# ikergarcia1996/AI-Generated-GTAV

Hardware: AMD Instinct MI355X
Metric: generated frames/sec (32-frame clip, 100 noise steps) (higher is better)
Workload: dtype fp16 (fp32 accumulate/residual)

## Files before the change

### ai-generated-gtav_amd/csrc/api.hip

```cpp
#include "api_internal.h"

namespace gtav_shared { thread_local hipEvent_t g_launch_ev[2] = {nullptr, nullptr}; }
namespace gtav {
static thread_local char g_err[1024] = "";
void set_error(const char* fmt, ...) {
    va_list ap;
    va_start(ap, fmt);
    vsnprintf(g_err, sizeof(g_err), fmt, ap);
    va_end(ap);
}
const char* last_error() { return g_err; }
}
namespace gtav_bf16 {
void set_error(const char* fmt, ...) {
    va_list ap;
    va_start(ap, fmt);
    vsnprintf(gtav::g_err, sizeof(gtav::g_err), fmt, ap);
    va_end(ap);
}
const char* last_error() { return gtav::g_err; }
}

namespace {
const gtav_bf16::GemmParams& bfp(const GemmParams& p) { return reinterpret_cast<const gtav_bf16::GemmParams&>(p); }
const gtav_bf16::LnPending* bfl(const LnPending* p) { return reinterpret_cast<const gtav_bf16::LnPending*>(p); }
int f16_attn_spatial(const f16* Q, const f16* K, const f16* Vt, f16* O, int NB, int heads, int S, hipStream_t st, bool qp) { return launch_attn_spatial(Q, K, Vt, O, NB, heads, S, st, qp); }
int bf_gemm(const GemmParams& p, int epi, hipStream_t st) { return gtav_bf16::launch_gemm(bfp(p), epi, st); }
int bf_ln_modulate(float* x, int ldx, f16* out, int ldo, int M, int D, const float* shift, const float* scale, int mod_stride, const int* rows, int rpm,
                   const LnPending* pend, int* ef, hipStream_t st) {
    return gtav_bf16::launch_ln_modulate(x, ldx, (__bf16*)out, ldo, M, D, shift, scale, mod_stride, rows, rpm, bfl(pend), ef, st);
}
int bf_ln_affine(float* x, int ldx, f16* out, int ldo, int M, int D, const float* gamma, const float* beta, const LnPending* pend, int* ef, hipStream_t st) {
    return gtav_bf16::launch_ln_affine(x, ldx, (__bf16*)out, ldo, M, D, gamma, beta, bfl(pend), ef, st);
}
int bf_patchify(const float* img, const int* fi, int NB, int C, int H, int W, int p, f16* out, int ldo, float a, float b, int* ef, hipStream_t st) {
    return gtav_bf16::launch_patchify(img, fi, NB, C, H, W, p, (__bf16*)out, ldo, a, b, ef, st);
}
int f16_convert_pad(const float* src, int lds, int R, int C, f16* dst, int Rp, int Cp, float scale, int tiled, hipStream_t st, int* ef) {
    return launch_convert_pad_f16(src, lds, R, C, dst, Rp, Cp, scale, tiled, st, ef);
}
int bf_convert_pad(const float* src, int lds, int R, int C, f16* dst, int Rp, int Cp, float scale, int tiled, hipStream_t st, int* ef) {
    return gtav_bf16::launch_convert_pad_f16(src, lds, R, C, (__bf16*)dst, Rp, Cp, scale, tiled, st, ef);
}
int bf_unpad(const f16* src, int lds, int R, int C, float* dst, int tiled, hipStream_t st) { return gtav_bf16::launch_unpad_f16_to_f32((const __bf16*)src, lds, R, C, dst, tiled, st); }
int bf_attn_spatial(const f16* Q, const f16* K, const f16* Vt, f16* O, int NB, int heads, int S, hipStream_t st, bool qp) {
    return gtav_bf16::launch_attn_spatial((const __bf16*)Q, (const __bf16*)K, (const __bf16*)Vt, (__bf16*)O, NB, heads, S, st, qp);
}
int bf_attn_temporal(const f16* q, const f16* kv, f16* O, int B, int P, int D, int Tq, int t0, int Tmax, hipStream_t st) {
    return gtav_bf16::launch_attn_temporal((const __bf16*)q, (const __bf16*)kv, (__bf16*)O, B, P, D, Tq, t0, Tmax, st);
}
const OperandOps OPS_F16 = {launch_gemm, launch_ln_modulate, launch_ln_affine, launch_patchify, f16_convert_pad, launch_unpad_f16_to_f32, f16_attn_spatial,
                            launch_attn_temporal, false};
const OperandOps OPS_BF16 = {bf_gemm, bf_ln_modulate, bf_ln_affine, bf_patchify, bf_convert_pad, bf_unpad, bf_attn_spatial, bf_attn_temporal, true};
}
const OperandOps& gtav::operand_ops(bool bf16) { return bf16 ? OPS_BF16 : OPS_F16; }

namespace {
typedef const __bf16* cbp;
typedef __bf16* bp;
int f16_dw_grouped(const GemmDwGroup* g, int n, int K, int* ef, hipStream_t st, bool tn) { return launch_gemm_dw_grouped(g, n, K, ef, st, tn); }
int bf_gemm_tn(const GemmParams& p, hipStream_t st) { return gtav_bf16::launch_gemm_tn(bfp(p), st); }
int bf_dw_grouped(const GemmDwGroup* g, int n, int K, int* ef, hipStream_t st, bool tn) {
    return gtav_bf16::launch_gemm_dw_grouped(reinterpret_cast<const gtav_bf16::GemmDwGroup*>(g), n, K, ef, st, tn);
}
int bf_transpose(const f16* src, int R, int C, f16* dst, hipStream_t st) { return gtav_bf16::launch_transpose_tiled_f16((cbp)src, R, C, (bp)dst, st); }
int bf_convert_T(const float* src, int lds, int R, int C, f16* dst, hipStream_t st) { return gtav_bf16::launch_convert_T_f16(src, lds, R, C, (bp)dst, st); }
int bf_gelu(const f16* u, f16* h, size_t n, hipStream_t st) { return gtav_bf16::launch_gelu_tiled((cbp)u, (bp)h, n, st); }
int bf_gelu_bwd(const f16* dh, const f16* u, f16* du, size_t n, int* ef, hipStream_t st) { return gtav_bf16::launch_gelu_bwd_tiled((cbp)dh, (cbp)u, (bp)du, n, ef, st); }
int bf_gelu_bwd_colsum(const f16* dh, const f16* u, f16* du, int M, int N, float* db, float* ws, int* ef, hipStream_t st) {
    return gtav_bf16::launch_gelu_bwd_tiled_colsum((cbp)dh, (cbp)u, (bp)du, M, N, db, ws, ef, st);
}
int bf_gate_bwd(const float* dres, const float* gate, int ms, int rpm, int M, int D, f16* dy, int* ef, hipStream_t st) {
    return gtav_bf16::launch_gate_bwd(dres, gate, ms, rpm, M, D, (bp)dy, ef, st);
}
int bf_frame_reduce_gate(const float* dres, const f16* y, int frames, int P, int D, float* dgate, int ms, hipStream_t st) {
    return gtav_bf16::launch_frame_reduce_gate(dres, (cbp)y, frames, P, D, dgate, ms, st);
}
int bf_gate_bwd_fused(const float* dres, const f16* y, const float* gate, int ms, int frames, int P, int D, f16* dy, float* dgate, float* db, float* ws, int* ef,
                      hipStream_t st) {
    return gtav_bf16::launch_gate_bwd_fused(dres, (cbp)y, gate, ms, frames, P, D, (bp)dy, dgate, db, ws, ef, st);
}
int bf_colsum(const f16* dy, int M, int N, float* db, float* ws, hipStream_t st) { return gtav_bf16::launch_colsum_tiled_f16((cbp)dy, M, N, db, ws, st); }
int bf_to_tiled(const float* a, int M, int D, f16* out, int* ef, hipStream_t st) { return gtav_bf16::launch_to_tiled_f16(a, M, D, (bp)out, ef, st); }
int bf_mse_bwd(const float* vp, const float* vt, int B, int T, int C, int H, int W, int p, float scale, f16* dfo, int ldf, int* ef, hipStream_t st) {
    return gtav_bf16::launch_mse_bwd_patch(vp, vt, B, T, C, H, W, p, scale, (bp)dfo, ldf, ef, st);
}
int bf_attn_spatial_bwd(const f16* Q, const f16* K, const f16* Vt, const f16* dO, int NB, int heads, int S, int D, const float* cs, f16* dqkv, int* ef,
                        hipStream_t st) {
    return gtav_bf16::launch_attn_spatial_bwd((cbp)Q, (cbp)K, (cbp)Vt, (cbp)dO, NB, heads, S, D, cs, (bp)dqkv, ef, st);
}
int bf_attn_temporal_bwd(const f16* q, const f16* kv, const f16* dO, int B, int P, int D, int T, int Tmax, const float* cs, f16* dqkv, int* ef, hipStream_t st) {
    return gtav_bf16::launch_attn_temporal_bwd((cbp)q, (cbp)kv, (cbp)dO, B, P, D, T, Tmax, cs, (bp)dqkv, ef, st);
}
int bf_adamw_multi(const AdamParam* params, const AdamItem* items, int n, const float* ctl, float lr, float b1, float b2, float eps, float wd, hipStream_t st) {
    return gtav_bf16::launch_adamw_multi(reinterpret_cast<const gtav_bf16::AdamParam*>(params), reinterpret_cast<const gtav_bf16::AdamItem*>(items), n, ctl, lr,
                                         b1, b2, eps, wd, st);
}
const TrainOps TRAIN_F16 = {launch_gemm_tn, f16_dw_grouped, launch_transpose_tiled_f16, launch_convert_T_f16, launch_gelu_tiled, launch_gelu_bwd_tiled,
                            launch_gelu_bwd_tiled_colsum, launch_gate_bwd, launch_frame_reduce_gate, launch_gate_bwd_fused, launch_colsum_tiled_f16,
                            launch_to_tiled_f16, launch_mse_bwd_patch, launch_attn_spatial_bwd, launch_attn_temporal_bwd, launch_adamw_multi, false};
const TrainOps TRAIN_BF16 = {bf_gemm_tn, bf_dw_grouped, bf_transpose, bf_convert_T, bf_gelu, bf_gelu_bwd, bf_gelu_bwd_colsum, bf_gate_bwd, bf_frame_reduce_gate,
                             bf_gate_bwd_fused, bf_colsum, bf_to_tiled, bf_mse_bwd, bf_attn_spatial_bwd, bf_attn_temporal_bwd, bf_adamw_multi, true};
// ... 79 lines not shown
    g.gate = gate; g.gate_stride = gate_stride; g.rows_per_gate = rows_per_gate;
    return launch_gemm(g, epilogue, (hipStream_t)stream);
}
int gtav_op_gemm_qkv(const void* x, int32_t ldx, const void* w, const float* bias, int32_t M, int32_t D, int32_t mode, void* q,
                     void* k, void* v, int32_t S, int32_t Tq, int32_t t0, int32_t Tmax, const float* rope_cs, void* stream) {
    GemmParams g;
    memset(&g, 0, sizeof(g));
    g.X = (const f16*)x; g.ldx = ldx; g.W = (const f16*)w; g.M = M; g.N = 3 * D; g.K = D; g.bias = bias; g.D = D; g.S = S;
    g.qkv_mode = mode; g.q = (f16*)q; g.k = (f16*)k; g.v = (f16*)v; g.Tq = Tq; g.t0 = t0; g.Tmax = Tmax;
    g.rope_cs = rope_cs;
    return launch_gemm(g, EPI_QKV, (hipStream_t)stream);
}
#ifdef GTAV_EXPERIMENTS
int gtav_op_gemm_fold_producer(const void* x, const void* w, const float* bias, float* resid, int32_t M, int32_t N, int32_t K, const float* gate,
                               const float* next_scale, int32_t mod_stride, int32_t tokens_per_frame, void* a_out, float* stats_out, void* stream) {
    GemmParams g;
    memset(&g, 0, sizeof(g));
    g.X = (const f16*)x; g.ldx = K; g.W = (const f16*)w; g.M = M; g.N = N; g.K = K; g.bias = bias; g.out = resid; g.ldo = N;
    g.gate = gate; g.gate_stride = mod_stride; g.rows_per_gate = tokens_per_frame;
    g.f_P = tokens_per_frame; g.f_scale = next_scale; g.f_stats_out = stats_out; g.f_a = (f16*)a_out;
    return launch_gemm(g, EPI_RESID_FOLD, (hipStream_t)stream);
}
int gtav_op_gemm_fold_consumer(const void* a, const void* w, int32_t M, int32_t N, int32_t K, int32_t epi, const float* stats, const float* c1, const float* c2,
                               int32_t ldc, int32_t tokens_per_frame, void* out, int32_t ldo, void* stream) {
    GTAV_REQUIRE(epi == EPI_F32 || epi == EPI_GELU_TANH, "gemm_fold_consumer: epilogue %d (0 = f32 row-major, 2 = GELU-tanh fp16 tile-major)", epi);
    GemmParams g;
    memset(&g, 0, sizeof(g));
    g.X = (const f16*)a; g.ldx = K; g.W = (const f16*)w; g.M = M; g.N = N; g.K = K; g.out = out; g.ldo = ldo;
    g.f_P = tokens_per_frame; g.f_stats = stats; g.f_nslot = K / 64; g.f_c1 = c1; g.f_c2 = c2; g.f_ldc = ldc;
    return launch_gemm(g, epi == EPI_F32 ? EPI_F32_FOLD : EPI_GELU_TANH_FOLD, (hipStream_t)stream);
}
#endif
int gtav_op_skinny_f32(const float* x, int32_t ldx, const float* w, const float* bias, float* y, int32_t ldy, int32_t M,
                       int32_t N, int32_t K, int32_t act_silu, void* stream) {
    RET_IF(skinny_init());
    return launch_skinny_f32(x, ldx, w, bias, y, ldy, M, N, K, act_silu, (hipStream_t)stream);
}
int gtav_op_ln_modulate(const float* x, void* out, int32_t M, int32_t D, const float* shift, const float* scale,
                        int32_t mod_stride, int32_t rows_per_mod, void* stream) {
    return launch_ln_modulate((float*)x, D, (f16*)out, D, M, D, shift, scale, mod_stride, nullptr, rows_per_mod, nullptr, nullptr, (hipStream_t)stream);
}
int gtav_op_ln_affine(const float* x, void* out, int32_t M, int32_t D, const float* gamma, const float* beta, void* stream) {
    return launch_ln_affine((float*)x, D, (f16*)out, D, M, D, gamma, beta, nullptr, nullptr, (hipStream_t)stream);
}
int gtav_op_attn_spatial(const void* q, const void* k, const void* vt, void* o, int32_t NB, int32_t heads, int32_t S, void* stream) {
    return launch_attn_spatial((const f16*)q, (const f16*)k, (const f16*)vt, (f16*)o, NB, heads, S, (hipStream_t)stream);
}
int gtav_op_attn_temporal(const void* q, const void* kv, void* o, int32_t B, int32_t P, int32_t D, int32_t Tq, int32_t t0,
                          int32_t Tmax, void* stream) {
    return launch_attn_temporal((const f16*)q, (const f16*)kv, (f16*)o, B, P, D, Tq, t0, Tmax, (hipStream_t)stream);
}
int gtav_op_attn_temporal_bf16(const void* q, const void* kv, void* o, int32_t B, int32_t P, int32_t D, int32_t Tq, int32_t t0,
                               int32_t Tmax, void* stream) {
    return gtav_bf16::launch_attn_temporal((const __bf16*)q, (const __bf16*)kv, (__bf16*)o, B, P, D, Tq, t0, Tmax, (hipStream_t)stream);
}
int gtav_op_qkv_head_major(const void* w, void* w_hm, int32_t D, void* stream) {
    return launch_qkv_head_major((const f16*)w, (f16*)w_hm, D, (hipStream_t)stream);
}
int gtav_op_gemm_qkvt_attn(const void* x_tperm, const void* w_hm, int32_t M, int32_t D, int32_t P, int32_t Tq, int32_t t0,
                           int32_t Tmax, const float* rope_cs, void* kv, void* o, void* stream) {
    GemmParams g;
    memset(&g, 0, sizeof(g));
    g.X = (const f16*)x_tperm; g.ldx = D; g.W = (const f16*)w_hm; g.M = M; g.N = 3 * D; g.K = D; g.D = D; g.S = P;
    g.qkv_mode = QKV_TEMPORAL; g.k = (f16*)kv; g.v = (f16*)kv; g.out = o; g.ldo = D; g.Tq = Tq; g.t0 = t0; g.Tmax = Tmax;
    g.rope_cs = rope_cs;
    return launch_gemm_qkvt_attn(g, (hipStream_t)stream);
}
int gtav_op_qkv_head_major_spatial(const void* w, void* w_hm, int32_t D, void* stream) {
    return launch_qkv_head_major((const f16*)w, (f16*)w_hm, D, (hipStream_t)stream, 1);
}
int gtav_op_gemm_qkvs_attn(const void* x, const void* w_hm, int32_t M, int32_t D, int32_t P, const float* rope_cs, void* o, void* stream) {
    GemmParams g;
    memset(&g, 0, sizeof(g));
    g.X = (const f16*)x; g.ldx = D; g.W = (const f16*)w_hm; g.M = M; g.N = 3 * D; g.K = D; g.D = D; g.S = P;
    g.qkv_mode = QKV_SPATIAL; g.out = o; g.ldo = D; g.rope_cs = rope_cs;
    return launch_gemm_qkvs_attn(g, (hipStream_t)stream);
}
int gtav_op_attn_spatial_bwd(const void* q, const void* k, const void* vt, const void* d_o, int32_t NB, int32_t heads, int32_t S,
                             const float* rope_cs, void* dqkv, void* stream) {
    return launch_attn_spatial_bwd((const f16*)q, (const f16*)k, (const f16*)vt, (const f16*)d_o, NB, heads, S, heads * 64, rope_cs, (f16*)dqkv, nullptr,
                                   (hipStream_t)stream);
}
int gtav_op_attn_spatial_bwd_bf16(const void* q, const void* k, const void* vt, const void* d_o, int32_t NB, int32_t heads, int32_t S,
                                  const float* rope_cs, void* dqkv, void* stream) {
    return gtav_bf16::launch_attn_spatial_bwd((const __bf16*)q, (const __bf16*)k, (const __bf16*)vt, (const __bf16*)d_o, NB, heads, S, heads * 64, rope_cs,
                                              (__bf16*)dqkv, nullptr, (hipStream_t)stream);
}
int gtav_op_gemm_tn(const void* x, const void* w, int32_t M, int32_t N, int32_t K, float* out, int32_t ldo, void* stream) {
    GemmParams q;
    memset(&q, 0, sizeof(q));
    q.X = (const f16*)x; q.ldx = M; q.W = (const f16*)w; q.M = M; q.N = N; q.K = K; q.out = out; q.ldo = ldo;
    return launch_gemm_tn(q, (hipStream_t)stream);
}
int gtav_op_gemm_dw_grouped(int32_t n, const void* const* x, const void* const* w, float* const* out, const int32_t* M, const int32_t* N, const int32_t* ldo,
                            int32_t K, void* stream) {
    GTAV_REQUIRE(n >= 1 && n <= GEMM_DW_MAX_GROUPS && x && w && out && M && N && ldo, "op_gemm_dw_grouped: 1 .. %d groups", GEMM_DW_MAX_GROUPS);
    GemmDwGroup g[GEMM_DW_MAX_GROUPS];
    for (int i = 0; i < n; ++i) g[i] = GemmDwGroup{(const f16*)x[i], (const f16*)w[i], out[i], M[i], N[i], ldo[i]};
    return launch_gemm_dw_grouped(g, n, K, nullptr, (hipStream_t)stream);
}
int gtav_op_gemm_splitk_ln(const void* x, int32_t ldx, const void* w, const float* bias, int32_t M, int32_t N, int32_t K,
                           int32_t splitk, float* parts, float* resid, const float* gate, int32_t gate_stride,
                           int32_t rows_per_gate, void* out_f16, const float* shift, const float* scale, int32_t mod_stride,
                           void* stream) {
    GemmParams g;
    memset(&g, 0, sizeof(g));
    g.X = (const f16*)x; g.ldx = ldx; g.W = (const f16*)w; g.M = M; g.N = N; g.K = K; g.out = parts; g.ldo = N;
// ... 62 lines not shown
```

### ai-generated-gtav_amd/csrc/api_dit.hip

```cpp
#include "api_internal.h"

#ifdef GTAV_EXPERIMENTS
static int fold_alloc(gtav_dit* h) {
    gtav_dit::Fold& f = h->fold;
    if (f.ok) return 0;
    GTAV_REQUIRE(f.geom_ok, "dit_set_fold: this geometry has no LayerNorm fold (tokens per frame %d must be a multiple of 16 and >= 64, hidden %% 256 == 0)", h->P);
    Arena& a = h->arena;
    const int D = h->D;
    const size_t Mx = round_up(h->Mmax, 128);
    int rc = 0;
#define A_(expr) do { if (!rc) rc = (expr); } while (0)
    {
        const int nhb = h->L * 2, nseam = 2 * nhb + 1;
        f.col_c.assign(nseam, 0);
        int col = 0;
        for (int hb = 0; hb < nhb; ++hb) { f.col_c[2 * hb + 1] = col; col += 2 * h->Hm; }
        for (int hb = 0; hb < nhb; ++hb) { f.col_c[2 * hb] = col; col += 2 * 3 * D; }
        f.col_c[2 * nhb] = col; col += 2 * h->Nfin;
        f.CTW = col;
        f.n_groups = 2 * nseam; f.n_groups_a = 2 * nhb;
        f.Rp = round_up(h->max_rows, 128);
        A_(a.alloc_t(&f.ctab, (size_t)h->max_rows * f.CTW));
        A_(a.alloc_t(&f.ctab_cur, (size_t)h->maxB * h->maxT * f.CTW));
        A_(a.alloc_t(&f.stats, Mx * (size_t)(D / 64) * 2));
// ... 15 lines not shown
                add(nhb + hb, 2 * hb, h->halves[hb].w_qkv, 3 * D, nullptr, (hb * 6 + 0) * D, (hb * 6 + 1) * D);
            }
            add(2 * nhb, 2 * nhb, h->w_final, h->Nfin, h->b_final, h->L * 12 * D, h->L * 12 * D + D);
            if (hipMemcpy(f.groups_dev, groups.data(), groups.size() * sizeof(GemmGroup), hipMemcpyHostToDevice) != hipSuccess ||
                hipMemcpy(f.gcol_dev, gcol.data(), gcol.size() * sizeof(int), hipMemcpyHostToDevice) != hipSuccess ||
                hipMemcpy(f.gscale_dev, gsc.data(), gsc.size() * sizeof(int), hipMemcpyHostToDevice) != hipSuccess) {
                set_error("dit_create: upload of the LayerNorm-fold group tables failed");
                rc = 1;
            }
            f.ok = !rc;
        }
    }
#undef A_
    return rc;
}
#endif

static bool fused_spatial_ok(int M, int D, int P) { return gemm_qkvs_attn_ok(M, D, P) && M / P >= 5 && (M / P) * (D / 64) >= 80; }

static void fold_policy(const gtav_dit* h, int M, bool& fa, bool& fb) {
    const gtav_dit::Fold& f = h->fold;
    fa = fb = false;
    if (!f.ok || f.mode == 0 || h->tr.on || h->fuse_tattn || h->any_bf16) return;
    fa = f.mode == 2 || M >= f.min_m_a;
    fb = f.mode == 2 || M >= f.min_m_b;
}
static int dit_fold_tables(gtav_dit* h, int rows, bool fa, bool fb, hipStream_t s) {
    if (!fa && !fb) return 0;
#ifndef GTAV_EXPERIMENTS
    (void)h; (void)rows; (void)s;
    GTAV_REQUIRE(false, "the LayerNorm fold exists only in the experiments build");
#else
    gtav_dit::Fold& f = h->fold;
    const int ng = fb ? f.n_groups : f.n_groups_a;
    RET_IF(launch_ctab_inputs(h->mod, h->MODW, rows, round_up(rows, 128), h->D, f.gcol_dev, f.gscale_dev, ng, f.sx, (size_t)f.Rp * h->D, s));
    return launch_gemm_grouped(f.groups_dev, ng, h->Hm > 3 * h->D ? h->Hm : 3 * h->D, rows, h->D, s);
#endif
}

static int dit_cond(gtav_dit* h, const int64_t* t64, int rows, int Tq, const StepParams* sp, int use_cur, const float* actions,
                    int64_t act_outer, int64_t act_inner, hipStream_t s) {
    GTAV_REQUIRE(rows <= h->max_rows, "conditioning rows %d exceed max_cond_rows %d", rows, h->max_rows);
    const int ldhc = h->D + h->Apad;
    RET_IF(launch_cond_inputs(t64, rows, Tq, sp, use_cur, h->sincos, h->E, actions, act_outer, act_inner, h->A, h->HC, ldhc,
                              h->D, h->Apad, h->err_flag, s));
    RET_IF(launch_skinny_f32(h->E, 256, h->w_t0, h->b_t0, h->HC, ldhc, rows, h->D, 256, 1, s));
    RET_IF(launch_skinny_f32(h->HC, ldhc, h->w_t2cat, actions ? h->b_t2a : h->b_t2, h->Sc, h->D, rows, h->D, ldhc, 1, s));
    RET_IF(launch_skinny_f32(h->Sc, h->D, h->w_ada, h->b_ada, h->mod, h->MODW, rows, h->MODW, h->D, 0, s));
    bool fa, fb;
    fold_policy(h, rows * h->P, fa, fb);
    return dit_fold_tables(h, rows, fa, fb, s);
}

static int dit_forward_core(gtav_dit* h, const float* x_src, const int* frame_index, int B, int Tq, int t0,
                            const float* mod, const int* mod_rows, const float* ctab, float* v_out, hipStream_t s) {
    const int D = h->D, P = h->P, NB = B * Tq, M = NB * P;
    GTAV_REQUIRE(M <= h->Mmax, "forward: %d tokens exceed workspace (%d)", M, h->Mmax);
    bool fold_a, fold_b;
    fold_policy(h, M, fold_a, fold_b);
    const gtav_dit::Fold& fo = h->fold;
    auto fold_consumer = [&](GemmParams& q, int seam, int N) {
        q.bias = nullptr;
        q.f_P = P; q.f_rows = mod_rows; q.f_stats = fo.stats; q.f_nslot = D / 64;
        q.f_c1 = ctab + fo.col_c[seam]; q.f_c2 = q.f_c1 + N; q.f_ldc = fo.CTW;
    };
    auto fold_producer = [&](int cls, const f16* X, const f16* Wt, int K, const float* bias, const float* gate, const float* next_scale) -> int {
        GemmParams q;
        memset(&q, 0, sizeof(q));
        q.X = X; q.ldx = K; q.W = Wt; q.M = M; q.N = D; q.K = K; q.out = h->resid; q.ldo = D; q.bias = bias; q.err_flag = h->err_flag;
        q.gate = gate; q.gate_stride = h->MODW; q.gate_rows = mod_rows; q.rows_per_gate = P;
        q.f_P = P; q.f_rows = mod_rows; q.f_scale = next_scale; q.f_stats_out = fo.stats; q.f_a = h->xn;
        PROF(h, cls, s, launch_gemm(q, EPI_RESID_FOLD, s));
        return 0;
    };
    const int g_embed = 2 * h->L, g_final = 2 * h->L + 1;
    PROF(h, PC_OTHER, s, h->ops(g_embed).patchify(x_src, frame_index, NB, h->C, h->H, h->W, h->p, h->xp, h->Kpe, 1.f, 0.f, h->err_of(g_embed), s));
    GemmParams g;
    memset(&g, 0, sizeof(g));
    g.X = h->xp; g.ldx = h->Kpe; g.W = h->w_pe; g.M = M; g.N = D; g.K = h->Kpe; g.bias = h->b_pe; g.out = h->resid; g.ldo = D;
    PROF(h, PC_OTHER, s, h->ops(g_embed).gemm(g, EPI_F32, s));
    LnPending pend;
    bool have_pend = false;
    const int pf_max_m = 1536;
    static const int pf_min_m = GTAV_ENV_INT("GTAV_PF_MIN_M", 256);
    const bool pf_on = h->w_prefetch && M >= pf_min_m && M <= pf_max_m;
    struct PfNext { const f16* W; int N, K, sk, consumer; };
    auto pf_target = [&](int hb, int pos) -> PfNext {
        const int q = pos + 1, hb2 = hb + q / 4, p2 = q % 4;
        if (!pf_on || hb2 >= 2 * h->L) return PfNext{nullptr, 0, 0, 1, 0};
        const gtav_dit::Half& w2 = h->halves[hb2];
        if (p2 == 0) {
            const bool fused2 = !h->tr.on && w2.w_qkv_hm && !h->ops(hb2).bf16 &&
                                ((hb2 & 1) ? h->fuse_tattn && gemm_qkvt_attn_ok(M, D, P, Tq, t0) : h->fuse_sattn && fused_spatial_ok(M, D, P));
            return PfNext{fused2 ? w2.w_qkv_hm : w2.w_qkv, 3 * D, D, 1, 3};
        }
        if (p2 == 1) return PfNext{w2.w_out, D, D, gemm_choose_splitk(M, D, D), 0};
        if (p2 == 2) return PfNext{w2.w_fc1, h->Hm, D, 1, 1};
        return PfNext{w2.w_fc2, D, h->Hm_pad, gemm_choose_splitk(M, D, h->Hm_pad), 2};
    };
    auto set_pf = [&](GemmParams& q, const PfNext& t) {
        const int v = h->w_prefetch_cls[t.consumer];
        if (!pf_on || !t.W || !v) return;
        const int nkt = t.K / 64;
        int skn = t.sk;
        if (skn < 1 || nkt % skn || (skn >= 8 ? skn % 8 : 8 % skn)) skn = 1;
        q.pf = PrefetchDesc{t.W, cdiv(t.N, 128), nkt, skn, v >= 2 ? v : 0};
    };
    auto resid_gemm = [&](const OperandOps& ops, int cls, const f16* X, int ldx, const f16* Wt, int K, const float* bias, const float* gate, const PfNext& pfn) -> int {
        GemmParams q;
        memset(&q, 0, sizeof(q));
        q.X = X; q.ldx = ldx; q.W = Wt; q.M = M; q.N = D; q.K = K; q.out = h->parts; q.ldo = D;
        set_pf(q, pfn);
        q.splitk = gemm_choose_splitk(M, D, K);
        if (gemm_pp_ok(M, D, K, EPI_RESID) || (q.splitk == 1 && M >= h->resid_inplace_min_m) || gemm_resid_inplace_ok(M, D, K, P)) {
            q.splitk = 0; q.out = h->resid; q.bias = bias; q.gate = gate; q.gate_stride = h->MODW; q.gate_rows = mod_rows;
            q.rows_per_gate = P;
            PROF(h, cls, s, ops.gemm(q, EPI_RESID, s));
            have_pend = false;
            return 0;
        }
        GTAV_REQUIRE((size_t)q.splitk * M <= h->parts_rows, "split-K slabs exceed workspace");
        PROF(h, cls, s, ops.gemm(q, EPI_PARTIAL, s));
        memset(&pend, 0, sizeof(pend));
        pend.parts = h->parts; pend.nsplit = q.splitk; pend.slab_stride = (size_t)M * D; pend.ld = D; pend.bias = bias;
        pend.gate = gate; pend.gate_stride = h->MODW; pend.gate_rows = mod_rows; pend.rows_per_gate = P;
        have_pend = true;
        return 0;
    };
    bool folded_in = false;
    for (int l = 0; l < h->L; ++l) {
        for (int hf = 0; hf < 2; ++hf) {
            const int hb = l * 2 + hf;
            const gtav_dit::Half& w = h->halves[hb];
            const OperandOps& ops = h->ops(hb);
            int* const ef = h->err_of(hb);
            const float* mb = mod + (size_t)hb * 6 * D;
            const bool fused_t = hf == 1 && h->fuse_tattn && !h->tr.on && !ops.bf16 && w.w_qkv_hm && gemm_qkvt_attn_ok(M, D, P, Tq, t0);
            if (fused_t) {
                if (!have_pend) memset(&pend, 0, sizeof(pend));
                pend.tperm_T = Tq; pend.tperm_P = P;
            }
            if (!folded_in)
                PROF(h, PC_LN, s, ops.ln_modulate(h->resid, D, h->xn, D, M, D, mb, mb + D, h->MODW, mod_rows, P, (have_pend || fused_t) ? &pend : nullptr, ef, s));
            have_pend = false;
            memset(&g, 0, sizeof(g));
            g.X = h->xn; g.ldx = D; g.W = w.w_qkv; g.M = M; g.N = 3 * D; g.K = D; g.D = D; g.S = P; g.err_flag = ef;
            if (folded_in) fold_consumer(g, 2 * hb, 3 * D);
            set_pf(g, pf_target(hb, 0));
            const bool fused_s = hf == 0 && h->fuse_sattn && !h->tr.on && !ops.bf16 && !folded_in && w.w_qkv_hm && fused_spatial_ok(M, D, P);
            if (fused_t) {
                g.W = w.w_qkv_hm; g.qkv_mode = QKV_TEMPORAL; g.k = h->kvcache[l]; g.v = h->kvcache[l]; g.out = h->ao; g.ldo = D;
                g.Tq = Tq; g.t0 = t0; g.Tmax = h->maxT; g.rope_cs = h->rope_t.cs_dev;
                PROF(h, PC_ATTN_T, s, launch_gemm_qkvt_attn(g, s));
            } else if (fused_s) {
                g.W = w.w_qkv_hm; g.qkv_mode = QKV_SPATIAL; g.out = h->ao; g.ldo = D; g.rope_cs = h->rope_s.cs_dev;
                PROF(h, PC_ATTN_S, s, launch_gemm_qkvs_attn(g, s));
            } else {
                if (hf == 0) {
                    g.qkv_mode = QKV_SPATIAL; g.q = h->qs; g.k = h->ks; g.v = h->vts;
                    g.rope_cs = h->rope_s.cs_dev;
                } else {
                    g.qkv_mode = QKV_TEMPORAL; g.q = h->qt; g.k = h->kvcache[l]; g.v = h->kvcache[l];
                    g.Tq = Tq; g.t0 = t0; g.Tmax = h->maxT;
                    g.rope_cs = h->rope_t.cs_dev;
                }
                PROF(h, PC_QKV, s, ops.gemm(g, folded_in ? EPI_QKV_FOLD : EPI_QKV, s));
                if (hf == 0) PROF(h, PC_ATTN_S, s, ops.attn_spatial(h->qs, h->ks, h->vts, h->ao, NB, h->heads, P, s, false));
                else PROF(h, PC_ATTN_T, s, ops.attn_temporal(h->qt, h->kvcache[l], h->ao, B, P, D, Tq, t0, h->maxT, s));
            }
            folded_in = false;
            memset(&g, 0, sizeof(g));
            g.X = h->xn; g.ldx = D; g.W = w.w_fc1; g.M = M; g.N = h->Hm; g.K = D; g.bias = w.b_fc1; g.out = h->hbuf; g.ldo = h->Hm_pad; g.err_flag = ef;
            set_pf(g, pf_target(hb, 2));
            if (fold_a) {
                RET_IF(fold_producer(PC_OUT, h->ao, w.w_out, D, w.b_out, mb + 2 * D, mb + 4 * D));
                fold_consumer(g, 2 * hb + 1, h->Hm);
                PROF(h, PC_FC1, s, launch_gemm(g, EPI_GELU_TANH_FOLD, s));
            } else {
                RET_IF(resid_gemm(ops, PC_OUT, h->ao, D, w.w_out, D, w.b_out, mb + 2 * D, pf_target(hb, 1)));
                PROF(h, PC_LN, s, ops.ln_modulate(h->resid, D, h->xn, D, M, D, mb + 3 * D, mb + 4 * D, h->MODW, mod_rows, P, have_pend ? &pend : nullptr, ef, s));
                have_pend = false;
                PROF(h, PC_FC1, s, ops.gemm(g, EPI_GELU_TANH, s));
            }
            if (fold_b) {
                const float* next_scale = hb + 1 < 2 * h->L ? mod + (size_t)(hb + 1) * 6 * D + D : mod + (size_t)h->L * 12 * D + D;
                RET_IF(fold_producer(PC_FC2, h->hbuf, w.w_fc2, h->Hm_pad, w.b_fc2, mb + 5 * D, next_scale));
                folded_in = true;
            } else {
                RET_IF(resid_gemm(ops, PC_FC2, h->hbuf, h->Hm_pad, w.w_fc2, h->Hm_pad, w.b_fc2, mb + 5 * D, pf_target(hb, 3)));
            }
        }
    }
    const float* mf = mod + (size_t)h->L * 12 * D;
    if (!folded_in)
        PROF(h, PC_LN, s, h->ops(g_final).ln_modulate(h->resid, D, h->xn, D, M, D, mf, mf + D, h->MODW, mod_rows, P, have_pend ? &pend : nullptr, h->err_of(g_final), s));
    memset(&g, 0, sizeof(g));
    g.X = h->xn; g.ldx = D; g.W = h->w_final; g.M = M; g.N = h->Nfin; g.K = D; g.bias = h->b_final; g.out = h->fo; g.ldo = h->Nfin;
    if (folded_in) fold_consumer(g, 4 * h->L, h->Nfin);
    PROF(h, PC_OTHER, s, h->ops(g_final).gemm(g, folded_in ? EPI_F32_FOLD : EPI_F32, s));
    PROF(h, PC_OTHER, s, launch_unpatchify(h->fo, h->Nfin, v_out, NB, h->C, h->H, h->W, h->p, 0, 1.f, 0.f, s));
    PROF(h, PC_EMPTY, s, 0);
    return h->prof.collect(s);
}

extern "C" {



int gtav_dit_create(const gtav_dit_config* c, gtav_dit** out) {
    GTAV_REQUIRE(c && out, "dit_create: null argument");
    GTAV_REQUIRE(c->hidden_size % 256 == 0 && c->hidden_size <= 2048, "hidden_size=%d must be a multiple of 256, <= 2048", c->hidden_size);
    GTAV_REQUIRE(c->num_heads > 0 && c->hidden_size / c->num_heads == 64 && c->hidden_size % c->num_heads == 0,
                 "only head_dim 64 is implemented (hidden %d, heads %d)", c->hidden_size, c->num_heads);
    GTAV_REQUIRE(c->input_h % c->patch_size == 0 && c->input_w % c->patch_size == 0, "input %dx%d not divisible by patch %d",
                 c->input_h, c->input_w, c->patch_size);
    GTAV_REQUIRE(c->max_frames >= 1 && c->max_frames <= 32, "max_frames=%d must be in [1, 32]", c->max_frames);
    GTAV_REQUIRE(c->max_batch >= 1 && c->depth >= 1, "bad max_batch/depth");
    RET_IF(skinny_init());
    gtav_dit* h = new gtav_dit();
    h->cfg = *c;
    h->D = c->hidden_size; h->L = c->depth; h->heads = c->num_heads; h->C = c->in_channels; h->p = c->patch_size;
    h->H = c->input_h; h->W = c->input_w; h->gh = h->H / h->p; h->gw = h->W / h->p; h->P = h->gh * h->gw;
    const int D = h->D;
    if ((h->P % 8) != 0) {
        set_error("tokens per frame P=%d must be a multiple of 8", h->P);
        delete h;
        return 2;
    }
    h->Hm = (int)(D * c->mlp_ratio); h->Hm_pad = round_up(h->Hm, 128);
    h->A = c->external_cond_dim > 0 ? c->external_cond_dim : 0; h->Apad = round_up(h->A > 0 ? h->A : 1, 32);
    h->MODW = h->L * 12 * D + 2 * D;
    h->Kpe = round_up(h->C * h->p * h->p, 64);
    h->Nfin = h->p * h->p * h->C;
    h->maxB = c->max_batch; h->maxT = c->max_frames; h->Mmax = h->maxB * h->maxT * h->P;
    h->max_rows = c->max_cond_rows > h->maxB * h->maxT ? c->max_cond_rows : h->maxB * h->maxT;
    Arena& a = h->arena;
    WeightTable& wt = h->wt;
    int rc = 0;
#define A_(expr) do { if (!rc) rc = (expr); } while (0)
    A_(a.alloc_t(&h->w_pe, (size_t)round_up(D, 128) * h->Kpe));
    h->n_groups = 2 * h->L + 2;
    h->grp_bf16.assign(h->n_groups, 0);
    wt.add_f16("x_embedder.proj.weight", D, h->C * h->p * h->p, h->w_pe, round_up(D, 128), h->Kpe, 2 * h->L);
    A_(a.alloc_t(&h->b_pe, D)); wt.add_f32("x_embedder.proj.bias", 1, D, h->b_pe, D);
    A_(a.alloc_t(&h->w_t0, (size_t)D * 256)); wt.add_f32("t_embedder.mlp.0.weight", D, 256, h->w_t0, 256);
    A_(a.alloc_t(&h->b_t0, D)); wt.add_f32("t_embedder.mlp.0.bias", 1, D, h->b_t0, D);
    const int ldhc = D + h->Apad;
    A_(a.alloc_t(&h->w_t2cat, (size_t)D * ldhc)); wt.add_f32("t_embedder.mlp.2.weight", D, D, h->w_t2cat, ldhc, 0);
    A_(a.alloc_t(&h->b_t2, D)); wt.add_f32("t_embedder.mlp.2.bias", 1, D, h->b_t2, D);
    A_(a.alloc_t(&h->b_ext, D)); A_(a.alloc_t(&h->b_t2a, D));
    if (h->A > 0) {
        wt.add_f32("external_cond.weight", D, h->A, h->w_t2cat, ldhc, D);
        wt.add_f32("external_cond.bias", 1, D, h->b_ext, D);
// ... 106 lines not shown
                const float ang = (float)t * ft[d / 2];
                c[t * 64 + d] = cosf(ang); sn[t * 64 + d] = sinf(ang);
            }
        RET_IF(upload(h->rope_t.cos_dev, c)); RET_IF(upload(h->rope_t.sin_dev, sn));
    }
    if (!h->wt.slots["tables.timestep_sincos"].set) {
        std::vector<float> tab((size_t)1000 * 256);
        for (int k = 0; k < 128; ++k) {
            const float f = expf(-logf(10000.0f) * (float)k / 128.0f);
            for (int t = 0; t < 1000; ++t) {
                const float arg = (float)t * f;
                tab[(size_t)t * 256 + k] = cosf(arg);
                tab[(size_t)t * 256 + 128 + k] = sinf(arg);
            }
        }
        RET_IF(upload(h->sincos, tab));
    }
    for (size_t hb = 0; hb < h->halves.size(); ++hb) {
        gtav_dit::Half& w = h->halves[hb];
        if (w.w_qkv_hm) RET_IF(launch_qkv_head_major(w.w_qkv, w.w_qkv_hm, D, s, (hb & 1) ? 0 : 1));
    }
    RET_IF(launch_rope_interleave(h->rope_s.cos_dev, h->rope_s.sin_dev, h->rope_s.cs_dev, h->P, s));
    RET_IF(launch_rope_interleave(h->rope_t.cos_dev, h->rope_t.sin_dev, h->rope_t.cs_dev, h->maxT, s));
    GTAV_CHECK_HIP(hipStreamSynchronize(s));
    h->finalized = true;
    return 0;
}

int gtav_dit_forward(gtav_dit* h, const float* x, const int64_t* t, const float* actions, float* out, int32_t B, int32_t T,
                     void* stream) {
    GTAV_REQUIRE(h && x && t && out, "dit_forward: null argument");
    GTAV_REQUIRE(h->finalized, "dit_forward: call gtav_dit_finalize first");
    GTAV_REQUIRE(B >= 1 && B <= h->maxB && T >= 1 && T <= h->maxT, "dit_forward: B=%d T=%d outside capacity (%d, %d)", B, T, h->maxB, h->maxT);
    GTAV_REQUIRE(!actions || h->A > 0, "dit_forward: model has no external_cond");
    hipStream_t s = (hipStream_t)stream;
    h->prepared.valid = false;
    h->kvrec.valid = false;
    RET_IF(dit_cond(h, t, B * T, 1, nullptr, 0, actions, h->A, 0, s));
    return dit_forward_core(h, x, nullptr, B, T, 0, h->mod, nullptr, h->fold.ctab, out, s);
}

int gtav_dit_set_schedule(gtav_dit* h, const float* ac, int32_t n) {
    GTAV_REQUIRE(h && ac && n == 1000, "dit_set_schedule: expected 1000 alphas_cumprod values");
    h->ac_host.assign(ac, ac + n);
    GTAV_CHECK_HIP(hipMemcpy(h->ac_table, ac, n * sizeof(float), hipMemcpyHostToDevice));
    return 0;
}

static int denoise_step_body(gtav_dit* h, float* x, int B, int F, int T, const float* actions, int mode, float* v_out,
                             bool prepared, hipStream_t s) {
    const size_t fsz = (size_t)h->C * h->H * h->W;
    const int Tq = mode == 1 ? 1 : T, t0 = mode == 1 ? T - 1 : 0;
    if (!prepared) RET_IF(dit_cond(h, nullptr, B * Tq, Tq, h->step_dev, mode == 1, actions, (int64_t)F * h->A, h->A, s));
    RET_IF(dit_forward_core(h, x, h->frame_idx, B, Tq, t0, prepared ? h->mod_cur : h->mod, nullptr, prepared ? h->fold.ctab_cur : h->fold.ctab, h->vout, s));
    const float* vlast = h->vout + (size_t)(Tq - 1) * fsz;
    RET_IF(launch_ddim_update_step(x, F, vlast, (size_t)Tq * fsz, B, (int)fsz, h->step_dev, s));
    if (v_out) RET_IF(launch_copy_rows_f32(vlast, (size_t)Tq * fsz, v_out, fsz, B, fsz, s));
    return 0;
}

int gtav_dit_prepare_frame(gtav_dit* h, int32_t B, int32_t F, int32_t start, int32_t cur, int32_t t_ctx,
                           const int32_t* t_steps_host, int32_t n_steps, const float* actions, void* stream) {
    GTAV_REQUIRE(h && t_steps_host, "prepare_frame: null argument");
    GTAV_REQUIRE(h->finalized, "prepare_frame: finalize the model first");
    const int T = cur - start + 1;
    GTAV_REQUIRE(start >= 0 && cur < F && T >= 1 && T <= h->maxT && B >= 1 && B <= h->maxB && n_steps >= 1 && n_steps <= 1024,
                 "prepare_frame: bad window [%d, %d] / steps %d", start, cur, n_steps);
    GTAV_REQUIRE(!actions || h->A > 0, "prepare_frame: model has no external_cond");
    const int rows = B * (T - 1) + n_steps * B;
    GTAV_REQUIRE(rows <= h->max_rows, "prepare_frame: %d conditioning rows exceed max_cond_rows %d", rows, h->max_rows);
    hipStream_t s = (hipStream_t)stream;
    GTAV_CHECK_HIP(hipStreamSynchronize(s));
    GTAV_CHECK_HIP(hipMemcpy(h->t_steps_dev, t_steps_host, n_steps * sizeof(int), hipMemcpyHostToDevice));
    const int ldhc = h->D + h->Apad;
    RET_IF(launch_cond_inputs_frame(rows, B, T, F, start, cur, t_ctx, h->t_steps_dev, h->sincos, h->E, actions, h->A, h->HC, ldhc,
                                    h->D, h->Apad, h->err_flag, s));
    RET_IF(launch_skinny_f32(h->E, 256, h->w_t0, h->b_t0, h->HC, ldhc, rows, h->D, 256, 1, s));
    RET_IF(launch_skinny_f32(h->HC, ldhc, h->w_t2cat, actions ? h->b_t2a : h->b_t2, h->Sc, h->D, rows, h->D, ldhc, 1, s));
    RET_IF(launch_skinny_f32(h->Sc, h->D, h->w_ada, h->b_ada, h->mod, h->MODW, rows, h->MODW, h->D, 0, s));
    {
        bool fa, fb, fa1, fb1;
        fold_policy(h, B * T * h->P, fa, fb);
        fold_policy(h, B * h->P, fa1, fb1);
        RET_IF(dit_fold_tables(h, rows, fa || fa1, fb || fb1, s));
        h->prepared.fold_tables = fa || fa1 || fb || fb1;
    }
    GTAV_CHECK_HIP(hipMemsetAsync(h->mod_last, 0xFF, (size_t)h->maxB * h->maxT * sizeof(int), s));
    h->prepared.valid = true; h->prepared.B = B; h->prepared.F = F; h->prepared.start = start; h->prepared.cur = cur;
    h->prepared.n_steps = n_steps; h->prepared.actions = actions;
    return 0;
}

int gtav_dit_denoise_step(gtav_dit* h, float* x, int32_t B, int32_t F, int32_t start, int32_t cur, int32_t t_ctx,
                          int32_t t_cur, int32_t t_next, int32_t is_final, const float* actions, int32_t mode,
                          int32_t cond_step, float* v_out, void* stream) {
    GTAV_REQUIRE(h && x, "denoise_step: null argument");
    GTAV_REQUIRE(h->finalized && !h->ac_host.empty(), "denoise_step: finalize the model and set the schedule first");
    const int T = cur - start + 1;
    GTAV_REQUIRE(start >= 0 && cur < F && T >= 1 && T <= h->maxT && B >= 1 && B <= h->maxB, "denoise_step: bad window [%d, %d] of %d frames", start, cur, F);
    GTAV_REQUIRE(t_cur >= 0 && t_cur < 1000 && t_next >= 0 && t_next < 1000 && t_ctx >= 0 && t_ctx < 1000, "denoise_step: timestep out of range");
    GTAV_REQUIRE(!actions || h->A > 0, "denoise_step: model has no external_cond");
    GTAV_REQUIRE(mode == 0 || mode == 1, "denoise_step: mode %d", mode);
    const bool prepared = cond_step >= 0;
    if (prepared)
        GTAV_REQUIRE(h->prepared.valid && h->prepared.B == B && h->prepared.F == F && h->prepared.start == start &&
                         h->prepared.cur == cur && cond_step < h->prepared.n_steps && h->prepared.actions == actions,
                     "denoise_step: cond_step=%d but gtav_dit_prepare_frame was not called for this window", cond_step);
// ... 247 lines not shown
```

### ai-generated-gtav_amd/csrc/api_train.hip

```cpp
#include "api_internal.h"

static int g_dw_grouped = GTAV_ENV_INT("GTAV_DW_GROUPED", 1);
static int g_fuse_gelu_fwd = GTAV_ENV_INT("GTAV_FUSE_GELU_FWD", 1);
static int g_fuse_gelu = GTAV_ENV_INT("GTAV_FUSE_GELU_BWD", 1);
static int g_fuse_ln = GTAV_ENV_INT("GTAV_FUSE_LN_BWD", 1);
static int g_fuse_gate = GTAV_ENV_INT("GTAV_FUSE_GATE", 1);
static int g_dw_tn = GTAV_ENV_INT("GTAV_DW_TN", 1);

static int train_enable_body(gtav_dit* h, float* grad_arena_dev, int64_t grad_arena_numel);

static int train_window_ok(const gtav_dit* h) {
    GTAV_REQUIRE(h->maxT <= 8, "train_enable: training is implemented for windows of at most 8 frames (the backward temporal attention and the adaLN-gradient "
                 "reduction are sized for it); this handle was created with max_frames=%d", h->maxT);
    return 0;
}

extern "C" {

int gtav_dit_train_enable(gtav_dit* h, float* grad_arena_dev, int64_t grad_arena_numel) {
    GTAV_REQUIRE(h, "train_enable: null handle");
    RET_IF(train_window_ok(h));
    GTAV_REQUIRE(!h->tr.on, "train_enable: already enabled");
    GTAV_REQUIRE(!h->any_bf16, "train_enable: the training step runs on fp16 operands (gtav_dit_set_operand_dtype(h, -1, GTAV_OPERAND_F16) first)");
    return train_enable_body(h, grad_arena_dev, grad_arena_numel);
// ... 161 lines not shown
    GTAV_REQUIRE(h && x && t64 && out, "train_forward: null argument");
    GTAV_REQUIRE(h->tr.on && h->finalized, "train_forward: call gtav_dit_train_enable, load the weights and finalize first");
    GTAV_REQUIRE(B >= 1 && B <= h->maxB && T >= 1 && T <= h->maxT, "train_forward: B=%d T=%d outside capacity (%d, %d)", B, T, h->maxB, h->maxT);
    GTAV_REQUIRE(!actions || h->A > 0, "train_forward: model has no external_cond");
    hipStream_t s = (hipStream_t)stream;
    gtav_dit::Train& tr = h->tr;
    const int D = h->D, P = h->P, NB = B * T, M = NB * P, L = h->L, rows = NB, ldhc = D + h->Apad;
    h->prepared.valid = false;
    h->kvrec.valid = false;
    RET_IF(launch_cond_inputs(t64, rows, 1, nullptr, 0, h->sincos, h->E, actions, h->A, 0, h->A, h->HC, ldhc, D, h->Apad, h->err_flag, s));
    RET_IF(launch_skinny_f32(h->E, 256, h->w_t0, h->b_t0, tr.z0, D, rows, D, 256, 0, s));
    RET_IF(launch_silu(tr.z0, D, h->HC, ldhc, rows, D, s));
    RET_IF(launch_skinny_f32(h->HC, ldhc, h->w_t2cat, actions ? h->b_t2a : h->b_t2, tr.cpre, D, rows, D, ldhc, 0, s));
    RET_IF(launch_silu(tr.cpre, D, h->Sc, D, rows, D, s));
    RET_IF(launch_skinny_f32(h->Sc, D, h->w_ada, h->b_ada, h->mod, h->MODW, rows, h->MODW, D, 0, s));
    const float* mod = h->mod;
    const OperandOps& oe = h->ops(2 * L), &ofin = h->ops(2 * L + 1);
    RET_IF(oe.patchify(x, nullptr, NB, h->C, h->H, h->W, h->p, tr.xp, h->Kpe, 1.f, 0.f, h->err_flag, s));
    GemmParams g;
    memset(&g, 0, sizeof(g));
    g.X = tr.xp; g.ldx = h->Kpe; g.W = h->w_pe; g.M = M; g.N = D; g.K = h->Kpe; g.bias = h->b_pe; g.out = tr.res[0]; g.ldo = D;
    RET_IF(oe.gemm(g, EPI_F32, s));
    LnPending pend;
    bool have_pend = false;
    auto resid_gemm = [&](const OperandOps& o, const f16* X, const f16* Wt, int K, const float* bias, const float* gate, float* x_out, f16* y_save) -> int {
        GemmParams q;
        memset(&q, 0, sizeof(q));
        q.X = X; q.ldx = K; q.W = Wt; q.M = M; q.N = D; q.K = K; q.out = h->parts; q.ldo = D;
        q.splitk = gemm_choose_splitk(M, D, K);
        GTAV_REQUIRE((size_t)q.splitk * M <= h->parts_rows, "split-K slabs exceed workspace");
        RET_IF(o.gemm(q, EPI_PARTIAL, s));
        memset(&pend, 0, sizeof(pend));
        pend.parts = h->parts; pend.nsplit = q.splitk; pend.slab_stride = (size_t)M * D; pend.ld = D; pend.bias = bias;
        pend.gate = gate; pend.gate_stride = h->MODW; pend.gate_rows = nullptr; pend.rows_per_gate = P;
        pend.x_out = x_out; pend.y_save = y_save;
        have_pend = true;
        return 0;
    };
    for (int l = 0; l < L; ++l)
        for (int hf = 0; hf < 2; ++hf) {
            const int i = l * 2 + hf;
            const gtav_dit::Half& w = h->halves[i];
            gtav_dit::Train::HB& b = tr.hb[i];
            const float* mb = mod + (size_t)i * 6 * D;
            const OperandOps& o = h->ops(i);
            RET_IF(o.ln_modulate(i == 0 ? tr.res[0] : tr.res[2 * i - 1], D, b.xnA, D, M, D, mb, mb + D, h->MODW, nullptr, P, have_pend ? &pend : nullptr, h->err_flag, s));
            have_pend = false;
            memset(&g, 0, sizeof(g));
            g.X = b.xnA; g.ldx = D; g.W = w.w_qkv; g.M = M; g.N = 3 * D; g.K = D; g.D = D; g.S = P; g.err_flag = h->err_flag;
            if (hf == 0) { g.qkv_mode = QKV_SPATIAL; g.q = b.q; g.k = b.k; g.v = b.v; g.rope_cs = h->rope_s.cs_dev; }
            else { g.qkv_mode = QKV_TEMPORAL; g.q = b.q; g.k = b.k; g.v = b.k; g.Tq = T; g.t0 = 0; g.Tmax = h->maxT; g.rope_cs = h->rope_t.cs_dev; }
            RET_IF(o.gemm(g, EPI_QKV, s));
            if (hf == 0) RET_IF(o.attn_spatial(b.q, b.k, b.v, b.ao, NB, h->heads, P, s, false));
            else RET_IF(o.attn_temporal(b.q, b.k, b.ao, B, P, D, T, 0, h->maxT, s));
            RET_IF(resid_gemm(o, b.ao, w.w_out, D, w.b_out, mb + 2 * D, tr.res[2 * i + 1], b.y1));
            RET_IF(o.ln_modulate(tr.res[2 * i], D, b.xnB, D, M, D, mb + 3 * D, mb + 4 * D, h->MODW, nullptr, P, &pend, h->err_flag, s));
            have_pend = false;
            memset(&g, 0, sizeof(g));
            g.X = b.xnB; g.ldx = D; g.W = w.w_fc1; g.M = M; g.N = h->Hm; g.K = D; g.bias = w.b_fc1; g.out = b.u; g.ldo = h->Hm_pad; g.err_flag = h->err_flag;
            if (g_fuse_gelu_fwd) g.out2 = b.hh;
            RET_IF(o.gemm(g, EPI_F16_TILED, s));
            if (!g_fuse_gelu_fwd) RET_IF(h->tops(i).gelu_tiled(b.u, b.hh, (size_t)round_up(M, 128) * h->Hm_pad, s));
            RET_IF(resid_gemm(o, b.hh, w.w_fc2, h->Hm_pad, w.b_fc2, mb + 5 * D, tr.res[2 * i + 2], b.y2));
        }
    const float* mf = mod + (size_t)L * 12 * D;
    RET_IF(ofin.ln_modulate(tr.res[4 * L - 1], D, tr.xnF, D, M, D, mf, mf + D, h->MODW, nullptr, P, &pend, h->err_flag, s));
    memset(&g, 0, sizeof(g));
    g.X = tr.xnF; g.ldx = D; g.W = h->w_final; g.M = M; g.N = h->Nfin; g.K = D; g.bias = h->b_final; g.out = h->fo; g.ldo = h->Nfin;
    RET_IF(ofin.gemm(g, EPI_F32, s));
    RET_IF(launch_unpatchify(h->fo, h->Nfin, out, NB, h->C, h->H, h->W, h->p, 0, 1.f, 0.f, s));
    tr.B = B; tr.T = T; tr.M = M; tr.Mp = round_up(M, 64); tr.rows = rows; tr.have_actions = actions != nullptr; tr.have_fwd = true;
    return 0;
}

int gtav_dit_train_get_residual(gtav_dit* h, int32_t k, float* dst, int64_t numel, void* stream) {
    GTAV_REQUIRE(h && dst && h->tr.on && h->tr.have_fwd, "train_get_residual: no saved forward");
    GTAV_REQUIRE(k >= 0 && k <= 4 * h->L, "train_get_residual: k=%d must be in [0, %d]", k, 4 * h->L);
    GTAV_REQUIRE(numel == (int64_t)h->tr.M * h->D, "train_get_residual: expected %lld elements", (long long)h->tr.M * h->D);
    GTAV_CHECK_HIP(hipMemcpyAsync(dst, h->tr.res[k], numel * sizeof(float), hipMemcpyDeviceToDevice, (hipStream_t)stream));
    return 0;
}

int gtav_dit_train_backward_phases(gtav_dit* h, const float* v_pred, const float* v_target, int32_t phase_begin, int32_t phase_end, void* stream) {
    GTAV_REQUIRE(h && v_pred && v_target, "train_backward: null argument");
    GTAV_REQUIRE(h->tr.on && h->tr.have_fwd, "train_backward: no saved forward (gtav_dit_train_forward)");
    GTAV_REQUIRE(phase_begin >= 0 && phase_begin <= phase_end && phase_end <= h->L + 2, "train_backward: phases [%d, %d) outside [0, %d]", phase_begin, phase_end,
                 h->L + 2);
    hipStream_t s = (hipStream_t)stream;
    gtav_dit::Train& tr = h->tr;
    const int D = h->D, P = h->P, L = h->L, B = tr.B, T = tr.T, M = tr.M, Mp = tr.Mp, NB = B * T, rows = tr.rows, Hp = h->Hm_pad, MODW = h->MODW;
    const int ldhc = D + h->Apad;
    auto slot = [&](const std::string& n) -> Slot& { return h->wt.slots[n]; };
    const OperandOps* op = &h->ops(2 * L + 1);
    const TrainOps* to = &h->tops(2 * L + 1);
    auto gemm_dx = [&](const f16* A, const f16* WT, int N, int Kc, int epi, void* out, int ldo) -> int {
        GemmParams q;
        memset(&q, 0, sizeof(q));
        q.X = A; q.ldx = Kc; q.W = WT; q.M = M; q.N = N; q.K = Kc; q.out = out; q.ldo = ldo; q.err_flag = h->err_flag;
        return op->gemm(q, epi, s);
    };
    GemmDwGroup dwg[GEMM_DW_MAX_GROUPS];
    int ndw = 0;
    bool defer_dw = false;
    if (tr.tAg[0] && g_dw_grouped) {
        const GemmDwGroup probe[4] = {{tr.tAg[0], tr.tBg[0], tr.dres, D, Hp, Hp}, {tr.tAg[1], tr.tBg[1], tr.dres, Hp, D, D}, {tr.tAg[2], tr.tBg[2], tr.dres, D, D, D},
                                      {tr.tAg[3], tr.tBg[3], tr.dres, 3 * D, D, D}};
        defer_dw = gemm_dw_grouped_ok(probe, 4, Mp);
// ... 240 lines not shown
```

### ai-generated-gtav_amd/csrc/attention.hip

```cpp
#include "ops.h"
#include "attn_tile.h"

#include <cstdlib>

namespace gtav {

namespace {

constexpr float kScaleLog2e = kAttnQScale;

template <int NW, int NK>
__global__ __launch_bounds__(64 * NW) void attn_spatial_1p_kernel(const f16* __restrict__ Q, const f16* __restrict__ K,
                                                              const f16* __restrict__ Vt, f16* __restrict__ O, int heads, int S,
                                                              int qsplit, int sc1) {
    constexpr int S_pad = 16 * NK;
    static_assert(NK % 2 == 0 && NK <= 10, "an even number of 16-key tiles, at most 160 keys");
    extern __shared__ __attribute__((aligned(16))) char smem[];
    char* Ks = smem;
    constexpr int vstride = (S_pad + 8) * 2;
    char* Vs = smem + (size_t)S_pad * 128;
    const int tid = threadIdx.x, lane = tid & 63, w = tid >> 6;
    const int li = lane & 15, g = lane >> 4;
    const int bh = blockIdx.x;
    const int nb = bh / heads, head = bh - nb * heads;
// ... 249 lines not shown
                    const float alpha = __builtin_amdgcn_exp2f(-delta);
#pragma unroll
                    for (int dt = 0; dt < 5; ++dt) o[qt][dt] = o[qt][dt] * alpha;
                }
                nmref[qt] -= delta;
#pragma unroll
                for (int kt = 0; kt < 4; ++kt)
#pragma unroll
                    for (int r = 0; r < 4; ++r) sc[qt][kt][r] -= delta;
            }
        }
#pragma unroll
        for (int s2 = 0; s2 < 2; ++s2) {
            f16x8 pf[NQT];
#pragma unroll
            for (int qt = 0; qt < NQT; ++qt)
#pragma unroll
                for (int r = 0; r < 4; ++r) {
                    pf[qt][r] = (f16)__builtin_amdgcn_exp2f(sc[qt][2 * s2][r]);
                    pf[qt][4 + r] = (f16)__builtin_amdgcn_exp2f(sc[qt][2 * s2 + 1][r]);
                }
#pragma unroll
            for (int dt = 0; dt < 4; ++dt) {
                const f16x8 vf = *(const f16x8*)(sb + dt * 2048 + voff[s2]);
#pragma unroll
                for (int qt = 0; qt < NQT; ++qt) o[qt][dt] = mfma16(vf, pf[qt], o[qt][dt], 0, 0, 0);
            }
#pragma unroll
            for (int qt = 0; qt < NQT; ++qt) o[qt][4] = mfma16(ones, pf[qt], o[qt][4], 0, 0, 0);
        }
    }

    const int Dm = heads * 64;
#pragma unroll
    for (int qt = 0; qt < NQT; ++qt) {
        const float inv = 1.0f / o[qt][4][0];
        const int qrow = (qt0 + qt) * 16 + li;
        if (qrow < S) {
            const int mrow = nb * S + qrow;
#pragma unroll
            for (int dt = 0; dt < 4; ++dt) {
                f16x4 h;
#pragma unroll
                for (int r = 0; r < 4; ++r) h[r] = (f16)(o[qt][dt][r] * inv);
                store_f16x4_paired<16>(O + tiled_off(mrow, head * 64 + dt * 16 + 4 * g, Dm), h, lane, sc1 & 1);
            }
        }
    }
}

template <int TM>
__global__ __launch_bounds__(256) void attn_temporal_kernel(const f16* __restrict__ q, const f16* __restrict__ kv,
                                                            f16* __restrict__ O, int ncol, int P, int D, int Tq, int t0, int Tmax,
                                                            int split) {
    const int tpc = D >> 3;
    const int ci = threadIdx.x / tpc, lc = threadIdx.x - ci * tpc;
    const int bp = blockIdx.x * ((int)blockDim.x / tpc) + ci;
    if (bp >= ncol) return;
    const int b = bp / P, p = bp - b * P;
    const int c = lc * 8;
    const int tl_lo = split ? blockIdx.y : 0, tl_hi = split ? blockIdx.y + 1 : Tq;
    const int Tk = t0 + tl_hi;
    union H8 { f16x8 v; f16x2 h[4]; };
    H8 k8[TM], v8[TM];
#pragma unroll
    for (int t = 0; t < TM; ++t) {
        if (t < Tk) {
            const f16* base = kv + (((size_t)b * Tmax + t) * P + p) * 2 * D;
            k8[t].v = *(const f16x8*)(base + c);
            v8[t].v = *(const f16x8*)(base + D + c);
        }
    }
    H8 qall[TM];
#pragma unroll
    for (int tl = 0; tl < TM; ++tl)
        if (tl >= tl_lo && tl < tl_hi) qall[tl].v = *(const f16x8*)(q + (((size_t)b * Tq + tl) * P + p) * D + c);
#pragma unroll
    for (int tl = 0; tl < TM; ++tl) {
        if (tl >= tl_hi) break;
        if (tl < tl_lo) continue;
        const int tq = t0 + tl;
        const size_t row = ((size_t)b * Tq + tl) * P + p;
        float s[TM];
        float mx = -INFINITY;
#pragma unroll
        for (int t = 0; t < TM; ++t) {
            s[t] = -INFINITY;
            if (t <= tq) {
                float d = 0.f;
#pragma unroll
                for (int e = 0; e < 4; ++e) d = dot2acc(qall[tl].h[e], k8[t].h[e], d, false);
                s[t] = group8_sum(d) * 0.125f;
                mx = fmaxf(mx, s[t]);
            }
        }
        float den = 0.f, acc[8] = {0.f, 0.f, 0.f, 0.f, 0.f, 0.f, 0.f, 0.f};
#pragma unroll
        for (int t = 0; t < TM; ++t) {
            if (t <= tq) {
                const float pr = __builtin_amdgcn_exp2f((s[t] - mx) * 1.4426950408889634f);
                den += pr;
#pragma unroll
                for (int e = 0; e < 8; ++e) acc[e] = __builtin_fmaf(pr, (float)v8[t].v[e], acc[e]);
            }
        }
        const float inv = 1.0f / den;
        f16x8 o8;
#pragma unroll
        for (int e = 0; e < 8; ++e) o8[e] = (f16)(acc[e] * inv);
        *(f16x8*)(O + tiled_off((int)row, c, D)) = o8;
    }
}

template <int QG, int FB>
__global__ __launch_bounds__(256) void attn_temporal_stream_kernel(const f16* __restrict__ q, const f16* __restrict__ kv,
                                                                   f16* __restrict__ O, int ncol, int P, int D, int Tq, int t0, int Tmax) {
#pragma clang fp contract(off)
    const int tpc = D >> 3;
    const int ci = threadIdx.x / tpc, lc = threadIdx.x - ci * tpc;
    const int bp = blockIdx.x * ((int)blockDim.x / tpc) + ci;
    if (bp >= ncol) return;
    const int b = bp / P, p = bp - b * P;
    const int c = lc * 8;
    const int tl0 = blockIdx.y * QG;
    const int nq = Tq - tl0 < QG ? Tq - tl0 : QG;
    const int Tk = t0 + tl0 + nq;
    union H8 { f16x8 v; f16x2 h[4]; };
    H8 qv[QG];
    float m[QG], den[QG], acc[QG][8];
#pragma unroll
    for (int j = 0; j < QG; ++j) {
        qv[j].v = f16x8{};
        if (j < nq) qv[j].v = *(const f16x8*)(q + (((size_t)b * Tq + tl0 + j) * P + p) * D + c);
        m[j] = -INFINITY; den[j] = 0.f;
#pragma unroll
        for (int e = 0; e < 8; ++e) acc[j][e] = 0.f;
    }
    const size_t fstride = (size_t)P * 2 * D;
    const f16* const base = kv + ((size_t)b * Tmax * P + p) * 2 * D + c;
    H8 kc[FB], vc[FB];
#pragma unroll
    for (int i = 0; i < FB; ++i) {
        kc[i].v = f16x8{}; vc[i].v = f16x8{};
        if (i < Tk) {
            kc[i].v = *(const f16x8*)(base + i * fstride);
            vc[i].v = *(const f16x8*)(base + i * fstride + D);
        }
    }
    for (int tb = 0; tb < Tk; tb += FB) {
        H8 kn[FB], vn[FB];
#pragma unroll
        for (int i = 0; i < FB; ++i) {
            kn[i].v = f16x8{}; vn[i].v = f16x8{};
            if (tb + FB + i < Tk) {
                kn[i].v = *(const f16x8*)(base + (size_t)(tb + FB + i) * fstride);
                vn[i].v = *(const f16x8*)(base + (size_t)(tb + FB + i) * fstride + D);
            }
        }
#pragma unroll
        for (int i = 0; i < FB; ++i) {
            const int t = tb + i;
            if (t < Tk) {
                float vf[8];
#pragma unroll
                for (int e = 0; e < 8; ++e) vf[e] = (float)vc[i].v[e];
#pragma unroll
                for (int j = 0; j < QG; ++j) {
                    if (j < nq && t <= t0 + tl0 + j) {
                        float d = 0.f;
#pragma unroll
                        for (int e = 0; e < 4; ++e) d = dot2acc(qv[j].h[e], kc[i].h[e], d, false);
                        const float s = group8_sum(d) * 0.125f;
                        if (s > m[j]) {
                            const float r = __builtin_amdgcn_exp2f((m[j] - s) * 1.4426950408889634f);
                            den[j] *= r;
#pragma unroll
                            for (int e = 0; e < 8; ++e) acc[j][e] *= r;
                            m[j] = s;
                        }
                        const float pr = __builtin_amdgcn_exp2f((s - m[j]) * 1.4426950408889634f);
                        den[j] += pr;
#pragma unroll
                        for (int e = 0; e < 8; ++e) acc[j][e] = __builtin_fmaf(pr, vf[e], acc[j][e]);
                    }
                }
            }
// ... 49 lines not shown
            }                                                                                                                         \
            GTAV_LAUNCH((attn_spatial_1p_kernel<4, NK_>), grid, dim3(256), lds, stream, Q, K, Vt, O, heads, S, qsplit, g_attn_sc1 & 1);   \
        } while (0)
#ifdef GTAV_EXPERIMENTS
        static const int nw_exp = GTAV_ENV_INT("GTAV_ATTN_1P_NW", 4);
#define GTAV_ATTN_1P_NW(NW_)                                                                                                            \
        do {                                                                                                                          \
            GTAV_CHECK_HIP(hipFuncSetAttribute((const void*)attn_spatial_1p_kernel<NW_, 10>, hipFuncAttributeMaxDynamicSharedMemorySize, 160 * 1024)); \
            int qs_ = 1;                                                                                                              \
            GTAV_LAUNCH((attn_spatial_1p_kernel<NW_, 10>), dim3(NB * heads, qs_), dim3(64 * NW_), lds, stream, Q, K, Vt, O, heads, S, qs_, g_attn_sc1 & 1); \
        } while (0)
        if (nk == 10 && nw_exp == 3) { GTAV_ATTN_1P_NW(3); GTAV_CHECK_HIP(hipGetLastError()); return 0; }
        if (nk == 10 && nw_exp == 5) { GTAV_ATTN_1P_NW(5); GTAV_CHECK_HIP(hipGetLastError()); return 0; }
        if (nk == 10 && nw_exp == 9) { GTAV_ATTN_1P_NW(9); GTAV_CHECK_HIP(hipGetLastError()); return 0; }
#undef GTAV_ATTN_1P_NW
#endif
        if (nk == 2) GTAV_ATTN_1P(2);
        else if (nk == 4) GTAV_ATTN_1P(4);
        else if (nk == 6) GTAV_ATTN_1P(6);
        else if (nk == 8) GTAV_ATTN_1P(8);
        else GTAV_ATTN_1P(10);
#undef GTAV_ATTN_1P
        GTAV_CHECK_HIP(hipGetLastError());
        return 0;
    }
    int best = 0, best_pad = 1 << 30, best_nqb = 0;
    for (int c = 2; c <= 4; ++c) {
        const int nqb_c = cdiv(nqt, 4 * c), pad = nqb_c * c;
        const bool better = pad < best_pad || (pad == best_pad && NB * heads * best_nqb >= 512);
        if (better) best = c, best_pad = pad, best_nqb = nqb_c;
    }
    static const int force_nqt = GTAV_ENV_INT("GTAV_ATTN_FLASH_NQT", 0), occ3 = GTAV_ENV_INT("GTAV_ATTN_FLASH_OCC3", 1);
    if (force_nqt >= 2 && force_nqt <= 4) best = force_nqt, best_nqb = cdiv(nqt, 4 * force_nqt);
    const int nfh = NB * heads;
    GTAV_REQUIRE((long long)nfh * best_nqb < (1ll << 31) && (long long)S * 64 * 2 < (1ll << 31), "attn_spatial: grid / sequence too large");
    const dim3 fgrid(nfh * best_nqb);
#define GTAV_ATTN_FLASH_(NQT_, OCC_, RG_, PS_) GTAV_LAUNCH((attn_flash_kernel<NQT_, OCC_, RG_, PS_>), fgrid, dim3(256), 0, stream, Q, K, Vt, O, heads, S, nfh, best_nqb, g_attn_sc1)
#define GTAV_ATTN_FLASH(NQT_, OCC_)                                                                    \
    do {                                                                                               \
        if (S % 64 != 0) { if (q_prescaled) GTAV_ATTN_FLASH_(NQT_, OCC_, true, true); else GTAV_ATTN_FLASH_(NQT_, OCC_, true, false); }   \
        else { if (q_prescaled) GTAV_ATTN_FLASH_(NQT_, OCC_, false, true); else GTAV_ATTN_FLASH_(NQT_, OCC_, false, false); }             \
    } while (0)
    if (best == 2) GTAV_ATTN_FLASH(2, 3);
    else if (best == 3 && occ3) GTAV_ATTN_FLASH(3, 3);
    else if (best == 3) GTAV_ATTN_FLASH(3, 2);
    else GTAV_ATTN_FLASH(4, 2);
#undef GTAV_ATTN_FLASH
#undef GTAV_ATTN_FLASH_
    GTAV_CHECK_HIP(hipGetLastError());
    return 0;
}

int launch_attn_temporal(const f16* q, const f16* kv, f16* O, int B, int P, int D, int Tq, int t0, int Tmax,
                         hipStream_t stream) {
    GTAV_REQUIRE(D % 256 == 0 && D <= 2048, "attn_temporal: D=%d must be a multiple of 256 and <= 2048", D);
    GTAV_REQUIRE(Tq > 0 && t0 >= 0 && t0 + Tq <= Tmax && Tmax <= 32, "attn_temporal: window t0=%d Tq=%d Tmax=%d (max 32)", t0, Tq, Tmax);
    GTAV_REQUIRE(P > 0 && B > 0 && (long long)B * Tq * P < (1ll << 31), "attn_temporal: B=%d P=%d Tq=%d", B, P, Tq);
    const int tpc = D / 8, cpb = tpc >= 256 ? 1 : 256 / tpc;
    const int Tvis = t0 + Tq;
    if (Tvis > 8) {
        if (Tq == 1) {
            GTAV_LAUNCH((attn_temporal_stream_kernel<1, 8>), dim3(cdiv(B * P, cpb), 1), dim3(tpc * cpb), 0, stream, q, kv, O, B * P, P, D, Tq, t0, Tmax);
        } else {
            GTAV_LAUNCH((attn_temporal_stream_kernel<8, 4>), dim3(cdiv(B * P, cpb), cdiv(Tq, 8)), dim3(tpc * cpb), 0, stream, q, kv, O, B * P, P, D, Tq, t0, Tmax);
        }
        GTAV_CHECK_HIP(hipGetLastError());
        return 0;
    }
    static const int split_max = GTAV_ENV_INT("GTAV_ATTN_T_SPLIT_MAX", 1024);
    const int split = (Tq > 1 && B * P < split_max) ? 1 : 0;
    const dim3 grid(cdiv(B * P, cpb), split ? Tq : 1), block(tpc * cpb);
    if (Tvis <= 5) GTAV_LAUNCH(attn_temporal_kernel<5>, grid, block, 0, stream, q, kv, O, B * P, P, D, Tq, t0, Tmax, split);
    else GTAV_LAUNCH(attn_temporal_kernel<8>, grid, block, 0, stream, q, kv, O, B * P, P, D, Tq, t0, Tmax, split);
    GTAV_CHECK_HIP(hipGetLastError());
    return 0;
}

}
```

### ai-generated-gtav_amd/csrc/common.h

```cpp
#pragma once
#include <hip/hip_runtime.h>
#include <hip/hip_fp16.h>
#include <hip/hip_ext.h>
#include <stdint.h>

#ifdef GTAV_BF16_OPERANDS
#define GTAV_F16_T __bf16
#else
#define GTAV_F16_T _Float16
#endif

namespace gtav {

typedef GTAV_F16_T f16;
typedef GTAV_F16_T f16x4 __attribute__((ext_vector_type(4)));
typedef GTAV_F16_T f16x8 __attribute__((ext_vector_type(8)));
typedef GTAV_F16_T f16x2 __attribute__((ext_vector_type(2)));
typedef float f32x4 __attribute__((ext_vector_type(4)));
typedef float f32x16 __attribute__((ext_vector_type(16)));

__device__ __forceinline__ f32x4 mfma16(f16x8 a, f16x8 b, f32x4 c, int, int, int) {
#ifdef GTAV_BF16_OPERANDS
    return __builtin_amdgcn_mfma_f32_16x16x32_bf16(a, b, c, 0, 0, 0);
#else
// ... 107 lines not shown
__device__ __forceinline__ f16x4 sat4(float a, float b, float c, float d, float& amax) {
    amax = __builtin_fmaxf(__builtin_fmaxf(__builtin_fabsf(a), __builtin_fabsf(b)), amax);
    amax = __builtin_fmaxf(__builtin_fmaxf(__builtin_fabsf(c), __builtin_fabsf(d)), amax);
    return f16x4{(f16)__builtin_amdgcn_fmed3f(a, -F16_MAX, F16_MAX), (f16)__builtin_amdgcn_fmed3f(b, -F16_MAX, F16_MAX),
                 (f16)__builtin_amdgcn_fmed3f(c, -F16_MAX, F16_MAX), (f16)__builtin_amdgcn_fmed3f(d, -F16_MAX, F16_MAX)};
}
__device__ __forceinline__ void sat_report(float amax, int* err_flag) {
    if (err_flag && amax > F16_MAX) atomicOr(err_flag, ERR_F16_SAT);
}

__device__ __forceinline__ float group8_sum(float v) {
    v += __builtin_bit_cast(float, __builtin_amdgcn_update_dpp(0, __builtin_bit_cast(int, v), 0xB1, 0xF, 0xF, true));
    v += __builtin_bit_cast(float, __builtin_amdgcn_update_dpp(0, __builtin_bit_cast(int, v), 0x4E, 0xF, 0xF, true));
    v += __builtin_bit_cast(float, __builtin_amdgcn_update_dpp(0, __builtin_bit_cast(int, v), 0x141, 0xF, 0xF, true));
    return v;
}

__device__ __forceinline__ float silu_f(float x) { return x / (1.0f + __expf(-x)); }

__device__ __forceinline__ float gelu_tanh_f(float x) {
    const float a = -2.0f * 1.4426950408889634f * 0.7978845608028654f, b = a * 0.044715f;
    const float e = __builtin_amdgcn_exp2f(x * __builtin_fmaf(x * x, b, a));
    return x * __builtin_amdgcn_rcpf(1.0f + e);
}

typedef float f32x2_ __attribute__((ext_vector_type(2)));
__device__ __forceinline__ void gelu_tanh_f4(const float (&x)[4], float (&y)[4]) {
    const float a = -2.0f * 1.4426950408889634f * 0.7978845608028654f, b = a * 0.044715f;
#pragma unroll
    for (int h = 0; h < 2; ++h) {
        const f32x2_ v = f32x2_{x[2 * h], x[2 * h + 1]};
        const f32x2_ t = __builtin_elementwise_fma(v * v, f32x2_{b, b}, f32x2_{a, a});
        const f32x2_ arg = v * t;
        const f32x2_ e = f32x2_{__builtin_amdgcn_exp2f(arg[0]), __builtin_amdgcn_exp2f(arg[1])};
        const f32x2_ d = e + f32x2_{1.0f, 1.0f};
        const f32x2_ r = f32x2_{__builtin_amdgcn_rcpf(d[0]), __builtin_amdgcn_rcpf(d[1])};
        const f32x2_ o = v * r;
        y[2 * h] = o[0];
        y[2 * h + 1] = o[1];
    }
}

__device__ __forceinline__ f32x2_ gelu_tanh_grad_f2(f32x2_ v) {
    const float k = 0.7978845608028654f, c = 0.044715f;
    const float a = -2.0f * 1.4426950408889634f * k, b = a * c, k2 = 2.0f * k, k6 = 6.0f * k * c;
    const f32x2_ z = v * v;
    const f32x2_ arg = v * __builtin_elementwise_fma(z, f32x2_{b, b}, f32x2_{a, a});
    const f32x2_ d = f32x2_{__builtin_amdgcn_exp2f(arg[0]), __builtin_amdgcn_exp2f(arg[1])} + f32x2_{1.0f, 1.0f};
    const f32x2_ s = f32x2_{__builtin_amdgcn_rcpf(d[0]), __builtin_amdgcn_rcpf(d[1])};
    const f32x2_ t = (v * s) * __builtin_elementwise_fma(z, f32x2_{k6, k6}, f32x2_{k2, k2});
    return __builtin_elementwise_fma(t, f32x2_{1.0f, 1.0f} - s, s);
}

__device__ __forceinline__ float gelu_erf_f(float x) { return 0.5f * x * (1.0f + erff(x * 0.7071067811865476f)); }

constexpr float kGeluErfL = 4.5f;
constexpr float kGeluErfC[10] = {9.985491633e-01f, -4.911968410e-01f, 3.479329944e-01f, -2.564433515e-01f, 1.821636558e-01f,
                                 -1.155658439e-01f, 6.453407556e-02f, -4.252957553e-02f, 2.962661162e-02f, -9.964072146e-03f};
__device__ __forceinline__ void gelu_erf_f4(const float (&x)[4], float (&y)[4]) {
    constexpr float r2 = 1.4142135623730951f, zs = r2 / kGeluErfL;
#pragma unroll
    for (int h = 0; h < 2; ++h) {
        const f32x2_ v = f32x2_{x[2 * h], x[2 * h + 1]};
        const f32x2_ z = v * f32x2_{zs, zs};
        const f32x2_ zc = f32x2_{__builtin_amdgcn_fmed3f(z[0], -r2, r2), __builtin_amdgcn_fmed3f(z[1], -r2, r2)};
        const f32x2_ sm = __builtin_elementwise_fma(zc, zc, f32x2_{-1.0f, -1.0f});
        f32x2_ q = f32x2_{kGeluErfC[9], kGeluErfC[9]};
#pragma unroll
        for (int k = 8; k >= 0; --k) q = __builtin_elementwise_fma(q, sm, f32x2_{kGeluErfC[k], kGeluErfC[k]});
        const f32x2_ f = zc * q;
        const f32x2_ hx = v * f32x2_{0.5f, 0.5f};
        const f32x2_ o = __builtin_elementwise_fma(hx, f, hx);
        y[2 * h] = o[0];
        y[2 * h + 1] = o[1];
    }
}

__device__ __forceinline__ float wave_sum_dpp(float v) {
#define GTAV_DPP_ADD(ctrl, rmask) \
    v += __builtin_bit_cast(float, __builtin_amdgcn_update_dpp(0, __builtin_bit_cast(int, v), ctrl, rmask, 0xF, true))
    GTAV_DPP_ADD(0xB1, 0xF);
    GTAV_DPP_ADD(0x4E, 0xF);
    GTAV_DPP_ADD(0x141, 0xF);
    GTAV_DPP_ADD(0x140, 0xF);
    GTAV_DPP_ADD(0x142, 0xA);
    GTAV_DPP_ADD(0x143, 0xC);
#undef GTAV_DPP_ADD
    return __builtin_bit_cast(float, __builtin_amdgcn_readlane(__builtin_bit_cast(int, v), 63));
}

__device__ __forceinline__ float wave_sum(float v) {
#pragma unroll
    for (int o = 32; o > 0; o >>= 1) v += __shfl_xor(v, o, 64);
    return v;
}
__device__ __forceinline__ float wave_max(float v) {
#pragma unroll
    for (int o = 32; o > 0; o >>= 1) v = fmaxf(v, __shfl_xor(v, o, 64));
    return v;
}

typedef unsigned u32x4 __attribute__((ext_vector_type(4)));
__device__ __forceinline__ void store16_sc1(void* dst, u32x4 v) {
    asm volatile("global_store_dwordx4 %0, %1, off sc1\n\ts_nop 1" ::"v"(dst), "v"(v) : "memory");
}
__device__ __forceinline__ void store16_sc1(void* dst, f32x4 v) {
// ... 25 lines not shown
```

### ai-generated-gtav_amd/csrc/elementwise.hip

```cpp
#include "ops.h"

#include <cstdlib>
#include <type_traits>

#include <cstring>

namespace gtav {

namespace {

template <int MODE, int NV>
__global__ __launch_bounds__(256) void ln_wave_row_kernel(const float* __restrict__ x, int ldx, f16* __restrict__ out, int M, int D,
                                                          const float* __restrict__ p0, const float* __restrict__ p1, int mod_stride,
                                                          const int* __restrict__ rows, int rows_per_mod, int flags, int* err_flag) {
    const int lane = threadIdx.x & 63;
    const int m = blockIdx.x * 4 + (threadIdx.x >> 6);
    if (m >= M) return;
    const float* xr = x + (size_t)m * ldx;
    f32x4 v[NV], av[NV], bv[NV];
#pragma unroll
    for (int i = 0; i < NV; ++i) v[i] = *(const f32x4*)(xr + i * 256 + lane * 4);
    const float *a, *b;
    if (MODE == 0) {
        int row = m / rows_per_mod;
        if (rows) row = rows[row];
        a = p1 + (size_t)row * mod_stride;
        b = p0 + (size_t)row * mod_stride;
    } else {
        a = p0;
        b = p1;
    }
#pragma unroll
    for (int i = 0; i < NV; ++i) {
        av[i] = *(const f32x4*)(a + i * 256 + lane * 4);
        bv[i] = *(const f32x4*)(b + i * 256 + lane * 4);
    }
    const float kshift = __builtin_bit_cast(float, __builtin_amdgcn_readfirstlane(__builtin_bit_cast(int, v[0][0])));
    float s1 = 0.f, s2 = 0.f;
#pragma unroll
    for (int i = 0; i < NV; ++i) {
        const float a0 = v[i][0] - kshift, a1 = v[i][1] - kshift, a2 = v[i][2] - kshift, a3 = v[i][3] - kshift;
        s1 += (a0 + a1) + (a2 + a3);
        s2 += (a0 * a0 + a1 * a1) + (a2 * a2 + a3 * a3);
    }
    const float t1 = wave_sum_dpp(s1), t2 = wave_sum_dpp(s2);
    const float m1 = t1 / (float)D, mean = kshift + m1;
    const float var = fmaxf(t2 / (float)D - m1 * m1, 0.f);
    const float rstd = 1.0f / sqrtf(var + 1e-6f);
    float amax = 0.f;
#pragma unroll
    for (int i = 0; i < NV; ++i) {
        float yv[4];
#pragma unroll
        for (int e = 0; e < 4; ++e) {
            const float xh = (v[i][e] - mean) * rstd;
            if (MODE == 0) {
                const float sc = av[i][e] + 1e-6f;
                yv[e] = xh * (1.0f + sc) + bv[i][e];
            } else {
                yv[e] = xh * av[i][e] + bv[i][e];
            }
        }
        store_f16x4_paired<1>(out + tiled_off(m, i * 256 + lane * 4, D), sat4(yv[0], yv[1], yv[2], yv[3], amax), lane, flags & 2);
    }
    sat_report(amax, err_flag);
}

#ifdef GTAV_EXPERIMENTS
#define LN_DBG(pd, b) ((pd).flags & (b))
#else
#define LN_DBG(pd, b) false
#endif
template <int MODE, bool PEND>
__global__ __launch_bounds__(512) void ln_row_block_kernel(float* __restrict__ x, int ldx, f16* __restrict__ out, int M, int D,
                                                           const float* __restrict__ p0, const float* __restrict__ p1,
                                                           int mod_stride, const int* __restrict__ rows, int rows_per_mod,
                                                           LnPending pd) {
    __shared__ float red[16];
    const int m = blockIdx.x;
    const int c = threadIdx.x * 4;
    const int nw = (blockDim.x + 63) >> 6, wid = threadIdx.x >> 6, lane = threadIdx.x & 63;
    float* xr = x + (size_t)m * ldx;
    const bool act = c < D;
    const bool nt = PEND && (pd.flags & 4);
    f32x4 v = f32x4{0.f, 0.f, 0.f, 0.f}, av = v, bv = v;
    if (act) v = nt ? __builtin_nontemporal_load((const f32x4*)(xr + c)) : *(const f32x4*)(xr + c);
    f32x4 sl[8];
    int nchunk = 0;
    if (PEND && act) {
        const float* pp = pd.parts + (size_t)m * pd.ld + c;
        auto slab = [&](int sp) -> f32x4 {
            const f32x4* q = (const f32x4*)(pp + (size_t)sp * pd.slab_stride);
            return nt ? __builtin_nontemporal_load(q) : *q;
        };
        nchunk = pd.nsplit <= 1 ? 1 : pd.nsplit <= 2 ? 2 : pd.nsplit <= 4 ? 4 : 8;
        if (nchunk == 1) {
            sl[0] = slab(0);
        } else if (nchunk == 2) {
#pragma unroll
            for (int sp = 0; sp < 2; ++sp) sl[sp] = slab(sp < pd.nsplit ? sp : 0);
        } else if (nchunk == 4) {
#pragma unroll
            for (int sp = 0; sp < 4; ++sp) sl[sp] = slab(sp < pd.nsplit ? sp : 0);
        } else {
#pragma unroll
            for (int sp = 0; sp < 8; ++sp) sl[sp] = slab(sp < pd.nsplit ? sp : 0);
        }
    }
    int row = 0, gr = 0;
    if (MODE == 0) {
        row = m / rows_per_mod;
        if (rows && !LN_DBG(pd, 0x2000)) row = rows[row];
    }
    if (PEND && pd.gate) {
        gr = m / pd.rows_per_gate;
        if (pd.gate_rows && !LN_DBG(pd, 0x2000)) gr = pd.gate_rows[gr];
    }
    const float kshift = LN_DBG(pd, 0x200) ? 0.f : xr[0];
    if (act && !LN_DBG(pd, 0x100)) {
        av = *(const f32x4*)((MODE == 0 ? p1 + (size_t)row * mod_stride : p0) + c);
        bv = *(const f32x4*)((MODE == 0 ? p0 + (size_t)row * mod_stride : p1) + c);
    }
    if (PEND && act) {
        f32x4 y = pd.bias && !LN_DBG(pd, 0x100) ? *(const f32x4*)(pd.bias + c) : f32x4{0.f, 0.f, 0.f, 0.f};
        f32x4 g4 = f32x4{1.f, 1.f, 1.f, 1.f};
        if (pd.gate && !LN_DBG(pd, 0x100)) g4 = *(const f32x4*)(pd.gate + (size_t)gr * pd.gate_stride + c);
#pragma unroll
        for (int sp = 0; sp < 8; ++sp)
            if (sp < nchunk && sp < pd.nsplit) y = y + sl[sp];
        if (pd.y_save) {
            float am = 0.f;
            *(f16x4*)(pd.y_save + (size_t)m * pd.ld + c) = sat4(y[0], y[1], y[2], y[3], am);
        }
        if (pd.gate) y = y * g4;
        v = v + y;
    }
    const float a0 = act ? v[0] - kshift : 0.f, a1 = act ? v[1] - kshift : 0.f, a2 = act ? v[2] - kshift : 0.f, a3 = act ? v[3] - kshift : 0.f;
    const float s1 = wave_sum_dpp((a0 + a1) + (a2 + a3));
    const float s2 = wave_sum_dpp((a0 * a0 + a1 * a1) + (a2 * a2 + a3 * a3));
    if (lane == 0) { red[wid] = s1; red[8 + wid] = s2; }
    if (!LN_DBG(pd, 0x400)) __syncthreads();
    if (PEND && act) {
        float* xw = pd.x_out ? pd.x_out + (size_t)m * ldx + c : xr + c;
        if (LN_DBG(pd, 0x800)) {}
        else if (pd.flags & 1) store16_sc1(xw, v);
        else *(f32x4*)xw = v;
    }
    float t1 = 0.f, t2 = 0.f;
#pragma unroll
    for (int i = 0; i < 8; ++i) { t1 += i < nw ? red[i] : 0.f; t2 += i < nw ? red[8 + i] : 0.f; }
    const float m1 = t1 / (float)D, mean = kshift + m1;
    const float var = fmaxf(t2 / (float)D - m1 * m1, 0.f);
    const float rstd = 1.0f / sqrtf(var + 1e-6f);
    if (!act) return;
    const float dd[4] = {v[0] - mean, v[1] - mean, v[2] - mean, v[3] - mean};
    float yv[4], amax = 0.f;
#pragma unroll
    for (int e = 0; e < 4; ++e) {
        const float xh = dd[e] * rstd;
        if (MODE == 0) {
            const float sc = av[e] + 1e-6f;
            yv[e] = xh * (1.0f + sc) + bv[e];
        } else {
            yv[e] = xh * av[e] + bv[e];
        }
    }
    int mo = m;
    if (pd.tperm_T > 0) {
        const int fr = m / pd.tperm_P, pp = m - fr * pd.tperm_P, bb = fr / pd.tperm_T, tt = fr - bb * pd.tperm_T;
        mo = ((bb * (pd.tperm_P >> 4) + (pp >> 4)) * pd.tperm_T + tt) * 16 + (pp & 15);
    }
    if (!LN_DBG(pd, 0x1000)) store_f16x4_paired<1>(out + tiled_off(mo, c, D), sat4(yv[0], yv[1], yv[2], yv[3], amax), lane, pd.flags & 2);
    else if (yv[0] == 1.2345f) out[0] = (f16)yv[1];
    sat_report(amax, pd.err_flag);
}

__global__ void patchify_kernel(const float* __restrict__ img, const int* __restrict__ frame_index, int NB, int C, int H,
                                int W, int p, f16* __restrict__ out, int ldo, float a, float b, int* err_flag) {
    const int gh = H / p, gw = W / p, Kp = C * p * p;
    const size_t total = (size_t)NB * gh * gw * ldo;
    for (size_t idx = (size_t)blockIdx.x * blockDim.x + threadIdx.x; idx < total; idx += (size_t)gridDim.x * blockDim.x) {
        const int k = (int)(idx % ldo);
        const size_t m = idx / ldo;
        float val = 0.f;
        if (k < Kp) {
            const int pw = k % p, ph = (k / p) % p, c = k / (p * p);
            const int x = (int)(m % gw), y = (int)((m / gw) % gh), nb = (int)(m / ((size_t)gw * gh));
            const int f = frame_index ? frame_index[nb] : nb;
            val = a * img[(((size_t)f * C + c) * H + (y * p + ph)) * W + (x * p + pw)] + b;
            if (!(__builtin_fabsf(val) <= F16_MAX)) {
                if (err_flag) atomicOr(err_flag, val != val || __builtin_isinf(val) ? ERR_NONFINITE : ERR_F16_SAT);
                if (val == val) val = __builtin_amdgcn_fmed3f(val, -F16_MAX, F16_MAX);
            }
        }
        out[tiled_off((int)m, k, ldo)] = (f16)val;
    }
// ... 149 lines not shown
    *(u32x4*)(sx + (size_t)g * group_stride + tiled_off(r, k, D)) = o.u;
}

__global__ void cond_inputs_frame_kernel(int rows, int B, int T, int F, int start, int cur, int t_ctx, const int* __restrict__ t_steps,
                                         const float* __restrict__ sincos, float* __restrict__ E,
                                         const float* __restrict__ actions, int A, float* __restrict__ HC, int ldhc, int D,
                                         int Apad, int* err_flag) {
    const int r = blockIdx.x;
    if (r >= rows) return;
    const int nctx = B * (T - 1);
    int t, b, frame;
    if (r < nctx) {
        b = r / (T - 1);
        frame = start + (r - b * (T - 1));
        t = t_ctx;
    } else {
        const int q = r - nctx;
        const int sidx = q / B;
        b = q - sidx * B;
        frame = cur;
        t = t_steps[sidx];
    }
    if (t < 0 || t > 999) {
        if (threadIdx.x == 0 && err_flag) atomicOr(err_flag, 1);
        t = t < 0 ? 0 : 999;
    }
    for (int j = threadIdx.x; j < 256; j += blockDim.x) E[(size_t)r * 256 + j] = sincos[(size_t)t * 256 + j];
    const float* arow = actions ? actions + ((size_t)b * F + frame) * A : nullptr;
    for (int j = threadIdx.x; j < Apad; j += blockDim.x) HC[(size_t)r * ldhc + D + j] = (arow && j < A) ? arow[j] : 0.f;
}

__global__ void cond_inputs_kernel(const int64_t* __restrict__ t64, int rows, int Tq, const StepParams* __restrict__ sp, int use_cur,
                                   const float* __restrict__ sincos, float* __restrict__ E, const float* __restrict__ actions,
                                   long long act_outer, long long act_inner, int A, float* __restrict__ HC, int ldhc, int D,
                                   int Apad, int* err_flag) {
    const int r = blockIdx.x;
    if (r >= rows) return;
    const int ro = r / Tq, ri = r - ro * Tq;
    long long t;
    int frame0 = 0;
    if (t64) {
        t = (long long)t64[r];
    } else {
        t = ri == Tq - 1 ? sp->t_cur : sp->t_ctx;
        frame0 = use_cur ? sp->cur : sp->first;
    }
    if (t < 0 || t > 999) {
        if (threadIdx.x == 0 && err_flag) atomicOr(err_flag, 1);
        t = t < 0 ? 0 : 999;
    }
    for (int j = threadIdx.x; j < 256; j += blockDim.x) E[(size_t)r * 256 + j] = sincos[(size_t)t * 256 + j];
    const float* arow = actions ? actions + ro * act_outer + (frame0 + ri) * act_inner : nullptr;
    for (int j = threadIdx.x; j < Apad; j += blockDim.x) HC[(size_t)r * ldhc + D + j] = (arow && j < A) ? arow[j] : 0.f;
}

__device__ __forceinline__ float ddim_one(float xc, float vp, float at, float an, int is_final) {
    const float x0 = sqrtf(at) * xc - sqrtf(1.0f - at) * vp;
    if (is_final) return x0;
    const float eps = (sqrtf(1.0f / at) * xc - x0) / sqrtf(1.0f / at - 1.0f);
    return sqrtf(an) * x0 + sqrtf(1.0f - an) * eps;
}

__global__ void ddim_update_kernel(const float* __restrict__ x, size_t x_stride, const float* __restrict__ v, size_t v_stride,
                                   float* __restrict__ out, size_t out_stride, int n, const float* __restrict__ alpha_t,
                                   const float* __restrict__ alpha_next, int is_final) {
    const int b = blockIdx.y;
    const float at = alpha_t[b];
    const float an = alpha_next ? alpha_next[b] : 1.f;
    for (int i = blockIdx.x * blockDim.x + threadIdx.x; i < n; i += gridDim.x * blockDim.x)
        out[b * out_stride + i] = ddim_one(x[b * x_stride + i], v[b * v_stride + i], at, an, is_final);
}

__global__ void ddim_update_step_kernel(float* __restrict__ x, size_t frames_per_sample, const float* __restrict__ v,
                                        size_t v_stride, int n, const StepParams* __restrict__ sp) {
    const int b = blockIdx.y;
    const float at = sp->alpha_t, an = sp->alpha_next;
    const int fin = sp->is_final;
    float* xf = x + ((size_t)b * frames_per_sample + sp->cur) * n;
    for (int i = blockIdx.x * blockDim.x + threadIdx.x; i < n; i += gridDim.x * blockDim.x)
        xf[i] = ddim_one(xf[i], v[b * v_stride + i], at, an, fin);
}

__global__ void add_noise_kernel(const float* __restrict__ x, const float* __restrict__ noise, const float* __restrict__ alpha,
                                 float* __restrict__ out, int n, float clamp_abs) {
    const int r = blockIdx.y;
    const float a = alpha[r];
    const float sa = sqrtf(a), s1 = sqrtf(1.0f - a);
    for (int i = blockIdx.x * blockDim.x + threadIdx.x; i < n; i += gridDim.x * blockDim.x) {
        const size_t o = (size_t)r * n + i;
        const float z = fminf(fmaxf(noise[o], -clamp_abs), clamp_abs);
        out[o] = x[o] * sa + s1 * z;
    }
}

__global__ void vtarget_kernel(const float* __restrict__ x, const float* __restrict__ noise, const float* __restrict__ alpha,
                               float* __restrict__ vt, int n, float clamp_abs) {
    const int r = blockIdx.y;
    const float a = alpha[r];
    const float sa = sqrtf(a), s1 = sqrtf(1.0f - a);
    for (int i = blockIdx.x * blockDim.x + threadIdx.x; i < n; i += gridDim.x * blockDim.x) {
        const size_t o = (size_t)r * n + i;
        const float z = fminf(fmaxf(noise[o], -clamp_abs), clamp_abs);
        vt[o] = sa * z - s1 * x[o];
    }
}

__global__ __launch_bounds__(256) void mse_partial_kernel(const float* __restrict__ a, size_t a_stride, const float* __restrict__ b,
                                                          size_t b_stride, int n, float* __restrict__ partial) {
    __shared__ float red[4];
    const int r = blockIdx.x;
    float s = 0.f;
    for (int i = threadIdx.x; i < n; i += 256) {
        const float d = a[r * a_stride + i] - b[r * b_stride + i];
// ... 113 lines not shown
inline int grid_for(size_t total, int block = 256) {
    size_t g = (total + block - 1) / block;
    if (g > 256 * 16) g = 256 * 16;
    if (g < 1) g = 1;
    return (int)g;
}

__global__ void qkv_head_major_kernel(const f16* __restrict__ src, f16* __restrict__ dst, int D, int mode) {
    const size_t i = (size_t)blockIdx.x * blockDim.x + threadIdx.x;
    const int cpr = D >> 3;
    if (i >= (size_t)3 * D * cpr) return;
    const int nd = (int)(i / cpr), kc = (int)(i - (size_t)nd * cpr);
    const int hd = nd / 192, rem = nd - hd * 192;
    int which, d;
    if (mode == 0) {
        which = rem >> 6;
        d = rem & 63;
    } else {
        const int w = rem / 48, r48 = rem - w * 48;
        which = r48 >> 4;
        d = 16 * w + (r48 & 15);
    }
    const int ns = which * D + hd * 64 + d;
    *(uint4*)(dst + tiled_off(nd, kc * 8, D)) = *(const uint4*)(src + tiled_off(ns, kc * 8, D));
}

__global__ void calib_spin_kernel(unsigned long long ticks, unsigned long long* __restrict__ dev_ticks) {
    const unsigned long long t0 = __builtin_amdgcn_s_memrealtime();
    unsigned long long t1 = t0;
    while (t1 - t0 < ticks) {
        __builtin_amdgcn_s_sleep(2);
        t1 = __builtin_amdgcn_s_memrealtime();
    }
    if (threadIdx.x == 0) dev_ticks[0] = t1 - t0;
}

}

static int g_ln_flags = GTAV_ENV_INT("GTAV_LN_FLAGS", 7);

static int g_ln_wave_row_min = GTAV_ENV_INT("GTAV_LN_WAVE_ROW_MIN", 0);

#define LN_WAVE_ROW_(MODE, NV, P0, P1, STRIDE, ROWS, RPM) \
    GTAV_LAUNCH((ln_wave_row_kernel<MODE, NV>), dim3(cdiv(M, 4)), dim3(256), 0, stream, x, ldx, out, M, D, P0, P1, STRIDE, ROWS, RPM, pd_.flags, err_flag)
#define LN_DISPATCH(MODE, P0, P1, STRIDE, ROWS, RPM)                                                     \
    do {                                                                                                  \
        LnPending pd_;                                                                                    \
        memset(&pd_, 0, sizeof(pd_));                                                                     \
        if (pend) pd_ = *pend;                                                                            \
        pd_.flags = g_ln_flags;                                                                           \
        pd_.err_flag = err_flag;                                                                          \
        GTAV_REQUIRE(pd_.tperm_T == 0 || (pd_.tperm_P % 16 == 0 && M % (pd_.tperm_T * pd_.tperm_P) == 0), "ln: bad output row permutation"); \
        const bool upd_ = pend && pend->parts;    \
        if (!upd_ && pd_.tperm_T == 0 && M >= g_ln_wave_row_min && (D == 256 || D == 512 || D == 1024 || D == 2048)) { \
            if (D == 256) LN_WAVE_ROW_(MODE, 1, P0, P1, STRIDE, ROWS, RPM);                               \
            else if (D == 512) LN_WAVE_ROW_(MODE, 2, P0, P1, STRIDE, ROWS, RPM);                          \
            else if (D == 1024) LN_WAVE_ROW_(MODE, 4, P0, P1, STRIDE, ROWS, RPM);                         \
            else LN_WAVE_ROW_(MODE, 8, P0, P1, STRIDE, ROWS, RPM);                                        \
        } else {                                                                   \
            const dim3 g_(M), b_(round_up(D / 4, 64));                                                    \
            if (upd_) GTAV_LAUNCH((ln_row_block_kernel<MODE, true>), g_, b_, 0, stream, x, ldx, out, M, D, P0, P1, STRIDE, ROWS, RPM, pd_); \
            else GTAV_LAUNCH((ln_row_block_kernel<MODE, false>), g_, b_, 0, stream, x, ldx, out, M, D, P0, P1, STRIDE, ROWS, RPM, pd_);     \
        }                                                                                                 \
    } while (0)

int launch_ln_modulate(float* x, int ldx, f16* out, int ldo, int M, int D, const float* shift, const float* scale,
                       int mod_stride, const int* rows, int rows_per_mod, const LnPending* pend, int* err_flag, hipStream_t stream) {
    GTAV_REQUIRE(D % 64 == 0 && D <= 2048 && rows_per_mod > 0 && ldo == D, "ln_modulate: D=%d must be %%64, <= 2048, ldo == D", D);
    GTAV_REQUIRE(!pend || !pend->parts || (pend->nsplit >= 1 && pend->nsplit <= 8 && pend->ld % 4 == 0 && (!pend->gate || pend->rows_per_gate > 0)),
                 "ln_modulate: bad pending update");
    LN_DISPATCH(0, shift, scale, mod_stride, rows, rows_per_mod);
    GTAV_CHECK_HIP(hipGetLastError());
    return 0;
}

int launch_ln_affine(float* x, int ldx, f16* out, int ldo, int M, int D, const float* gamma, const float* beta,
                     const LnPending* pend, int* err_flag, hipStream_t stream) {
    GTAV_REQUIRE(D % 64 == 0 && D <= 2048 && ldo == D, "ln_affine: D=%d must be %%64, <= 2048, ldo == D", D);
    GTAV_REQUIRE(!pend || !pend->parts || (pend->nsplit >= 1 && pend->nsplit <= 8 && pend->ld % 4 == 0 && (!pend->gate || pend->rows_per_gate > 0)),
                 "ln_affine: bad pending update");
    LN_DISPATCH(1, gamma, beta, 0, (const int*)nullptr, 1);
    GTAV_CHECK_HIP(hipGetLastError());
    return 0;
}
#undef LN_DISPATCH
#undef LN_WAVE_ROW_

int launch_patchify(const float* img, const int* frame_index, int NB, int C, int H, int W, int p, f16* out, int ldo,
                    float a, float b, int* err_flag, hipStream_t stream) {
    GTAV_REQUIRE(H % p == 0 && W % p == 0 && ldo >= C * p * p, "patchify: bad geometry");
    const size_t total = (size_t)NB * (H / p) * (W / p) * ldo;
    if (p % 4 == 0 && W % 4 == 0 && ldo % 4 == 0 && ((uintptr_t)img & 15) == 0 && (size_t)NB * (H / p) * (W / p) < (1u << 31)) {
        hipLaunchKernelGGL(patchify4_kernel, dim3(NB * (H / p) * (W / p)), dim3(256), 0, stream, img, frame_index, C, H, W, p, out, ldo, a, b, err_flag);
        GTAV_CHECK_HIP(hipGetLastError());
        return 0;
    }
    hipLaunchKernelGGL(patchify_kernel, dim3(grid_for(total)), dim3(256), 0, stream, img, frame_index, NB, C, H, W, p, out,
                       ldo, a, b, err_flag);
    GTAV_CHECK_HIP(hipGetLastError());
    return 0;
}

int launch_unpatchify(const float* y, int ldy, float* img, int NB, int C, int H, int W, int p, int order, float a,
                      float b, hipStream_t stream) {
    GTAV_REQUIRE(H % p == 0 && W % p == 0 && ldy >= C * p * p, "unpatchify: bad geometry");
    const size_t total = (size_t)NB * C * H * W;
    hipLaunchKernelGGL(unpatchify_kernel, dim3(grid_for(total)), dim3(256), 0, stream, y, ldy, img, NB, C, H, W, p, order,
                       a, b);
    GTAV_CHECK_HIP(hipGetLastError());
    return 0;
}

int launch_convert_pad_f16(const float* src, int lds, int R, int C, f16* dst, int Rp, int Cp, float scale, int tiled,
                           hipStream_t stream, int* err_flag) {
// ... 180 lines not shown
```

### ai-generated-gtav_amd/csrc/gemm.h

```cpp
#pragma once
#include "common.h"

namespace gtav {

enum GemmEpi : int {
    EPI_F32 = 0,
    EPI_F16 = 1,
    EPI_GELU_TANH = 2,
    EPI_GELU_ERF = 3,
    EPI_RESID = 4,
    EPI_QKV = 5,
    EPI_PARTIAL = 6,
    EPI_F16_TILED = 7,
    EPI_RESID_FOLD = 8,
    EPI_QKV_FOLD = 9,
    EPI_GELU_TANH_FOLD = 10,
    EPI_F32_FOLD = 11,
};
constexpr bool epi_is_fold_consumer(int e) { return e == EPI_QKV_FOLD || e == EPI_GELU_TANH_FOLD || e == EPI_F32_FOLD; }
constexpr int epi_base(int e) { return e == EPI_QKV_FOLD ? EPI_QKV : e == EPI_GELU_TANH_FOLD ? EPI_GELU_TANH : e == EPI_F32_FOLD ? EPI_F32 : e; }

enum QkvMode : int {
    QKV_SPATIAL = 0,
    QKV_TEMPORAL = 1,
};

struct GemmParams {
    const f16* X;
    int ldx;
    const f16* W;
    int M, N, K;
    int debug;
    unsigned long long* stamps;
    int* err_flag;
    int out_sc1;
    int splitk;
    const float* bias;
    void* out2;
    void* out;
    int ldo;
    const float* gate;
    int gate_stride;
    const int* gate_rows;
    int rows_per_gate;
    int qkv_mode;
    f16* q;
    f16* k;
    f16* v;
    int D;
    int S;
    int Tq;
    int t0;
    int Tmax;
    const float* rope_cs;
    const float* rope_cs_q;
    struct TileMap { int tiles_m, tiles_n, gn, group, tiles; unsigned rcp_tiles, rcp_group, rcp_gn, rcp_gnlast; } tm;
    int f_P;
    const int* f_rows;
    const float* f_stats;
    int f_nslot;
    const float* f_c1;
    const float* f_c2;
    int f_ldc;
    float* f_stats_out;
    const float* f_scale;
    f16* f_a;
    PrefetchDesc pf;
    float* sk_ws;
    int* sk_flags;
    int sk_dp, sk_r;
};
constexpr int GEMM_SK_MAX_SPLIT = 128;
constexpr size_t gemm_sk_ws_bytes() { return (size_t)GEMM_SK_MAX_SPLIT * 256 * 256 * 4; }
constexpr size_t gemm_sk_flag_bytes() { return (size_t)GEMM_SK_MAX_SPLIT * 4; }

struct GemmGroup { const f16* X; const f16* W; float* out; const float* bias; int N; int ldo; };
int launch_gemm_grouped(const GemmGroup* groups_dev, int n_groups, int max_N, int M, int K, hipStream_t stream);

constexpr int GEMM_DW_MAX_GROUPS = 4;
struct GemmDwGroup { const f16* X; const f16* W; float* out; int M; int N; int ldo; };
bool gemm_dw_grouped_ok(const GemmDwGroup* g, int n, int K);
int launch_gemm_dw_grouped(const GemmDwGroup* g, int n, int K, int* err_flag, hipStream_t stream, bool tn = false);
// ... 21 lines not shown
```

### ai-generated-gtav_amd/csrc/gemm.hip

```cpp
#include "gemm.h"
#include "attn_tile.h"

#include <cstdlib>
#include <cstring>
#include <type_traits>
#include <hip/hip_ext.h>

namespace gtav {

namespace {

constexpr int TN = 128, TK = 64;
constexpr int TILE_BYTES = 128 * TK * 2;

typedef const __attribute__((address_space(1))) void* gptr_t;
typedef __attribute__((address_space(3))) void* lptr_t;

__device__ __forceinline__ void glds16(const char* src, char* lds_wave_base) {
    __builtin_amdgcn_global_load_lds((gptr_t)src, (lptr_t)lds_wave_base, 16, 0, 0);
}

__device__ __forceinline__ void glds16_s(const void* sbase, unsigned voff, unsigned lds_addr) {
    unsigned keep;
    asm volatile("s_mov_b32 %0, m0\n\ts_mov_b32 m0, %3\n\ts_nop 0\n\tglobal_load_lds_dwordx4 %1, %2\n\ts_mov_b32 m0, %0"
// ... 2132 lines not shown
    mainloop_l<false, NS, FI, FJ, WN, WM, NL>(p, smem, n0, m0, kt0, nkt, acc, bs, []() {});
    GTAV_STAMP(bs.t[2]);
    const int tid = threadIdx.x, lane = tid & 63, w = (tid >> 6) - NL, li = lane & 15, g = lane >> 4;
    const int head = n0 / TNB;
    const int pgs = p.S >> 4, tile_m = m0 / TM, b = tile_m / pgs, pg = tile_m - b * pgs;
    float amax = 0.f;
    __syncthreads();
    if (w >= 0) {
#pragma unroll
        for (int i = 0; i < FI; ++i) {
            const int nl = 16 * FI * w + 16 * i + 4 * g;
            const bool rope = nl < 128;
            const int d = nl & 63;
#pragma unroll
            for (int j = 0; j < FJ; ++j) {
                const int ml = 16 * j + li;
                f32x4 v = acc[i][j];
                if (rope) {
                    const f32x4 cs = *(const f32x4*)(p.rope_cs + (p.t0 + j) * 64 + d);
                    v = rope4(v, cs);
                }
                char* dst = smem + ml * PN + (((nl >> 3) ^ (ml & 7)) << 4) + ((nl >> 2) & 1) * 8;
                *(uint2*)dst = pack4(amax, v[0], v[1], v[2], v[3]);
            }
        }
    }
    sat_report(amax, p.err_flag);
    __syncthreads();
    for (int q = tid; q < TM * 16 && !GTAV_DBG(p, 512); q += 512) {
        const int r = q >> 4, cc = q & 15, t = r >> 4, pl = r & 15;
        const uint4 val = *(const uint4*)(smem + r * PN + (((8 + cc) ^ (r & 7)) << 4));
        const size_t slot = ((size_t)b * p.Tmax + p.t0 + t) * p.S + 16 * pg + pl;
        f16* dst = p.k + slot * 2 * p.D + (cc >= 8 ? p.D : 0) + head * 64 + (cc & 7) * 8;
        if (p.out_sc1) store16q_sc1(dst, val);
        else *(uint4*)dst = val;
    }
    union H8 { f16x8 v; f16x2 h[4]; };
    if (tid < 3 * 128) {
        const int c = tid & 7, pl = (tid >> 3) & 15, grp = tid >> 7;
        H8 k8[TMAX], v8[TMAX];
        const int thi = TMAX - 1 - grp;
#pragma unroll
        for (int t = 0; t < TMAX; ++t) {
            if (t <= thi) {
                const int r = 16 * t + pl;
                k8[t].v = *(const f16x8*)(smem + r * PN + (((8 + c) ^ (r & 7)) << 4));
                v8[t].v = *(const f16x8*)(smem + r * PN + (((16 + c) ^ (r & 7)) << 4));
            }
        }
#pragma unroll
        for (int half = 0; half < 2; ++half) {
            const int tl = half == 0 ? thi : grp;
            if (half == 1 && grp == thi) break;
            H8 q8;
            {
                const int r = 16 * tl + pl;
                q8.v = *(const f16x8*)(smem + r * PN + ((c ^ (r & 7)) << 4));
            }
            float sc[TMAX];
            float mx = -INFINITY;
#pragma unroll
            for (int t = 0; t < TMAX; ++t) {
                sc[t] = -INFINITY;
                if (t <= tl) {
                    float dsum = 0.f;
#pragma unroll
                    for (int e = 0; e < 4; ++e) dsum = dot2acc(q8.h[e], k8[t].h[e], dsum, false);
                    sc[t] = group8_sum(dsum) * 0.125f;
                    mx = fmaxf(mx, sc[t]);
                }
            }
            float den = 0.f, o[8] = {0.f, 0.f, 0.f, 0.f, 0.f, 0.f, 0.f, 0.f};
#pragma unroll
            for (int t = 0; t < TMAX; ++t) {
                if (t <= tl) {
                    const float pr = __builtin_amdgcn_exp2f((sc[t] - mx) * 1.4426950408889634f);
                    den += pr;
#pragma unroll
                    for (int e = 0; e < 8; ++e) o[e] = __builtin_fmaf(pr, (float)v8[t].v[e], o[e]);
                }
            }
            const float inv = 1.0f / den;
            union { f16x8 h; u32x4 u; } o8;
#pragma unroll
            for (int e = 0; e < 8; ++e) o8.h[e] = (f16)(o[e] * inv);
            const int row = (b * p.Tq + tl) * p.S + 16 * pg + pl;
            store16_sc1((f16*)p.out + tiled_off(row, head * 64 + c * 8, p.D), o8.u);
        }
    }
    bs.template end<true>(p);
}


template <int NS>
__global__ __launch_bounds__(768, 1) void gemm_qkvs_attn_kernel(GemmParams p) {
    constexpr int FI = 3, FJ = 5, WN = 4, WM = 2, NL = 4, TNB = 192, TM = 144, NQT = TM / 16, NK = 10;
    constexpr int S_pad = 16 * NK, vstride = (S_pad + 8) * 2;
    constexpr int QS = 0, KS = TM * 128, VS = KS + S_pad * 128, IMG = VS + 64 * vstride;
    extern __shared__ __attribute__((aligned(16))) char smem_l[];
    static_assert(NS * (2 * FI * WN + 2 * FJ * WM) * 1024 >= IMG, "the ring must cover the epilogue's LDS image");
    static_assert(16 * FJ * WM >= TM && 16 * FJ * WM == S_pad, "two token halves cover the frame");
    char* smem = smem_l;
#define GTAV_PIN_S(x) asm volatile("" ::"s"(x))
    GTAV_PIN_S(p.X); GTAV_PIN_S(p.W); GTAV_PIN_S(p.M); GTAV_PIN_S(p.N); GTAV_PIN_S(p.K);
    GTAV_PIN_S(p.tm.tiles_m); GTAV_PIN_S(p.tm.tiles_n); GTAV_PIN_S(p.tm.gn); GTAV_PIN_S(p.tm.group); GTAV_PIN_S(p.tm.tiles);
    GTAV_PIN_S(p.tm.rcp_group); GTAV_PIN_S(p.tm.rcp_gn); GTAV_PIN_S(p.tm.rcp_gnlast);
#undef GTAV_PIN_S
    BlockStamps bs;
    bs.begin(p);
    int n0, m0, ks, kt0, nkt;
    tile_map_fast<false, TNB, TM>(p, n0, m0, ks, kt0, nkt);
    const int tid = threadIdx.x, lane = tid & 63, wraw = tid >> 6, w = wraw - NL, li = lane & 15, g = lane >> 4;
    const int wn = w & (WN - 1), wm = w >> 2;
    f32x4 acc[FI][FJ];
#pragma unroll
    for (int i = 0; i < FI; ++i)
#pragma unroll
        for (int j = 0; j < FJ; ++j) acc[i][j] = f32x4{0.f, 0.f, 0.f, 0.f};
    f32x4 cs[FJ];
    auto pf = [&]() {
#pragma unroll
        for (int j = 0; j < FJ; ++j) {
            const int pos = 16 * (FJ * wm + j) + li;
            cs[j] = *(const f32x4*)(p.rope_cs + (pos < TM ? pos : TM - 1) * 64 + 16 * wn + 4 * g);
        }
    };
    mainloop_l<false, NS, FI, FJ, WN, WM, NL, 2, true>(p, smem, n0, m0, kt0, nkt, acc, bs, pf);
    GTAV_STAMP(bs.t[2]);
    const int head = n0 / TNB, frame = m0 / TM;
    float amax = 0.f;
    __syncthreads();
    if (w >= 0) {
        const int d = 16 * wn + 4 * g;
#pragma unroll
        for (int j = 0; j < FJ; ++j) {
            const int jj = FJ * wm + j;
            if (jj < NQT) {
                const int ml = 16 * jj + li;
                const int off = ml * 128 + (((d >> 3) ^ (ml & 7)) << 4) + ((d >> 2) & 1) * 8;
// ... 768 lines not shown
```

### ai-generated-gtav_amd/csrc/ops.h

```cpp
#pragma once
#include "common.h"
#include "gemm.h"
#include "struct_layout.h"

namespace gtav {

int launch_skinny_f32(const float* X, int ldx, const float* W, const float* bias, float* Y, int ldy, int M, int N,
                      int K, int act_silu, hipStream_t stream);
int skinny_init();

struct StepParams {
    int first;
    int cur;
    int t_ctx;
    int t_cur;
    int is_final;
    float alpha_t, alpha_next;
    int cond_step;
};
int launch_step_setup(StepParams* dst, const StepParams& v, int* frame_idx, int* mod_rows, int* last_rows, int* changed, int B, int Tq, int T, int F,
                      int use_cur, hipStream_t stream);
int launch_gather_rows(const float* table, const int* rows, const int* changed, float* cur, int slots, int W, const float* table2, float* cur2, int W2,
                       hipStream_t stream);
int launch_ctab_inputs(const float* mod, int MODW, int R, int Rp, int D, const int* col, const int* is_scale, int n_groups, f16* sx, size_t group_stride,
                       hipStream_t stream);
int launch_cond_inputs_frame(int rows, int B, int T, int F, int start, int cur, int t_ctx, const int* t_steps, const float* sincos,
                             float* E, const float* actions, int A, float* HC, int ldhc, int D, int Apad, int* err_flag,
                             hipStream_t stream);

struct LnPending {
    const float* parts;
    int nsplit;
    size_t slab_stride;
    int ld;
    const float* bias;
    const float* gate;
    int gate_stride;
    const int* gate_rows;
    int rows_per_gate;
    int flags;
    int* err_flag;
    float* x_out;
    f16* y_save;
    int tperm_T, tperm_P;
};

int launch_ln_modulate(float* x, int ldx, f16* out, int ldo, int M, int D, const float* shift, const float* scale,
                       int mod_stride, const int* rows, int rows_per_mod, const LnPending* pend, int* err_flag, hipStream_t stream);
int launch_ln_affine(float* x, int ldx, f16* out, int ldo, int M, int D, const float* gamma, const float* beta,
                     const LnPending* pend, int* err_flag, hipStream_t stream);

int launch_patchify(const float* img, const int* frame_index, int NB, int C, int H, int W, int p, f16* out, int ldo,
                    float a, float b, int* err_flag, hipStream_t stream);
int launch_unpatchify(const float* y, int ldy, float* img, int NB, int C, int H, int W, int p, int order, float a,
                      float b, hipStream_t stream);

int launch_convert_pad_f16(const float* src, int lds, int R, int C, f16* dst, int Rp, int Cp, float scale, int tiled,
                           hipStream_t stream, int* err_flag = nullptr);
int launch_unpad_f16_to_f32(const f16* src, int lds, int R, int C, float* dst, int tiled, hipStream_t stream);
int launch_copy_f32_strided(const float* src, int lds, int R, int C, float* dst, int ldd, hipStream_t stream);
int launch_copy_rows_f32(const float* src, size_t src_stride, float* dst, size_t dst_stride, int rows, size_t n, hipStream_t stream);
int launch_clamp_cols(float* buf, int M, int ld, int c0, int c1, float lo, float hi, hipStream_t stream);
int launch_frames_to_u8(const float* img, uint8_t* out, int N, int H, int W, hipStream_t stream);
int launch_moments_to_latents(const float* mom, float* lat, int N, int hw, int latent, int mom_ch, float scale, hipStream_t stream);
int launch_latents_to_tokens(const float* lat, float* z, int N, int hw, int latent, hipStream_t stream);
int launch_resize_aa(const void* src, int src_is_u8_strip, float* dst, int n, int H, int W, int OH, int OW, hipStream_t stream);
int launch_copy_f32(const float* src, int lds, int R, int C, float* dst, int ldd, int c0, hipStream_t stream);
int launch_qkv_head_major(const f16* src, f16* dst, int D, hipStream_t stream, int mode = 0);
int launch_fill_f32(float* dst, size_t n, float v, hipStream_t stream);
int launch_rope_interleave(const float* cos_t, const float* sin_t, float* cs, int npos, hipStream_t stream);
int launch_add_f32(const float* a, const float* b, float* out, size_t n, hipStream_t stream);
int launch_calib_spin(unsigned long long ticks, unsigned long long* dev_ticks, hipStream_t stream);
int launch_axpy_f32(float* y, const float* x, float alpha, size_t n, hipStream_t stream);

int launch_cond_inputs(const int64_t* t64, int rows, int Tq, const StepParams* sp, int use_cur, const float* sincos ,
                       float* E, const float* actions, int64_t act_outer, int64_t act_inner, int A, float* HC, int ldhc,
                       int D, int Apad, int* err_flag, hipStream_t stream);

int launch_ddim_update(const float* x, size_t x_stride, const float* v, size_t v_stride, float* out, size_t out_stride,
                       int B, int n, const float* alpha_t, const float* alpha_next, int is_final, hipStream_t stream);
int launch_ddim_update_step(float* x, size_t frames_per_sample, const float* v, size_t v_stride, int B, int n,
                            const StepParams* sp, hipStream_t stream);

int launch_add_noise(const float* x, const float* noise, const float* alpha , float* out, int rows, int n,
                     float clamp_abs, hipStream_t stream);
int launch_vtarget(const float* x, const float* noise, const float* alpha , float* vt, int rows, int n,
                   float clamp_abs, hipStream_t stream);
int launch_mse(const float* a, size_t a_stride, const float* b, size_t b_stride, int rows, int n, float* out_scalar,
               hipStream_t stream);

int launch_transpose_tiled_f16(const f16* src, int R, int C, f16* dst, hipStream_t stream);
int launch_convert_T_f16(const float* src, int lds, int R, int C, f16* dst, hipStream_t stream);
int launch_gelu_tiled(const f16* u, f16* h, size_t n, hipStream_t stream);
int launch_gelu_bwd_tiled(const f16* dh, const f16* u, f16* du, size_t n, int* err_flag, hipStream_t stream);
int launch_ln_mod_bwd(const float* dxn, const float* x, const float* scale, int mod_stride, int rows_per_mod, int M, int D, float* dres, int accumulate,
                      float* stats, hipStream_t stream);
int launch_frame_reduce_ln(const float* dxn, const float* x, const float* stats, int frames, int P, int D, float* dshift, float* dscale, int mod_stride,
                           hipStream_t stream);
int launch_gelu_bwd_tiled_colsum(const f16* dh, const f16* u, f16* du, int M, int N, float* db, float* ws, int* err_flag, hipStream_t stream);
int gelu_bwd_colsum_splits(int M);
int launch_colsum_reduce_multi(const float* const* ws, float* const* db, const int* splits, const int* N, int njobs, hipStream_t stream);
bool ln_bwd_fused_ok(int D);
size_t ln_bwd_fused_workspace(int frames, int P, int D);
int launch_ln_mod_bwd_fused(const float* dxn, const float* x, const float* scale, int mod_stride, int frames, int P, int D, float* dres, int accumulate,
                            float* dshift, float* dscale, float* part, hipStream_t stream);
int launch_gate_bwd(const float* dres, const float* gate, int mod_stride, int rows_per_mod, int M, int D, f16* dy_tiled, int* err_flag, hipStream_t stream);
int launch_frame_reduce_gate(const float* dres, const f16* y, int frames, int P, int D, float* dgate, int mod_stride, hipStream_t stream);
int launch_gate_bwd_fused(const float* dres, const f16* y, const float* gate, int mod_stride, int frames, int P, int D, f16* dy_tiled, float* dgate, float* db,
                          float* ws, int* err_flag, hipStream_t stream);
size_t colsum_workspace(int M, int N);
int launch_colsum_tiled_f16(const f16* dy, int M, int N, float* db, float* ws, hipStream_t stream);
int launch_colsum_f32(const float* a, int lda, int M, int N, float* db, float* ws, hipStream_t stream);
int launch_to_tiled_f16(const float* a, int M, int D, f16* out, int* err_flag, hipStream_t stream);
int launch_mse_bwd_patch(const float* vpred, const float* vtarget, int B, int T, int C, int H, int W, int p, float scale, f16* dfo, int ldf, int* err_flag,
                         hipStream_t stream);
int launch_attn_spatial_bwd(const f16* Q, const f16* K, const f16* Vt, const f16* dO, int NB, int heads, int S, int D, const float* rope_cs, f16* dqkv,
                            int* err_flag, hipStream_t stream);
int launch_attn_temporal_bwd(const f16* q, const f16* kv, const f16* dO, int B, int P, int D, int T, int Tmax, const float* rope_cs, f16* dqkv, int* err_flag,
                             hipStream_t stream);
int launch_silu(const float* x, int ldx, float* y, int ldy, int R, int C, hipStream_t stream);
int launch_silu_bwd(const float* dy, int lddy, const float* x, int ldx, float* dx, int lddx, int R, int C, hipStream_t stream);
int launch_gemm_tn_f32(const float* dY, int lddy, const float* X, int ldx, int R, int N, int K, float* dW, int lddw, hipStream_t stream);
int launch_gemm_nn_f32(const float* dY, int lddy, const float* W, int ldw, int R, int N, int K, float* dX, int lddx, hipStream_t stream);
size_t ada_bwd_dx_workspace(int MODW, int D, int R);
int launch_ada_bwd_dx(const float* dmod, int MODW, const float* W, int D, int R, float* dSc, float* part, hipStream_t stream);
struct AdamParam {
    float* p; int ldp, R, C;
    const float* g; float *m, *v;
    f16* w16; int Cp16;
    f16* wT; int RpT;
};
struct AdamItem { int param; unsigned start; };
int launch_adamw_multi(const AdamParam* params, const AdamItem* items, int n_items, const float* ctl, float lr, float beta1, float beta2, float eps, float wd,
                       hipStream_t stream);
int sumsq_parts(size_t n);
int launch_sumsq(const float* g, size_t n, float* part, hipStream_t stream);
int launch_overflow_publish(const int* err_flag, float* g, hipStream_t stream);
int launch_err_clear(int* err_flag, int bits, hipStream_t stream);
int launch_clip_coef(float* ctl, const float* part, int nparts, float inv_scale, float max_norm, float beta1, float beta2, int* err_flag, hipStream_t stream);
int launch_adamw(float* p, int ldp, int R, int C, const float* g, float* m, float* v, const float* ctl, float lr, float beta1, float beta2, float eps,
                 float wd, hipStream_t stream);

int launch_attn_spatial(const f16* Q, const f16* K, const f16* Vt, f16* O, int NB, int heads, int S, hipStream_t stream, bool q_prescaled = false);
bool attn_spatial_wants_prescaled_q(int S);
constexpr float kAttnQScale = 0.125f * 1.4426950408889634f;
int launch_attn_temporal(const f16* q, const f16* kv, f16* O, int B, int P, int D, int Tq, int t0, int Tmax,
                         hipStream_t stream);

GTAV_LAYOUT_ASSERT(GemmParams)
GTAV_LAYOUT_ASSERT(LnPending)
GTAV_LAYOUT_ASSERT(GemmDwGroup)
GTAV_LAYOUT_ASSERT(AdamParam)
GTAV_LAYOUT_ASSERT(AdamItem)

}
```

### ai-generated-gtav_amd/csrc/ops_bf16.h

```cpp
#pragma once
#include "ops.h"

namespace gtav_bf16 {
struct GemmParams;
struct LnPending;
int launch_gemm(const GemmParams& p, int epi, hipStream_t stream);
int launch_ln_modulate(float* x, int ldx, __bf16* out, int ldo, int M, int D, const float* shift, const float* scale, int mod_stride, const int* rows,
                       int rows_per_mod, const LnPending* pend, int* err_flag, hipStream_t stream);
int launch_ln_affine(float* x, int ldx, __bf16* out, int ldo, int M, int D, const float* gamma, const float* beta, const LnPending* pend, int* err_flag,
                     hipStream_t stream);
int launch_patchify(const float* img, const int* frame_index, int NB, int C, int H, int W, int p, __bf16* out, int ldo, float a, float b, int* err_flag,
                    hipStream_t stream);
int launch_convert_pad_f16(const float* src, int lds, int R, int C, __bf16* dst, int Rp, int Cp, float scale, int tiled, hipStream_t stream, int* err_flag);
int launch_unpad_f16_to_f32(const __bf16* src, int lds, int R, int C, float* dst, int tiled, hipStream_t stream);
int launch_attn_spatial(const __bf16* Q, const __bf16* K, const __bf16* Vt, __bf16* O, int NB, int heads, int S, hipStream_t stream, bool q_prescaled);
int launch_attn_temporal(const __bf16* q, const __bf16* kv, __bf16* O, int B, int P, int D, int Tq, int t0, int Tmax, hipStream_t stream);
struct GemmDwGroup;
struct AdamParam;
struct AdamItem;
int launch_gemm_tn(const GemmParams& p, hipStream_t stream);
int launch_gemm_dw_grouped(const GemmDwGroup* g, int n, int K, int* err_flag, hipStream_t stream, bool tn);
int launch_transpose_tiled_f16(const __bf16* src, int R, int C, __bf16* dst, hipStream_t stream);
int launch_convert_T_f16(const float* src, int lds, int R, int C, __bf16* dst, hipStream_t stream);
int launch_gelu_tiled(const __bf16* u, __bf16* h, size_t n, hipStream_t stream);
int launch_gelu_bwd_tiled(const __bf16* dh, const __bf16* u, __bf16* du, size_t n, int* err_flag, hipStream_t stream);
int launch_gelu_bwd_tiled_colsum(const __bf16* dh, const __bf16* u, __bf16* du, int M, int N, float* db, float* ws, int* err_flag, hipStream_t stream);
int launch_gate_bwd(const float* dres, const float* gate, int mod_stride, int rows_per_mod, int M, int D, __bf16* dy_tiled, int* err_flag, hipStream_t stream);
int launch_frame_reduce_gate(const float* dres, const __bf16* y, int frames, int P, int D, float* dgate, int mod_stride, hipStream_t stream);
int launch_gate_bwd_fused(const float* dres, const __bf16* y, const float* gate, int mod_stride, int frames, int P, int D, __bf16* dy_tiled, float* dgate,
                          float* db, float* ws, int* err_flag, hipStream_t stream);
int launch_colsum_tiled_f16(const __bf16* dy, int M, int N, float* db, float* ws, hipStream_t stream);
int launch_to_tiled_f16(const float* a, int M, int D, __bf16* out, int* err_flag, hipStream_t stream);
int launch_mse_bwd_patch(const float* vpred, const float* vtarget, int B, int T, int C, int H, int W, int p, float scale, __bf16* dfo, int ldf, int* err_flag,
                         hipStream_t stream);
int launch_attn_spatial_bwd(const __bf16* Q, const __bf16* K, const __bf16* Vt, const __bf16* dO, int NB, int heads, int S, int D, const float* rope_cs,
                            __bf16* dqkv, int* err_flag, hipStream_t stream);
int launch_attn_temporal_bwd(const __bf16* q, const __bf16* kv, const __bf16* dO, int B, int P, int D, int T, int Tmax, const float* rope_cs, __bf16* dqkv,
                             int* err_flag, hipStream_t stream);
int launch_adamw_multi(const AdamParam* params, const AdamItem* items, int n_items, const float* ctl, float lr, float beta1, float beta2, float eps, float wd,
                       hipStream_t stream);
void set_error(const char* fmt, ...);
const char* last_error();
}

namespace gtav {

struct OperandOps {
    int (*gemm)(const GemmParams& p, int epi, hipStream_t stream);
    int (*ln_modulate)(float* x, int ldx, f16* out, int ldo, int M, int D, const float* shift, const float* scale, int mod_stride, const int* rows, int rows_per_mod,
                       const LnPending* pend, int* err_flag, hipStream_t stream);
    int (*ln_affine)(float* x, int ldx, f16* out, int ldo, int M, int D, const float* gamma, const float* beta, const LnPending* pend, int* err_flag, hipStream_t stream);
    int (*patchify)(const float* img, const int* frame_index, int NB, int C, int H, int W, int p, f16* out, int ldo, float a, float b, int* err_flag, hipStream_t stream);
    int (*convert_pad)(const float* src, int lds, int R, int C, f16* dst, int Rp, int Cp, float scale, int tiled, hipStream_t stream, int* err_flag);
    int (*unpad)(const f16* src, int lds, int R, int C, float* dst, int tiled, hipStream_t stream);
    int (*attn_spatial)(const f16* Q, const f16* K, const f16* Vt, f16* O, int NB, int heads, int S, hipStream_t stream, bool q_prescaled);
    int (*attn_temporal)(const f16* q, const f16* kv, f16* O, int B, int P, int D, int Tq, int t0, int Tmax, hipStream_t stream);
    bool bf16;
};
const OperandOps& operand_ops(bool bf16);

struct TrainOps {
    int (*gemm_tn)(const GemmParams& p, hipStream_t stream);
    int (*gemm_dw_grouped)(const GemmDwGroup* g, int n, int K, int* err_flag, hipStream_t stream, bool tn);
    int (*transpose_tiled)(const f16* src, int R, int C, f16* dst, hipStream_t stream);
    int (*convert_T)(const float* src, int lds, int R, int C, f16* dst, hipStream_t stream);
    int (*gelu_tiled)(const f16* u, f16* h, size_t n, hipStream_t stream);
    int (*gelu_bwd_tiled)(const f16* dh, const f16* u, f16* du, size_t n, int* err_flag, hipStream_t stream);
    int (*gelu_bwd_tiled_colsum)(const f16* dh, const f16* u, f16* du, int M, int N, float* db, float* ws, int* err_flag, hipStream_t stream);
    int (*gate_bwd)(const float* dres, const float* gate, int mod_stride, int rows_per_mod, int M, int D, f16* dy_tiled, int* err_flag, hipStream_t stream);
    int (*frame_reduce_gate)(const float* dres, const f16* y, int frames, int P, int D, float* dgate, int mod_stride, hipStream_t stream);
    int (*gate_bwd_fused)(const float* dres, const f16* y, const float* gate, int mod_stride, int frames, int P, int D, f16* dy_tiled, float* dgate, float* db,
                          float* ws, int* err_flag, hipStream_t stream);
    int (*colsum_tiled)(const f16* dy, int M, int N, float* db, float* ws, hipStream_t stream);
    int (*to_tiled)(const float* a, int M, int D, f16* out, int* err_flag, hipStream_t stream);
    int (*mse_bwd_patch)(const float* vpred, const float* vtarget, int B, int T, int C, int H, int W, int p, float scale, f16* dfo, int ldf, int* err_flag,
                         hipStream_t stream);
    int (*attn_spatial_bwd)(const f16* Q, const f16* K, const f16* Vt, const f16* dO, int NB, int heads, int S, int D, const float* rope_cs, f16* dqkv,
                            int* err_flag, hipStream_t stream);
    int (*attn_temporal_bwd)(const f16* q, const f16* kv, const f16* dO, int B, int P, int D, int T, int Tmax, const float* rope_cs, f16* dqkv, int* err_flag,
                             hipStream_t stream);
    int (*adamw_multi)(const AdamParam* params, const AdamItem* items, int n_items, const float* ctl, float lr, float beta1, float beta2, float eps, float wd,
                       hipStream_t stream);
    bool bf16;
};
const TrainOps& train_ops(bool bf16);

}
```

### ai-generated-gtav_amd/csrc/struct_layout.h

```cpp
#pragma once
#include <cstddef>

#define GTAV_LAYOUT_GemmParams_SIZE 352
#define GTAV_LAYOUT_GemmParams(F) \
    F(X, 0) F(ldx, 8) F(W, 16) F(M, 24) F(N, 28) F(K, 32) F(debug, 36) F(stamps, 40) F(err_flag, 48) F(out_sc1, 56) F(splitk, 60) F(bias, 64) \
    F(out2, 72) F(out, 80) F(ldo, 88) F(gate, 96) F(gate_stride, 104) F(gate_rows, 112) F(rows_per_gate, 120) F(qkv_mode, 124) F(q, 128) F(k, 136) \
    F(v, 144) F(D, 152) F(S, 156) F(Tq, 160) F(t0, 164) F(Tmax, 168) F(rope_cs, 176) F(rope_cs_q, 184) F(tm, 192) F(f_P, 228) F(f_rows, 232) \
    F(f_stats, 240) F(f_nslot, 248) F(f_c1, 256) F(f_c2, 264) F(f_ldc, 272) F(f_stats_out, 280) F(f_scale, 288) F(f_a, 296) F(pf, 304) F(sk_ws, 328) \
    F(sk_flags, 336) F(sk_dp, 344) F(sk_r, 348)
#define GTAV_LAYOUT_LnPending_SIZE 104
#define GTAV_LAYOUT_LnPending(F) \
    F(parts, 0) F(nsplit, 8) F(slab_stride, 16) F(ld, 24) F(bias, 32) F(gate, 40) F(gate_stride, 48) F(gate_rows, 56) F(rows_per_gate, 64) \
    F(flags, 68) F(err_flag, 72) F(x_out, 80) F(y_save, 88) F(tperm_T, 96) F(tperm_P, 100)
#define GTAV_LAYOUT_GemmDwGroup_SIZE 40
#define GTAV_LAYOUT_GemmDwGroup(F) \
    F(X, 0) F(W, 8) F(out, 16) F(M, 24) F(N, 28) F(ldo, 32)
#define GTAV_LAYOUT_AdamParam_SIZE 80
#define GTAV_LAYOUT_AdamParam(F) \
    F(p, 0) F(ldp, 8) F(R, 12) F(C, 16) F(g, 24) F(m, 32) F(v, 40) F(w16, 48) F(Cp16, 56) F(wT, 64) F(RpT, 72)
#define GTAV_LAYOUT_AdamItem_SIZE 8
#define GTAV_LAYOUT_AdamItem(F) \
    F(param, 0) F(start, 4)

#define GTAV_LAYOUT_ASSERT_FIELD_(S, f, off) static_assert(offsetof(S, f) == (off), #S "::" #f " is not at the offset its twin expects (struct_layout.h)");
#define GTAV_LAYOUT_FIELD_GemmParams(f, off) GTAV_LAYOUT_ASSERT_FIELD_(GemmParams, f, off)
#define GTAV_LAYOUT_FIELD_LnPending(f, off) GTAV_LAYOUT_ASSERT_FIELD_(LnPending, f, off)
#define GTAV_LAYOUT_FIELD_GemmDwGroup(f, off) GTAV_LAYOUT_ASSERT_FIELD_(GemmDwGroup, f, off)
#define GTAV_LAYOUT_FIELD_AdamParam(f, off) GTAV_LAYOUT_ASSERT_FIELD_(AdamParam, f, off)
#define GTAV_LAYOUT_FIELD_AdamItem(f, off) GTAV_LAYOUT_ASSERT_FIELD_(AdamItem, f, off)
#define GTAV_LAYOUT_ASSERT(S)                                                                                                      \
    static_assert(sizeof(S) == GTAV_LAYOUT_##S##_SIZE, "sizeof(" #S ") differs from the size its twin expects (struct_layout.h)"); \
    GTAV_LAYOUT_##S(GTAV_LAYOUT_FIELD_##S)
```

Measured before the change: 5.039.

## Fuse step head/tail kernels and compute only last-frame rows in final block

Adds a fused head kernel that does patchify, patch-embed GEMM and the first LayerNorm-modulate in one launch. It also adds a fused tail kernel that does the final LN, the final projection, unpatchify and the DDIM update in one launch. In addition, when several frames are processed, the last transformer block's attention output, out-projection, MLP and final head are restricted to the last frame's rows, since only the last frame's velocity is consumed. This removes several launches and intermediate buffers, and skips work on rows whose outputs are discarded. The cost is new custom kernels and extra geometry and route conditions, with a risk to correctness on edge paths.

```diff
diff --git a/ai-generated-gtav_amd/csrc/api.hip b/ai-generated-gtav_amd/csrc/api.hip
--- a/ai-generated-gtav_amd/csrc/api.hip
+++ b/ai-generated-gtav_amd/csrc/api.hip
@@ -46,8 +46,8 @@
 int bf_attn_spatial(const f16* Q, const f16* K, const f16* Vt, f16* O, int NB, int heads, int S, hipStream_t st, bool qp) {
     return gtav_bf16::launch_attn_spatial((const __bf16*)Q, (const __bf16*)K, (const __bf16*)Vt, (__bf16*)O, NB, heads, S, st, qp);
 }
-int bf_attn_temporal(const f16* q, const f16* kv, f16* O, int B, int P, int D, int Tq, int t0, int Tmax, hipStream_t st) {
-    return gtav_bf16::launch_attn_temporal((const __bf16*)q, (const __bf16*)kv, (__bf16*)O, B, P, D, Tq, t0, Tmax, st);
+int bf_attn_temporal(const f16* q, const f16* kv, f16* O, int B, int P, int D, int Tq, int t0, int Tmax, hipStream_t st, int live_last) {
+    return gtav_bf16::launch_attn_temporal((const __bf16*)q, (const __bf16*)kv, (__bf16*)O, B, P, D, Tq, t0, Tmax, st, live_last);
 }
 const OperandOps OPS_F16 = {launch_gemm, launch_ln_modulate, launch_ln_affine, launch_patchify, f16_convert_pad, launch_unpad_f16_to_f32, f16_attn_spatial,
                             launch_attn_temporal, false};
@@ -233,7 +233,7 @@
 }
 int gtav_op_attn_temporal_bf16(const void* q, const void* kv, void* o, int32_t B, int32_t P, int32_t D, int32_t Tq, int32_t t0,
                                int32_t Tmax, void* stream) {
-    return gtav_bf16::launch_attn_temporal((const __bf16*)q, (const __bf16*)kv, (__bf16*)o, B, P, D, Tq, t0, Tmax, (hipStream_t)stream);
+    return gtav_bf16::launch_attn_temporal((const __bf16*)q, (const __bf16*)kv, (__bf16*)o, B, P, D, Tq, t0, Tmax, (hipStream_t)stream, 0);
 }
 int gtav_op_qkv_head_major(const void* w, void* w_hm, int32_t D, void* stream) {
     return launch_qkv_head_major((const f16*)w, (f16*)w_hm, D, (hipStream_t)stream);
diff --git a/ai-generated-gtav_amd/csrc/api_dit.hip b/ai-generated-gtav_amd/csrc/api_dit.hip
--- a/ai-generated-gtav_amd/csrc/api_dit.hip
+++ b/ai-generated-gtav_amd/csrc/api_dit.hip
@@ -91,12 +91,22 @@
     return dit_fold_tables(h, rows, fa, fb, s);
 }
 
+struct StepTail { float* x; int F; float* v_last; bool fused; };
+
 static int dit_forward_core(gtav_dit* h, const float* x_src, const int* frame_index, int B, int Tq, int t0,
-                            const float* mod, const int* mod_rows, const float* ctab, float* v_out, hipStream_t s) {
+                            const float* mod, const int* mod_rows, const float* ctab, float* v_out, hipStream_t s, StepTail* st = nullptr) {
     const int D = h->D, P = h->P, NB = B * Tq, M = NB * P;
     GTAV_REQUIRE(M <= h->Mmax, "forward: %d tokens exceed workspace (%d)", M, h->Mmax);
     bool fold_a, fold_b;
     fold_policy(h, M, fold_a, fold_b);
+    const int g_embed = 2 * h->L, g_final = 2 * h->L + 1;
+    const bool head_fused = !h->tr.on && !h->ops(g_embed).bf16 && !h->ops(0).bf16 && step_head_ok(D, h->Kpe);
+    const bool tail_fused = !h->tr.on && !fold_b && !h->ops(g_final).bf16 && step_tail_ok(D, h->Nfin, nullptr);
+    const int hb_last = 2 * h->L - 1, Ml = B * P;
+    auto slab_route = [&](int Mx, int K) {
+        return !(gemm_pp_ok(Mx, D, K, EPI_RESID) || (gemm_choose_splitk(Mx, D, K) == 1 && Mx >= h->resid_inplace_min_m) || gemm_resid_inplace_ok(Mx, D, K, P));
+    };
+    const bool live = st && Tq > 1 && tail_fused && !fold_a && !h->ops(hb_last).bf16 && slab_route(Ml, D) && slab_route(Ml, h->Hm_pad);
     const gtav_dit::Fold& fo = h->fold;
     auto fold_consumer = [&](GemmParams& q, int seam, int N) {
         q.bias = nullptr;
@@ -112,12 +122,16 @@
         PROF(h, cls, s, launch_gemm(q, EPI_RESID_FOLD, s));
         return 0;
     };
-    const int g_embed = 2 * h->L, g_final = 2 * h->L + 1;
-    PROF(h, PC_OTHER, s, h->ops(g_embed).patchify(x_src, frame_index, NB, h->C, h->H, h->W, h->p, h->xp, h->Kpe, 1.f, 0.f, h->err_of(g_embed), s));
     GemmParams g;
-    memset(&g, 0, sizeof(g));
-    g.X = h->xp; g.ldx = h->Kpe; g.W = h->w_pe; g.M = M; g.N = D; g.K = h->Kpe; g.bias = h->b_pe; g.out = h->resid; g.ldo = D;
-    PROF(h, PC_OTHER, s, h->ops(g_embed).gemm(g, EPI_F32, s));
+    if (head_fused) {
+        PROF(h, PC_OTHER, s, launch_step_head(x_src, frame_index, NB, h->C, h->H, h->W, h->p, h->w_pe, h->b_pe, h->Kpe, h->resid, h->xn, D, mod, mod + D, h->MODW,
+                                              mod_rows, h->err_of(g_embed), h->err_of(0), s));
+    } else {
+        PROF(h, PC_OTHER, s, h->ops(g_embed).patchify(x_src, frame_index, NB, h->C, h->H, h->W, h->p, h->xp, h->Kpe, 1.f, 0.f, h->err_of(g_embed), s));
+        memset(&g, 0, sizeof(g));
+        g.X = h->xp; g.ldx = h->Kpe; g.W = h->w_pe; g.M = M; g.N = D; g.K = h->Kpe; g.bias = h->b_pe; g.out = h->resid; g.ldo = D;
+        PROF(h, PC_OTHER, s, h->ops(g_embed).gemm(g, EPI_F32, s));
+    }
     LnPending pend;
     bool have_pend = false;
     const int pf_max_m = 1536;
@@ -133,9 +147,10 @@
                                 ((hb2 & 1) ? h->fuse_tattn && gemm_qkvt_attn_ok(M, D, P, Tq, t0) : h->fuse_sattn && fused_spatial_ok(M, D, P));
             return PfNext{fused2 ? w2.w_qkv_hm : w2.w_qkv, 3 * D, D, 1, 3};
         }
-        if (p2 == 1) return PfNext{w2.w_out, D, D, gemm_choose_splitk(M, D, D), 0};
+        const int M2 = live && hb2 == hb_last ? Ml : M;
+        if (p2 == 1) return PfNext{w2.w_out, D, D, gemm_choose_splitk(M2, D, D), 0};
         if (p2 == 2) return PfNext{w2.w_fc1, h->Hm, D, 1, 1};
-        return PfNext{w2.w_fc2, D, h->Hm_pad, gemm_choose_splitk(M, D, h->Hm_pad), 2};
+        return PfNext{w2.w_fc2, D, h->Hm_pad, gemm_choose_splitk(M2, D, h->Hm_pad), 2};
     };
     auto set_pf = [&](GemmParams& q, const PfNext& t) {
         const int v = h->w_prefetch_cls[t.consumer];
@@ -145,13 +160,14 @@
         if (skn < 1 || nkt % skn || (skn >= 8 ? skn % 8 : 8 % skn)) skn = 1;
         q.pf = PrefetchDesc{t.W, cdiv(t.N, 128), nkt, skn, v >= 2 ? v : 0};
     };
-    auto resid_gemm = [&](const OperandOps& ops, int cls, const f16* X, int ldx, const f16* Wt, int K, const float* bias, const float* gate, const PfNext& pfn) -> int {
+    auto resid_gemm = [&](const OperandOps& ops, int cls, const f16* X, int ldx, const f16* Wt, int K, const float* bias, const float* gate, const PfNext& pfn, bool lv) -> int {
+        const int M = lv ? Ml : NB * P;
         GemmParams q;
         memset(&q, 0, sizeof(q));
         q.X = X; q.ldx = ldx; q.W = Wt; q.M = M; q.N = D; q.K = K; q.out = h->parts; q.ldo = D;
         set_pf(q, pfn);
         q.splitk = gemm_choose_splitk(M, D, K);
-        if (gemm_pp_ok(M, D, K, EPI_RESID) || (q.splitk == 1 && M >= h->resid_inplace_min_m) || gemm_resid_inplace_ok(M, D, K, P)) {
+        if (!slab_route(M, K)) {
             q.splitk = 0; q.out = h->resid; q.bias = bias; q.gate = gate; q.gate_stride = h->MODW; q.gate_rows = mod_rows;
             q.rows_per_gate = P;
             PROF(h, cls, s, ops.gemm(q, EPI_RESID, s));
@@ -163,6 +179,7 @@
         memset(&pend, 0, sizeof(pend));
         pend.parts = h->parts; pend.nsplit = q.splitk; pend.slab_stride = (size_t)M * D; pend.ld = D; pend.bias = bias;
         pend.gate = gate; pend.gate_stride = h->MODW; pend.gate_rows = mod_rows; pend.rows_per_gate = P;
+        if (lv) { pend.live_T = Tq; pend.live_P = P; }
         have_pend = true;
         return 0;
     };
@@ -179,7 +196,8 @@
                 if (!have_pend) memset(&pend, 0, sizeof(pend));
                 pend.tperm_T = Tq; pend.tperm_P = P;
             }
-            if (!folded_in)
+            const bool lv = live && hb == hb_last;
+            if (!folded_in && !(hb == 0 && head_fused))
                 PROF(h, PC_LN, s, ops.ln_modulate(h->resid, D, h->xn, D, M, D, mb, mb + D, h->MODW, mod_rows, P, (have_pend || fused_t) ? &pend : nullptr, ef, s));
             have_pend = false;
             memset(&g, 0, sizeof(g));
@@ -189,7 +207,7 @@
             const bool fused_s = hf == 0 && h->fuse_sattn && !h->tr.on && !ops.bf16 && !folded_in && w.w_qkv_hm && fused_spatial_ok(M, D, P);
             if (fused_t) {
                 g.W = w.w_qkv_hm; g.qkv_mode = QKV_TEMPORAL; g.k = h->kvcache[l]; g.v = h->kvcache[l]; g.out = h->ao; g.ldo = D;
-                g.Tq = Tq; g.t0 = t0; g.Tmax = h->maxT; g.rope_cs = h->rope_t.cs_dev;
+                g.Tq = Tq; g.t0 = t0; g.Tmax = h->maxT; g.rope_cs = h->rope_t.cs_dev; g.live_rows = lv;
                 PROF(h, PC_ATTN_T, s, launch_gemm_qkvt_attn(g, s));
             } else if (fused_s) {
                 g.W = w.w_qkv_hm; g.qkv_mode = QKV_SPATIAL; g.out = h->ao; g.ldo = D; g.rope_cs = h->rope_s.cs_dev;
@@ -205,19 +223,19 @@
                 }
                 PROF(h, PC_QKV, s, ops.gemm(g, folded_in ? EPI_QKV_FOLD : EPI_QKV, s));
                 if (hf == 0) PROF(h, PC_ATTN_S, s, ops.attn_spatial(h->qs, h->ks, h->vts, h->ao, NB, h->heads, P, s, false));
-                else PROF(h, PC_ATTN_T, s, ops.attn_temporal(h->qt, h->kvcache[l], h->ao, B, P, D, Tq, t0, h->maxT, s));
+                else PROF(h, PC_ATTN_T, s, ops.attn_temporal(h->qt, h->kvcache[l], h->ao, B, P, D, Tq, t0, h->maxT, s, lv));
             }
             folded_in = false;
             memset(&g, 0, sizeof(g));
-            g.X = h->xn; g.ldx = D; g.W = w.w_fc1; g.M = M; g.N = h->Hm; g.K = D; g.bias = w.b_fc1; g.out = h->hbuf; g.ldo = h->Hm_pad; g.err_flag = ef;
+            g.X = h->xn; g.ldx = D; g.W = w.w_fc1; g.M = lv ? Ml : M; g.N = h->Hm; g.K = D; g.bias = w.b_fc1; g.out = h->hbuf; g.ldo = h->Hm_pad; g.err_flag = ef;
             set_pf(g, pf_target(hb, 2));
             if (fold_a) {
                 RET_IF(fold_producer(PC_OUT, h->ao, w.w_out, D, w.b_out, mb + 2 * D, mb + 4 * D));
                 fold_consumer(g, 2 * hb + 1, h->Hm);
                 PROF(h, PC_FC1, s, launch_gemm(g, EPI_GELU_TANH_FOLD, s));
             } else {
-                RET_IF(resid_gemm(ops, PC_OUT, h->ao, D, w.w_out, D, w.b_out, mb + 2 * D, pf_target(hb, 1)));
-                PROF(h, PC_LN, s, ops.ln_modulate(h->resid, D, h->xn, D, M, D, mb + 3 * D, mb + 4 * D, h->MODW, mod_rows, P, have_pend ? &pend : nullptr, ef, s));
+                RET_IF(resid_gemm(ops, PC_OUT, h->ao, D, w.w_out, D, w.b_out, mb + 2 * D, pf_target(hb, 1), lv));
+                PROF(h, PC_LN, s, ops.ln_modulate(h->resid, D, h->xn, D, lv ? Ml : M, D, mb + 3 * D, mb + 4 * D, h->MODW, mod_rows, P, have_pend ? &pend : nullptr, ef, s));
                 have_pend = false;
                 PROF(h, PC_FC1, s, ops.gemm(g, EPI_GELU_TANH, s));
             }
@@ -226,18 +244,26 @@
                 RET_IF(fold_producer(PC_FC2, h->hbuf, w.w_fc2, h->Hm_pad, w.b_fc2, mb + 5 * D, next_scale));
                 folded_in = true;
             } else {
-                RET_IF(resid_gemm(ops, PC_FC2, h->hbuf, h->Hm_pad, w.w_fc2, h->Hm_pad, w.b_fc2, mb + 5 * D, pf_target(hb, 3)));
+                RET_IF(resid_gemm(ops, PC_FC2, h->hbuf, h->Hm_pad, w.w_fc2, h->Hm_pad, w.b_fc2, mb + 5 * D, pf_target(hb, 3), lv));
             }
         }
     }
     const float* mf = mod + (size_t)h->L * 12 * D;
-    if (!folded_in)
-        PROF(h, PC_LN, s, h->ops(g_final).ln_modulate(h->resid, D, h->xn, D, M, D, mf, mf + D, h->MODW, mod_rows, P, have_pend ? &pend : nullptr, h->err_of(g_final), s));
-    memset(&g, 0, sizeof(g));
-    g.X = h->xn; g.ldx = D; g.W = h->w_final; g.M = M; g.N = h->Nfin; g.K = D; g.bias = h->b_final; g.out = h->fo; g.ldo = h->Nfin;
-    if (folded_in) fold_consumer(g, 4 * h->L, h->Nfin);
-    PROF(h, PC_OTHER, s, h->ops(g_final).gemm(g, folded_in ? EPI_F32_FOLD : EPI_F32, s));
-    PROF(h, PC_OTHER, s, launch_unpatchify(h->fo, h->Nfin, v_out, NB, h->C, h->H, h->W, h->p, 0, 1.f, 0.f, s));
+    if (tail_fused) {
+        GTAV_REQUIRE(!folded_in && step_tail_ok(D, h->Nfin, have_pend ? &pend : nullptr), "forward: the tail launch cannot take this pending update");
+        PROF(h, PC_OTHER, s, launch_step_tail(h->resid, live ? Ml : M, D, P, have_pend ? &pend : nullptr, mf, mf + D, h->MODW, mod_rows, h->w_final, h->b_final, h->Nfin,
+                                              v_out, h->C, h->H, h->W, h->p, h->err_of(g_final), st ? st->x : nullptr, st ? st->F : 0, Tq, h->step_dev,
+                                              st ? st->v_last : nullptr, s));
+        if (st) st->fused = true;
+    } else {
+        if (!folded_in)
+            PROF(h, PC_LN, s, h->ops(g_final).ln_modulate(h->resid, D, h->xn, D, M, D, mf, mf + D, h->MODW, mod_rows, P, have_pend ? &pend : nullptr, h->err_of(g_final), s));
+        memset(&g, 0, sizeof(g));
+        g.X = h->xn; g.ldx = D; g.W = h->w_final; g.M = M; g.N = h->Nfin; g.K = D; g.bias = h->b_final; g.out = h->fo; g.ldo = h->Nfin;
+        if (folded_in) fold_consumer(g, 4 * h->L, h->Nfin);
+        PROF(h, PC_OTHER, s, h->ops(g_final).gemm(g, folded_in ? EPI_F32_FOLD : EPI_F32, s));
+        PROF(h, PC_OTHER, s, launch_unpatchify(h->fo, h->Nfin, v_out, NB, h->C, h->H, h->W, h->p, 0, 1.f, 0.f, s));
+    }
     PROF(h, PC_EMPTY, s, 0);
     return h->prof.collect(s);
 }
@@ -450,7 +476,9 @@
     const size_t fsz = (size_t)h->C * h->H * h->W;
     const int Tq = mode == 1 ? 1 : T, t0 = mode == 1 ? T - 1 : 0;
     if (!prepared) RET_IF(dit_cond(h, nullptr, B * Tq, Tq, h->step_dev, mode == 1, actions, (int64_t)F * h->A, h->A, s));
-    RET_IF(dit_forward_core(h, x, h->frame_idx, B, Tq, t0, prepared ? h->mod_cur : h->mod, nullptr, prepared ? h->fold.ctab_cur : h->fold.ctab, h->vout, s));
+    StepTail st{x, F, v_out, false};
+    RET_IF(dit_forward_core(h, x, h->frame_idx, B, Tq, t0, prepared ? h->mod_cur : h->mod, nullptr, prepared ? h->fold.ctab_cur : h->fold.ctab, h->vout, s, &st));
+    if (st.fused) return 0;
     const float* vlast = h->vout + (size_t)(Tq - 1) * fsz;
     RET_IF(launch_ddim_update_step(x, F, vlast, (size_t)Tq * fsz, B, (int)fsz, h->step_dev, s));
     if (v_out) RET_IF(launch_copy_rows_f32(vlast, (size_t)Tq * fsz, v_out, fsz, B, fsz, s));
diff --git a/ai-generated-gtav_amd/csrc/api_train.hip b/ai-generated-gtav_amd/csrc/api_train.hip
--- a/ai-generated-gtav_amd/csrc/api_train.hip
+++ b/ai-generated-gtav_amd/csrc/api_train.hip
@@ -237,7 +237,7 @@
             else { g.qkv_mode = QKV_TEMPORAL; g.q = b.q; g.k = b.k; g.v = b.k; g.Tq = T; g.t0 = 0; g.Tmax = h->maxT; g.rope_cs = h->rope_t.cs_dev; }
             RET_IF(o.gemm(g, EPI_QKV, s));
             if (hf == 0) RET_IF(o.attn_spatial(b.q, b.k, b.v, b.ao, NB, h->heads, P, s, false));
-            else RET_IF(o.attn_temporal(b.q, b.k, b.ao, B, P, D, T, 0, h->maxT, s));
+            else RET_IF(o.attn_temporal(b.q, b.k, b.ao, B, P, D, T, 0, h->maxT, s, 0));
             RET_IF(resid_gemm(o, b.ao, w.w_out, D, w.b_out, mb + 2 * D, tr.res[2 * i + 1], b.y1));
             RET_IF(o.ln_modulate(tr.res[2 * i], D, b.xnB, D, M, D, mb + 3 * D, mb + 4 * D, h->MODW, nullptr, P, &pend, h->err_flag, s));
             have_pend = false;
diff --git a/ai-generated-gtav_amd/csrc/attention.hip b/ai-generated-gtav_amd/csrc/attention.hip
--- a/ai-generated-gtav_amd/csrc/attention.hip
+++ b/ai-generated-gtav_amd/csrc/attention.hip
@@ -325,7 +325,7 @@
 template <int TM>
 __global__ __launch_bounds__(256) void attn_temporal_kernel(const f16* __restrict__ q, const f16* __restrict__ kv,
                                                             f16* __restrict__ O, int ncol, int P, int D, int Tq, int t0, int Tmax,
-                                                            int split) {
+                                                            int split, int qT, int qt0) {
     const int tpc = D >> 3;
     const int ci = threadIdx.x / tpc, lc = threadIdx.x - ci * tpc;
     const int bp = blockIdx.x * ((int)blockDim.x / tpc) + ci;
@@ -347,7 +347,7 @@
     H8 qall[TM];
 #pragma unroll
     for (int tl = 0; tl < TM; ++tl)
-        if (tl >= tl_lo && tl < tl_hi) qall[tl].v = *(const f16x8*)(q + (((size_t)b * Tq + tl) * P + p) * D + c);
+        if (tl >= tl_lo && tl < tl_hi) qall[tl].v = *(const f16x8*)(q + (((size_t)b * qT + qt0 + tl) * P + p) * D + c);
 #pragma unroll
     for (int tl = 0; tl < TM; ++tl) {
         if (tl >= tl_hi) break;
@@ -387,7 +387,7 @@
 
 template <int QG, int FB>
 __global__ __launch_bounds__(256) void attn_temporal_stream_kernel(const f16* __restrict__ q, const f16* __restrict__ kv,
-                                                                   f16* __restrict__ O, int ncol, int P, int D, int Tq, int t0, int Tmax) {
+                                                                   f16* __restrict__ O, int ncol, int P, int D, int Tq, int t0, int Tmax, int qT, int qt0) {
 #pragma clang fp contract(off)
     const int tpc = D >> 3;
     const int ci = threadIdx.x / tpc, lc = threadIdx.x - ci * tpc;
@@ -404,7 +404,7 @@
 #pragma unroll
     for (int j = 0; j < QG; ++j) {
         qv[j].v = f16x8{};
-        if (j < nq) qv[j].v = *(const f16x8*)(q + (((size_t)b * Tq + tl0 + j) * P + p) * D + c);
+        if (j < nq) qv[j].v = *(const f16x8*)(q + (((size_t)b * qT + qt0 + tl0 + j) * P + p) * D + c);
         m[j] = -INFINITY; den[j] = 0.f;
 #pragma unroll
         for (int e = 0; e < 8; ++e) acc[j][e] = 0.f;
@@ -560,17 +560,19 @@
 }
 
 int launch_attn_temporal(const f16* q, const f16* kv, f16* O, int B, int P, int D, int Tq, int t0, int Tmax,
-                         hipStream_t stream) {
+                         hipStream_t stream, int live_last) {
     GTAV_REQUIRE(D % 256 == 0 && D <= 2048, "attn_temporal: D=%d must be a multiple of 256 and <= 2048", D);
     GTAV_REQUIRE(Tq > 0 && t0 >= 0 && t0 + Tq <= Tmax && Tmax <= 32, "attn_temporal: window t0=%d Tq=%d Tmax=%d (max 32)", t0, Tq, Tmax);
+    const int qT = Tq, qt0 = live_last ? Tq - 1 : 0;
+    if (live_last) { t0 += Tq - 1; Tq = 1; }
     GTAV_REQUIRE(P > 0 && B > 0 && (long long)B * Tq * P < (1ll << 31), "attn_temporal: B=%d P=%d Tq=%d", B, P, Tq);
     const int tpc = D / 8, cpb = tpc >= 256 ? 1 : 256 / tpc;
     const int Tvis = t0 + Tq;
     if (Tvis > 8) {
         if (Tq == 1) {
-            GTAV_LAUNCH((attn_temporal_stream_kernel<1, 8>), dim3(cdiv(B * P, cpb), 1), dim3(tpc * cpb), 0, stream, q, kv, O, B * P, P, D, Tq, t0, Tmax);
+            GTAV_LAUNCH((attn_temporal_stream_kernel<1, 8>), dim3(cdiv(B * P, cpb), 1), dim3(tpc * cpb), 0, stream, q, kv, O, B * P, P, D, Tq, t0, Tmax, qT, qt0);
         } else {
-            GTAV_LAUNCH((attn_temporal_stream_kernel<8, 4>), dim3(cdiv(B * P, cpb), cdiv(Tq, 8)), dim3(tpc * cpb), 0, stream, q, kv, O, B * P, P, D, Tq, t0, Tmax);
+            GTAV_LAUNCH((attn_temporal_stream_kernel<8, 4>), dim3(cdiv(B * P, cpb), cdiv(Tq, 8)), dim3(tpc * cpb), 0, stream, q, kv, O, B * P, P, D, Tq, t0, Tmax, qT, qt0);
         }
         GTAV_CHECK_HIP(hipGetLastError());
         return 0;
@@ -578,8 +580,8 @@
     static const int split_max = GTAV_ENV_INT("GTAV_ATTN_T_SPLIT_MAX", 1024);
     const int split = (Tq > 1 && B * P < split_max) ? 1 : 0;
     const dim3 grid(cdiv(B * P, cpb), split ? Tq : 1), block(tpc * cpb);
-    if (Tvis <= 5) GTAV_LAUNCH(attn_temporal_kernel<5>, grid, block, 0, stream, q, kv, O, B * P, P, D, Tq, t0, Tmax, split);
-    else GTAV_LAUNCH(attn_temporal_kernel<8>, grid, block, 0, stream, q, kv, O, B * P, P, D, Tq, t0, Tmax, split);
+    if (Tvis <= 5) GTAV_LAUNCH(attn_temporal_kernel<5>, grid, block, 0, stream, q, kv, O, B * P, P, D, Tq, t0, Tmax, split, qT, qt0);
+    else GTAV_LAUNCH(attn_temporal_kernel<8>, grid, block, 0, stream, q, kv, O, B * P, P, D, Tq, t0, Tmax, split, qT, qt0);
     GTAV_CHECK_HIP(hipGetLastError());
     return 0;
 }
diff --git a/ai-generated-gtav_amd/csrc/common.h b/ai-generated-gtav_amd/csrc/common.h
--- a/ai-generated-gtav_amd/csrc/common.h
+++ b/ai-generated-gtav_amd/csrc/common.h
@@ -183,6 +183,13 @@
     return __builtin_elementwise_fma(t, f32x2_{1.0f, 1.0f} - s, s);
 }
 
+__device__ __forceinline__ float ddim_one(float xc, float vp, float at, float an, int is_final) {
+    const float x0 = sqrtf(at) * xc - sqrtf(1.0f - at) * vp;
+    if (is_final) return x0;
+    const float eps = (sqrtf(1.0f / at) * xc - x0) / sqrtf(1.0f / at - 1.0f);
+    return sqrtf(an) * x0 + sqrtf(1.0f - an) * eps;
+}
+
 __device__ __forceinline__ float gelu_erf_f(float x) { return 0.5f * x * (1.0f + erff(x * 0.7071067811865476f)); }
 
 constexpr float kGeluErfL = 4.5f;
diff --git a/ai-generated-gtav_amd/csrc/elementwise.hip b/ai-generated-gtav_amd/csrc/elementwise.hip
--- a/ai-generated-gtav_amd/csrc/elementwise.hip
+++ b/ai-generated-gtav_amd/csrc/elementwise.hip
@@ -71,7 +71,7 @@
 #else
 #define LN_DBG(pd, b) false
 #endif
-template <int MODE, bool PEND>
+template <int MODE, bool PEND, bool LIVE = false>
 __global__ __launch_bounds__(512) void ln_row_block_kernel(float* __restrict__ x, int ldx, f16* __restrict__ out, int M, int D,
                                                            const float* __restrict__ p0, const float* __restrict__ p1,
                                                            int mod_stride, const int* __restrict__ rows, int rows_per_mod,
@@ -80,7 +80,8 @@
     const int m = blockIdx.x;
     const int c = threadIdx.x * 4;
     const int nw = (blockDim.x + 63) >> 6, wid = threadIdx.x >> 6, lane = threadIdx.x & 63;
-    float* xr = x + (size_t)m * ldx;
+    const int mr = LIVE ? (m / pd.live_P) * pd.live_T * pd.live_P + (pd.live_T - 1) * pd.live_P + m % pd.live_P : m;
+    float* xr = x + (size_t)mr * ldx;
     const bool act = c < D;
     const bool nt = PEND && (pd.flags & 4);
     f32x4 v = f32x4{0.f, 0.f, 0.f, 0.f}, av = v, bv = v;
@@ -109,11 +110,11 @@
     }
     int row = 0, gr = 0;
     if (MODE == 0) {
-        row = m / rows_per_mod;
+        row = mr / rows_per_mod;
         if (rows && !LN_DBG(pd, 0x2000)) row = rows[row];
     }
     if (PEND && pd.gate) {
-        gr = m / pd.rows_per_gate;
+        gr = mr / pd.rows_per_gate;
         if (pd.gate_rows && !LN_DBG(pd, 0x2000)) gr = pd.gate_rows[gr];
     }
     const float kshift = LN_DBG(pd, 0x200) ? 0.f : xr[0];
@@ -141,7 +142,7 @@
     if (lane == 0) { red[wid] = s1; red[8 + wid] = s2; }
     if (!LN_DBG(pd, 0x400)) __syncthreads();
     if (PEND && act) {
-        float* xw = pd.x_out ? pd.x_out + (size_t)m * ldx + c : xr + c;
+        float* xw = pd.x_out ? pd.x_out + (size_t)mr * ldx + c : xr + c;
         if (LN_DBG(pd, 0x800)) {}
         else if (pd.flags & 1) store16_sc1(xw, v);
         else *(f32x4*)xw = v;
@@ -397,13 +398,6 @@
     for (int j = threadIdx.x; j < 256; j += blockDim.x) E[(size_t)r * 256 + j] = sincos[(size_t)t * 256 + j];
     const float* arow = actions ? actions + ro * act_outer + (frame0 + ri) * act_inner : nullptr;
     for (int j = threadIdx.x; j < Apad; j += blockDim.x) HC[(size_t)r * ldhc + D + j] = (arow && j < A) ? arow[j] : 0.f;
-}
-
-__device__ __forceinline__ float ddim_one(float xc, float vp, float at, float an, int is_final) {
-    const float x0 = sqrtf(at) * xc - sqrtf(1.0f - at) * vp;
-    if (is_final) return x0;
-    const float eps = (sqrtf(1.0f / at) * xc - x0) / sqrtf(1.0f / at - 1.0f);
-    return sqrtf(an) * x0 + sqrtf(1.0f - an) * eps;
 }
 
 __global__ void ddim_update_kernel(const float* __restrict__ x, size_t x_stride, const float* __restrict__ v, size_t v_stride,
@@ -623,6 +617,7 @@
         pd_.err_flag = err_flag;                                                                          \
         GTAV_REQUIRE(pd_.tperm_T == 0 || (pd_.tperm_P % 16 == 0 && M % (pd_.tperm_T * pd_.tperm_P) == 0), "ln: bad output row permutation"); \
         const bool upd_ = pend && pend->parts;    \
+        GTAV_REQUIRE(pd_.live_T == 0 || (upd_ && pd_.live_P > 0 && M % pd_.live_P == 0 && pd_.tperm_T == 0 && !pd_.x_out && !pd_.y_save), "ln: bad live-row map"); \
         if (!upd_ && pd_.tperm_T == 0 && M >= g_ln_wave_row_min && (D == 256 || D == 512 || D == 1024 || D == 2048)) { \
             if (D == 256) LN_WAVE_ROW_(MODE, 1, P0, P1, STRIDE, ROWS, RPM);                               \
             else if (D == 512) LN_WAVE_ROW_(MODE, 2, P0, P1, STRIDE, ROWS, RPM);                          \
@@ -630,7 +625,8 @@
             else LN_WAVE_ROW_(MODE, 8, P0, P1, STRIDE, ROWS, RPM);                                        \
         } else {                                                                   \
             const dim3 g_(M), b_(round_up(D / 4, 64));                                                    \
-            if (upd_) GTAV_LAUNCH((ln_row_block_kernel<MODE, true>), g_, b_, 0, stream, x, ldx, out, M, D, P0, P1, STRIDE, ROWS, RPM, pd_); \
+            if (upd_ && pd_.live_T > 0) GTAV_LAUNCH((ln_row_block_kernel<MODE, true, true>), g_, b_, 0, stream, x, ldx, out, M, D, P0, P1, STRIDE, ROWS, RPM, pd_); \
+            else if (upd_) GTAV_LAUNCH((ln_row_block_kernel<MODE, true>), g_, b_, 0, stream, x, ldx, out, M, D, P0, P1, STRIDE, ROWS, RPM, pd_); \
             else GTAV_LAUNCH((ln_row_block_kernel<MODE, false>), g_, b_, 0, stream, x, ldx, out, M, D, P0, P1, STRIDE, ROWS, RPM, pd_);     \
         }                                                                                                 \
     } while (0)
diff --git a/ai-generated-gtav_amd/csrc/gemm.h b/ai-generated-gtav_amd/csrc/gemm.h
--- a/ai-generated-gtav_amd/csrc/gemm.h
+++ b/ai-generated-gtav_amd/csrc/gemm.h
@@ -28,6 +28,7 @@
 struct GemmParams {
     const f16* X;
     int ldx;
+    int live_rows;
     const f16* W;
     int M, N, K;
     int debug;
diff --git a/ai-generated-gtav_amd/csrc/gemm.hip b/ai-generated-gtav_amd/csrc/gemm.hip
--- a/ai-generated-gtav_amd/csrc/gemm.hip
+++ b/ai-generated-gtav_amd/csrc/gemm.hip
@@ -2208,6 +2208,7 @@
         for (int half = 0; half < 2; ++half) {
             const int tl = half == 0 ? thi : grp;
             if (half == 1 && grp == thi) break;
+            if (p.live_rows && tl != p.Tq - 1) continue;
             H8 q8;
             {
                 const int r = 16 * tl + pl;
@@ -2240,7 +2241,7 @@
             union { f16x8 h; u32x4 u; } o8;
 #pragma unroll
             for (int e = 0; e < 8; ++e) o8.h[e] = (f16)(o[e] * inv);
-            const int row = (b * p.Tq + tl) * p.S + 16 * pg + pl;
+            const int row = p.live_rows ? b * p.S + 16 * pg + pl : (b * p.Tq + tl) * p.S + 16 * pg + pl;
             store16_sc1((f16*)p.out + tiled_off(row, head * 64 + c * 8, p.D), o8.u);
         }
     }
diff --git a/ai-generated-gtav_amd/csrc/ops.h b/ai-generated-gtav_amd/csrc/ops.h
--- a/ai-generated-gtav_amd/csrc/ops.h
+++ b/ai-generated-gtav_amd/csrc/ops.h
@@ -43,6 +43,7 @@
     float* x_out;
     f16* y_save;
     int tperm_T, tperm_P;
+    int live_T, live_P;
 };
 
 int launch_ln_modulate(float* x, int ldx, f16* out, int ldo, int M, int D, const float* shift, const float* scale,
@@ -88,6 +89,14 @@
                    float clamp_abs, hipStream_t stream);
 int launch_mse(const float* a, size_t a_stride, const float* b, size_t b_stride, int rows, int n, float* out_scalar,
                hipStream_t stream);
+
+bool step_head_ok(int D, int Kpe);
+int launch_step_head(const float* img, const int* frame_index, int NB, int C, int H, int W, int p, const f16* w_pe, const float* b_pe, int Kpe, float* resid, f16* xn,
+                     int D, const float* shift, const float* scale, int mod_stride, const int* mod_rows, int* err_in, int* err_ln, hipStream_t stream);
+bool step_tail_ok(int D, int Nfin, const LnPending* pend);
+int launch_step_tail(const float* x, int M, int D, int P, const LnPending* pend, const float* shift, const float* scale, int mod_stride, const int* mod_rows,
+                     const f16* w_fin, const float* b_fin, int Nfin, float* vout, int C, int H, int W, int p, int* err_ln, float* ddim_x, int F, int Tq,
+                     const StepParams* sp, float* v_last, hipStream_t stream);
 
 int launch_transpose_tiled_f16(const f16* src, int R, int C, f16* dst, hipStream_t stream);
 int launch_convert_T_f16(const float* src, int lds, int R, int C, f16* dst, hipStream_t stream);
@@ -145,7 +154,7 @@
 bool attn_spatial_wants_prescaled_q(int S);
 constexpr float kAttnQScale = 0.125f * 1.4426950408889634f;
 int launch_attn_temporal(const f16* q, const f16* kv, f16* O, int B, int P, int D, int Tq, int t0, int Tmax,
-                         hipStream_t stream);
+                         hipStream_t stream, int live_last = 0);
 
 GTAV_LAYOUT_ASSERT(GemmParams)
 GTAV_LAYOUT_ASSERT(LnPending)
diff --git a/ai-generated-gtav_amd/csrc/ops_bf16.h b/ai-generated-gtav_amd/csrc/ops_bf16.h
--- a/ai-generated-gtav_amd/csrc/ops_bf16.h
+++ b/ai-generated-gtav_amd/csrc/ops_bf16.h
@@ -14,7 +14,7 @@
 int launch_convert_pad_f16(const float* src, int lds, int R, int C, __bf16* dst, int Rp, int Cp, float scale, int tiled, hipStream_t stream, int* err_flag);
 int launch_unpad_f16_to_f32(const __bf16* src, int lds, int R, int C, float* dst, int tiled, hipStream_t stream);
 int launch_attn_spatial(const __bf16* Q, const __bf16* K, const __bf16* Vt, __bf16* O, int NB, int heads, int S, hipStream_t stream, bool q_prescaled);
-int launch_attn_temporal(const __bf16* q, const __bf16* kv, __bf16* O, int B, int P, int D, int Tq, int t0, int Tmax, hipStream_t stream);
+int launch_attn_temporal(const __bf16* q, const __bf16* kv, __bf16* O, int B, int P, int D, int Tq, int t0, int Tmax, hipStream_t stream, int live_last);
 struct GemmDwGroup;
 struct AdamParam;
 struct AdamItem;
@@ -54,7 +54,7 @@
     int (*convert_pad)(const float* src, int lds, int R, int C, f16* dst, int Rp, int Cp, float scale, int tiled, hipStream_t stream, int* err_flag);
     int (*unpad)(const f16* src, int lds, int R, int C, float* dst, int tiled, hipStream_t stream);
     int (*attn_spatial)(const f16* Q, const f16* K, const f16* Vt, f16* O, int NB, int heads, int S, hipStream_t stream, bool q_prescaled);
-    int (*attn_temporal)(const f16* q, const f16* kv, f16* O, int B, int P, int D, int Tq, int t0, int Tmax, hipStream_t stream);
+    int (*attn_temporal)(const f16* q, const f16* kv, f16* O, int B, int P, int D, int Tq, int t0, int Tmax, hipStream_t stream, int live_last);
     bool bf16;
 };
 const OperandOps& operand_ops(bool bf16);
diff --git a/ai-generated-gtav_amd/csrc/step_edges.hip b/ai-generated-gtav_amd/csrc/step_edges.hip
--- /dev/null
+++ b/ai-generated-gtav_amd/csrc/step_edges.hip
@@ -0,0 +1,350 @@
+#include "ops.h"
+
+#include <cstring>
+
+namespace gtav {
+
+namespace {
+
+constexpr int ER = 16;
+constexpr int ET = 1024;
+
+__device__ __forceinline__ int xs_off(int r, int k) { return (k >> 6) * (ER * 64) + r * 64 + ((((k >> 3) & 7) ^ (r & 7)) << 3) + (k & 7); }
+
+struct HeadArgs {
+    const float* img; const int* frame_index;
+    int C, H, W, p, P, M, D, Kpe;
+    const f16* w_pe; const float* b_pe;
+    float* resid; f16* xn;
+    const float *shift, *scale; int mod_stride; const int* mod_rows;
+    int *err_in, *err_ln;
+};
+
+template <int NT>
+__global__ __launch_bounds__(ET) void step_head_kernel(HeadArgs a) {
+    extern __shared__ __attribute__((aligned(16))) char smem[];
+    f16* xs = (f16*)smem;
+    float2* red = (float2*)(smem + (size_t)a.Kpe * ER * 2);
+    const int tid = threadIdx.x, lane = tid & 63, li = lane & 15, g = lane >> 4;
+    const int w = __builtin_amdgcn_readfirstlane(tid >> 6);
+    const int m0 = blockIdx.x * ER;
+    const int m = m0 + li;
+    const bool valid = m < a.M;
+    auto wfrag = [&](int tile, int k) { return *(const f16x8*)(a.w_pe + tiled_off(tile * 16 + li, k, a.Kpe)); };
+    f16x8 wf0[2], wf[2][NT];
+#pragma unroll
+    for (int s = 0; s < 2; ++s) {
+        wf0[s] = wfrag(0, (4 * s + g) * 8);
+#pragma unroll
+        for (int i = 0; i < NT; ++i) wf[s][i] = wfrag(w * NT + i, (4 * s + g) * 8);
+    }
+    f32x4 bias[NT];
+#pragma unroll
+    for (int i = 0; i < NT; ++i) bias[i] = *(const f32x4*)(a.b_pe + (w * NT + i) * 16 + 4 * g);
+    const float bias0 = a.b_pe[0];
+    int row = (valid ? m : a.M - 1) / a.P;
+    if (a.mod_rows) row = a.mod_rows[row];
+    {
+        const int gw = a.W / a.p, pp = a.p * a.p, Kp = a.C * pp, mg = m0 + w;
+        const float* base = nullptr;
+        if (mg < a.M) {
+            const int nb = mg / a.P, t = mg - nb * a.P, y = t / gw, x = t - y * gw;
+            const int f = a.frame_index ? a.frame_index[nb] : nb;
+            base = a.img + ((size_t)f * a.C * a.H + (size_t)y * a.p) * a.W + x * a.p;
+        }
+        int flags = 0;
+        for (int k = lane; k < a.Kpe; k += 64) {
+            float val = 0.f;
+            if (base && k < Kp) {
+                const int c = k / pp, rem = k - c * pp, ph = rem / a.p, pw = rem - ph * a.p;
+                val = base[((size_t)c * a.H + ph) * a.W + pw];
+                if (!(__builtin_fabsf(val) <= F16_MAX)) {
+                    flags |= (val != val || __builtin_isinf(val)) ? ERR_NONFINITE : ERR_F16_SAT;
+                    if (val == val) val = __builtin_amdgcn_fmed3f(val, -F16_MAX, F16_MAX);
+                }
+            }
+            xs[xs_off(w, k)] = (f16)val;
+        }
+        if (flags && a.err_in) atomicOr(a.err_in, flags);
+    }
+    __syncthreads();
+    f32x4 acc[NT], acc0 = f32x4{0.f, 0.f, 0.f, 0.f};
+#pragma unroll
+    for (int i = 0; i < NT; ++i) acc[i] = f32x4{0.f, 0.f, 0.f, 0.f};
+    for (int kt = 0; kt < (a.Kpe >> 6); ++kt) {
+#pragma unroll
+        for (int s = 0; s < 2; ++s) {
+            const int k = kt * 64 + (4 * s + g) * 8;
+            const f16x8 xf = *(const f16x8*)(xs + xs_off(li, k));
+            const bool pre = kt == 0;
+            acc0 = mfma16(pre ? wf0[s] : wfrag(0, k), xf, acc0, 0, 0, 0);
+#pragma unroll
+            for (int i = 0; i < NT; ++i) acc[i] = mfma16(pre ? wf[s][i] : wfrag(w * NT + i, k), xf, acc[i], 0, 0, 0);
+        }
+    }
+    const float* sc = a.scale + (size_t)row * a.mod_stride;
+    const float* sh = a.shift + (size_t)row * a.mod_stride;
+    f32x4 av[NT], bv[NT];
+#pragma unroll
+    for (int i = 0; i < NT; ++i) {
+        const int n = (w * NT + i) * 16 + 4 * g;
+        av[i] = *(const f32x4*)(sc + n);
+        bv[i] = *(const f32x4*)(sh + n);
+    }
+    const float kshift = __shfl(acc0[0] + bias0, li, 64);
+    f32x4 v[NT];
+    float s1 = 0.f, s2 = 0.f;
+#pragma unroll
+    for (int i = 0; i < NT; ++i) {
+        const int n = (w * NT + i) * 16 + 4 * g;
+        v[i] = acc[i] + bias[i];
+        if (valid) *(f32x4*)(a.resid + (size_t)m * a.D + n) = v[i];
+        const float a0 = v[i][0] - kshift, a1 = v[i][1] - kshift, a2 = v[i][2] - kshift, a3 = v[i][3] - kshift;
+        s1 += (a0 + a1) + (a2 + a3);
+        s2 += (a0 * a0 + a1 * a1) + (a2 * a2 + a3 * a3);
+    }
+    s1 += __shfl_xor(s1, 16, 64); s2 += __shfl_xor(s2, 16, 64);
+    s1 += __shfl_xor(s1, 32, 64); s2 += __shfl_xor(s2, 32, 64);
+    if (g == 0) red[w * ER + li] = float2{s1, s2};
+    __syncthreads();
+    float t1 = 0.f, t2 = 0.f;
+#pragma unroll
+    for (int i = 0; i < ET / 64; ++i) { const float2 q = red[i * ER + li]; t1 += q.x; t2 += q.y; }
+    const float m1 = t1 / (float)a.D, mean = kshift + m1;
+    const float var = fmaxf(t2 / (float)a.D - m1 * m1, 0.f);
+    const float rstd = 1.0f / sqrtf(var + 1e-6f);
+    if (!valid) return;
+    float amax = 0.f;
+#pragma unroll
+    for (int i = 0; i < NT; ++i) {
+        const int n = (w * NT + i) * 16 + 4 * g;
+        float yv[4];
+#pragma unroll
+        for (int e = 0; e < 4; ++e) yv[e] = (v[i][e] - mean) * rstd * (1.0f + (av[i][e] + 1e-6f)) + bv[i][e];
+        *(f16x4*)(a.xn + tiled_off(m, n, a.D)) = sat4(yv[0], yv[1], yv[2], yv[3], amax);
+    }
+    sat_report(amax, a.err_ln);
+}
+
+struct TailArgs {
+    const float* x; int M, D, P;
+    LnPending pd;
+    const float *shift, *scale; int mod_stride; const int* mod_rows;
+    const f16* w_fin; const float* b_fin; int Nfin;
+    float* vout; int C, H, W, p;
+    float* ddim_x; int F, Tq; const StepParams* sp; float* v_last;
+};
+
+template <int NV>
+__global__ __launch_bounds__(ET) void step_tail_kernel(TailArgs a) {
+    extern __shared__ __attribute__((aligned(16))) char smem[];
+    f16* xs = (f16*)smem;
+    f32x4* red = (f32x4*)smem;
+    const int tid = threadIdx.x, lane = tid & 63, li = lane & 15, g = lane >> 4;
+    const int w = __builtin_amdgcn_readfirstlane(tid >> 6);
+    const int m0 = blockIdx.x * ER;
+    const LnPending& pd = a.pd;
+    const int tile = w & 3, kq = w >> 2;
+    auto resid_row = [&](int i) { return pd.live_T > 0 ? (i / pd.live_P) * pd.live_T * pd.live_P + (pd.live_T - 1) * pd.live_P + i % pd.live_P : i; };
+    const int ms = m0 + li, n0 = tile * 16 + 4 * g, fsz = a.C * a.H * a.W;
+    const bool scat = kq == 0 && ms < a.M && n0 < a.Nfin;
+    bool upd = false;
+    int offs[4] = {0, 0, 0, 0}, nbs = 0, fin = 0;
+    float xin[4] = {0.f, 0.f, 0.f, 0.f}, at = 0.f, an = 0.f;
+    f32x4 bfin = f32x4{0.f, 0.f, 0.f, 0.f};
+    float* xf = nullptr;
+    if (scat) {
+        bfin = *(const f32x4*)(a.b_fin + n0);
+        const int mr = resid_row(ms), gw = a.W / a.p;
+        nbs = mr / a.P;
+        const int t = mr - nbs * a.P, y = t / gw, x = t - y * gw;
+#pragma unroll
+        for (int e = 0; e < 4; ++e) {
+            const int n = n0 + e, c = n % a.C, q = n / a.C, pw = q % a.p, ph = q / a.p;
+            offs[e] = n < a.Nfin ? (c * a.H + (y * a.p + ph)) * a.W + (x * a.p + pw) : -1;
+        }
+        upd = a.ddim_x && nbs % a.Tq == a.Tq - 1;
+        if (upd) {
+            at = a.sp->alpha_t; an = a.sp->alpha_next; fin = a.sp->is_final;
+            xf = a.ddim_x + ((size_t)(nbs / a.Tq) * a.F + a.sp->cur) * fsz;
+#pragma unroll
+            for (int e = 0; e < 4; ++e)
+                if (offs[e] >= 0) xin[e] = xf[offs[e]];
+        }
+    }
+    auto wfrag = [&](int t, int s) { return *(const f16x8*)(a.w_fin + tiled_off(tile * 16 + li, (kq * NV + t) * 64 + (4 * s + g) * 8, a.D)); };
+    f16x8 wf[NV][2];
+    {
+        const int m = m0 + w;
+        f16x4 o[NV];
+#pragma unroll
+        for (int i = 0; i < NV; ++i) o[i] = f16x4{(f16)0.f, (f16)0.f, (f16)0.f, (f16)0.f};
+        if (m < a.M) {
+            const int mr = resid_row(m);
+            const float* xr = a.x + (size_t)mr * a.D;
+            f32x4 v[NV];
+#pragma unroll
+            for (int i = 0; i < NV; ++i) v[i] = *(const f32x4*)(xr + i * 256 + lane * 4);
+            int row = mr / a.P;
+            if (a.mod_rows) row = a.mod_rows[row];
+            if (pd.parts) {
+                constexpr int CH = 4;
+                const float* pp = pd.parts + (size_t)m * pd.ld;
+                f32x4 y[NV], g4[NV];
+#pragma unroll
+                for (int i = 0; i < NV; ++i) {
+                    y[i] = pd.bias ? *(const f32x4*)(pd.bias + i * 256 + lane * 4) : f32x4{0.f, 0.f, 0.f, 0.f};
+                    g4[i] = f32x4{1.f, 1.f, 1.f, 1.f};
+                }
+                if (pd.gate) {
+                    int gr = mr / pd.rows_per_gate;
+                    if (pd.gate_rows) gr = pd.gate_rows[gr];
+                    const float* gp = pd.gate + (size_t)gr * pd.gate_stride;
+#pragma unroll
+                    for (int i = 0; i < NV; ++i) g4[i] = *(const f32x4*)(gp + i * 256 + lane * 4);
+                }
+                for (int s0 = 0; s0 < pd.nsplit; s0 += CH) {
+                    f32x4 sl[CH][NV];
+#pragma unroll
+                    for (int c = 0; c < CH; ++c) {
+                        const float* q = pp + (size_t)(s0 + c < pd.nsplit ? s0 + c : 0) * pd.slab_stride;
+#pragma unroll
+                        for (int i = 0; i < NV; ++i) sl[c][i] = __builtin_nontemporal_load((const f32x4*)(q + i * 256 + lane * 4));
+                    }
+#pragma unroll
+                    for (int c = 0; c < CH; ++c)
+                        if (s0 + c < pd.nsplit) {
+#pragma unroll
+                            for (int i = 0; i < NV; ++i) y[i] = y[i] + sl[c][i];
+                        }
+                }
+#pragma unroll
+                for (int i = 0; i < NV; ++i) v[i] = v[i] + (pd.gate ? y[i] * g4[i] : y[i]);
+            }
+#pragma unroll
+            for (int t = 0; t < NV; ++t)
+#pragma unroll
+                for (int s = 0; s < 2; ++s) wf[t][s] = wfrag(t, s);
+            const float* sc = a.scale + (size_t)row * a.mod_stride;
+            const float* sh = a.shift + (size_t)row * a.mod_stride;
+            f32x4 av[NV], bv[NV];
+#pragma unroll
+            for (int i = 0; i < NV; ++i) {
+                av[i] = *(const f32x4*)(sc + i * 256 + lane * 4);
+                bv[i] = *(const f32x4*)(sh + i * 256 + lane * 4);
+            }
+            const float kshift = __builtin_bit_cast(float, __builtin_amdgcn_readfirstlane(__builtin_bit_cast(int, v[0][0])));
+            float s1 = 0.f, s2 = 0.f;
+#pragma unroll
+            for (int i = 0; i < NV; ++i) {
+                const float a0 = v[i][0] - kshift, a1 = v[i][1] - kshift, a2 = v[i][2] - kshift, a3 = v[i][3] - kshift;
+                s1 += (a0 + a1) + (a2 + a3);
+                s2 += (a0 * a0 + a1 * a1) + (a2 * a2 + a3 * a3);
+            }
+            const float t1 = wave_sum_dpp(s1), t2 = wave_sum_dpp(s2);
+            const float m1 = t1 / (float)a.D, mean = kshift + m1;
+            const float var = fmaxf(t2 / (float)a.D - m1 * m1, 0.f);
+            const float rstd = 1.0f / sqrtf(var + 1e-6f);
+            float amax = 0.f;
+#pragma unroll
+            for (int i = 0; i < NV; ++i) {
+                float yv[4];
+#pragma unroll
+                for (int e = 0; e < 4; ++e) yv[e] = (v[i][e] - mean) * rstd * (1.0f + (av[i][e] + 1e-6f)) + bv[i][e];
+                o[i] = sat4(yv[0], yv[1], yv[2], yv[3], amax);
+            }
+            sat_report(amax, pd.err_flag);
+        } else {
+#pragma unroll
+            for (int t = 0; t < NV; ++t)
+#pragma unroll
+                for (int s = 0; s < 2; ++s) wf[t][s] = wfrag(t, s);
+        }
+#pragma unroll
+        for (int i = 0; i < NV; ++i) *(f16x4*)(xs + xs_off(w, i * 256 + lane * 4)) = o[i];
+    }
+    __syncthreads();
+    f32x4 acc = f32x4{0.f, 0.f, 0.f, 0.f};
+#pragma unroll
+    for (int t = 0; t < NV; ++t) {
+#pragma unroll
+        for (int s = 0; s < 2; ++s) {
+            const int k = (kq * NV + t) * 64 + (4 * s + g) * 8;
+            acc = mfma16(wf[t][s], *(const f16x8*)(xs + xs_off(li, k)), acc, 0, 0, 0);
+        }
+    }
+    __syncthreads();
+    if (kq > 0) red[((kq - 1) * 4 + tile) * 64 + lane] = acc;
+    __syncthreads();
+    if (!scat) return;
+    acc = ((acc + red[tile * 64 + lane]) + red[(4 + tile) * 64 + lane]) + red[(8 + tile) * 64 + lane];
+    const f32x4 val = acc + bfin;
+    float* vl = upd && a.v_last ? a.v_last + (size_t)(nbs / a.Tq) * fsz : nullptr;
+#pragma unroll
+    for (int e = 0; e < 4; ++e) {
+        if (offs[e] < 0) break;
+        a.vout[(size_t)nbs * fsz + offs[e]] = val[e];
+        if (upd) {
+            xf[offs[e]] = ddim_one(xin[e], val[e], at, an, fin);
+            if (vl) vl[offs[e]] = val[e];
+        }
+    }
+}
+
+}
+
+bool step_head_ok(int D, int Kpe) { return D % 256 == 0 && D >= 256 && D <= 1024 && Kpe % 64 == 0 && Kpe >= 64 && Kpe <= 1024; }
+
+int launch_step_head(const float* img, const int* frame_index, int NB, int C, int H, int W, int p, const f16* w_pe, const float* b_pe, int Kpe, float* resid, f16* xn,
+                     int D, const float* shift, const float* scale, int mod_stride, const int* mod_rows, int* err_in, int* err_ln, hipStream_t stream) {
+    GTAV_REQUIRE(step_head_ok(D, Kpe) && H % p == 0 && W % p == 0 && Kpe >= C * p * p, "step_head: bad geometry (D=%d, Kpe=%d)", D, Kpe);
+    HeadArgs a;
+    a.img = img; a.frame_index = frame_index; a.C = C; a.H = H; a.W = W; a.p = p; a.P = (H / p) * (W / p); a.M = NB * a.P; a.D = D; a.Kpe = Kpe;
+    a.w_pe = w_pe; a.b_pe = b_pe; a.resid = resid; a.xn = xn; a.shift = shift; a.scale = scale; a.mod_stride = mod_stride; a.mod_rows = mod_rows;
+    a.err_in = err_in; a.err_ln = err_ln;
+    const dim3 grid(cdiv(a.M, ER)), block(ET);
+    const size_t lds = (size_t)Kpe * ER * 2 + (ET / 64) * ER * sizeof(float2);
+    switch (D / 256) {
+        case 1: hipLaunchKernelGGL(step_head_kernel<1>, grid, block, lds, stream, a); break;
+        case 2: hipLaunchKernelGGL(step_head_kernel<2>, grid, block, lds, stream, a); break;
+        case 3: hipLaunchKernelGGL(step_head_kernel<3>, grid, block, lds, stream, a); break;
+        default: hipLaunchKernelGGL(step_head_kernel<4>, grid, block, lds, stream, a); break;
+    }
+    GTAV_CHECK_HIP(hipGetLastError());
+    return 0;
+}
+
+bool step_tail_ok(int D, int Nfin, const LnPending* pend) {
+    if (!(D % 256 == 0 && D >= 256 && D <= 1024 && Nfin >= 1 && Nfin <= 64)) return false;
+    if (!pend) return true;
+    if (pend->x_out || pend->y_save || pend->tperm_T) return false;
+    return !pend->parts || (pend->nsplit >= 1 && pend->nsplit <= 8 && pend->ld % 4 == 0 && (!pend->gate || pend->rows_per_gate > 0));
+}
+
+int launch_step_tail(const float* x, int M, int D, int P, const LnPending* pend, const float* shift, const float* scale, int mod_stride, const int* mod_rows,
+                     const f16* w_fin, const float* b_fin, int Nfin, float* vout, int C, int H, int W, int p, int* err_ln, float* ddim_x, int F, int Tq,
+                     const StepParams* sp, float* v_last, hipStream_t stream) {
+    GTAV_REQUIRE(step_tail_ok(D, Nfin, pend) && H % p == 0 && W % p == 0 && Nfin == C * p * p && P == (H / p) * (W / p), "step_tail: bad geometry (D=%d, Nfin=%d)", D, Nfin);
+    GTAV_REQUIRE(!ddim_x || (sp && Tq >= 1), "step_tail: the DDIM update needs the step parameters");
+    TailArgs a;
+    a.x = x; a.M = M; a.D = D; a.P = P;
+    memset(&a.pd, 0, sizeof(a.pd));
+    if (pend) a.pd = *pend;
+    a.pd.err_flag = err_ln;
+    GTAV_REQUIRE(a.pd.live_T == 0 || (a.pd.live_P == P && M % P == 0), "step_tail: bad live-row map");
+    a.shift = shift; a.scale = scale; a.mod_stride = mod_stride; a.mod_rows = mod_rows; a.w_fin = w_fin; a.b_fin = b_fin; a.Nfin = Nfin;
+    a.vout = vout; a.C = C; a.H = H; a.W = W; a.p = p; a.ddim_x = ddim_x; a.F = F; a.Tq = Tq > 0 ? Tq : 1; a.sp = sp; a.v_last = v_last;
+    const dim3 grid(cdiv(M, ER)), block(ET);
+    const size_t xs_bytes = (size_t)D * ER * 2, red_bytes = 3 * 4 * 64 * sizeof(f32x4);
+    const size_t lds = xs_bytes > red_bytes ? xs_bytes : red_bytes;
+    switch (D / 256) {
+        case 1: hipLaunchKernelGGL(step_tail_kernel<1>, grid, block, lds, stream, a); break;
+        case 2: hipLaunchKernelGGL(step_tail_kernel<2>, grid, block, lds, stream, a); break;
+        case 3: hipLaunchKernelGGL(step_tail_kernel<3>, grid, block, lds, stream, a); break;
+        default: hipLaunchKernelGGL(step_tail_kernel<4>, grid, block, lds, stream, a); break;
+    }
+    GTAV_CHECK_HIP(hipGetLastError());
+    return 0;
+}
+
+}
diff --git a/ai-generated-gtav_amd/csrc/struct_layout.h b/ai-generated-gtav_amd/csrc/struct_layout.h
--- a/ai-generated-gtav_amd/csrc/struct_layout.h
+++ b/ai-generated-gtav_amd/csrc/struct_layout.h
@@ -3,15 +3,15 @@
 
 #define GTAV_LAYOUT_GemmParams_SIZE 352
 #define GTAV_LAYOUT_GemmParams(F) \
-    F(X, 0) F(ldx, 8) F(W, 16) F(M, 24) F(N, 28) F(K, 32) F(debug, 36) F(stamps, 40) F(err_flag, 48) F(out_sc1, 56) F(splitk, 60) F(bias, 64) \
+    F(X, 0) F(ldx, 8) F(live_rows, 12) F(W, 16) F(M, 24) F(N, 28) F(K, 32) F(debug, 36) F(stamps, 40) F(err_flag, 48) F(out_sc1, 56) F(splitk, 60) F(bias, 64) \
     F(out2, 72) F(out, 80) F(ldo, 88) F(gate, 96) F(gate_stride, 104) F(gate_rows, 112) F(rows_per_gate, 120) F(qkv_mode, 124) F(q, 128) F(k, 136) \
     F(v, 144) F(D, 152) F(S, 156) F(Tq, 160) F(t0, 164) F(Tmax, 168) F(rope_cs, 176) F(rope_cs_q, 184) F(tm, 192) F(f_P, 228) F(f_rows, 232) \
     F(f_stats, 240) F(f_nslot, 248) F(f_c1, 256) F(f_c2, 264) F(f_ldc, 272) F(f_stats_out, 280) F(f_scale, 288) F(f_a, 296) F(pf, 304) F(sk_ws, 328) \
     F(sk_flags, 336) F(sk_dp, 344) F(sk_r, 348)
-#define GTAV_LAYOUT_LnPending_SIZE 104
+#define GTAV_LAYOUT_LnPending_SIZE 112
 #define GTAV_LAYOUT_LnPending(F) \
     F(parts, 0) F(nsplit, 8) F(slab_stride, 16) F(ld, 24) F(bias, 32) F(gate, 40) F(gate_stride, 48) F(gate_rows, 56) F(rows_per_gate, 64) \
-    F(flags, 68) F(err_flag, 72) F(x_out, 80) F(y_save, 88) F(tperm_T, 96) F(tperm_P, 100)
+    F(flags, 68) F(err_flag, 72) F(x_out, 80) F(y_save, 88) F(tperm_T, 96) F(tperm_P, 100) F(live_T, 104) F(live_P, 108)
 #define GTAV_LAYOUT_GemmDwGroup_SIZE 40
 #define GTAV_LAYOUT_GemmDwGroup(F) \
     F(X, 0) F(W, 8) F(out, 16) F(M, 24) F(N, 28) F(ldo, 32)
```

Measured after the change: 5.052 (median of 2 runs). Within noise of the previous version (+0.2%).
